# funkelab/cellulus

Measured on AMD Instinct MI355X. Metric: train crops/sec (U-Net fwd+bwd + OCE loss + Adam), higher is better.
Workload: dtype f32 (exact 3xbf16 operand split, 6 products, f32 accumulate)

## Files before the change

### cellulus_amd/_clx.py

```python

import ctypes
import os
from ctypes import POINTER, Structure, c_char_p, c_double, c_int, c_longlong, c_size_t, c_void_p

import torch

_HERE = os.path.dirname(os.path.abspath(__file__))
LIB_PATH = os.path.join(_HERE, "libclx.so")


class ClxError(RuntimeError):
    """A libclx entry point returned a negative status."""


class ClxSrc(Structure):

    _fields_ = [
        ("ptr", c_void_p),
        ("C", c_int),
        ("ld", c_int),
        ("D", c_int),
        ("H", c_int),
        ("W", c_int),
        ("oz", c_int),
        ("oy", c_int),
        ("ox", c_int),
        ("fz", c_int),
        ("fy", c_int),
        ("fx", c_int),
    ]


class ClxPackJob(Structure):

    _fields_ = [("w", c_void_p), ("wp", c_void_p), ("cout", c_int), ("cin", c_int), ("taps", c_int),
                ("cin_pad", c_int), ("cout_pad", c_int), ("mode", c_int)]


class ClxConvDesc(Structure):

    _fields_ = [
        ("nsrc", c_int),
        ("src", ClxSrc * 2),
        ("B", c_int),
        ("ID", c_int),
        ("IH", c_int),
        ("IW", c_int),
        ("KD", c_int),
        ("KH", c_int),
        ("KW", c_int),
        ("PD", c_int),
        ("PH", c_int),
        ("PW", c_int),
        ("N", c_int),
        ("wpack", c_void_p),
        ("bias", c_void_p),
        ("relu", c_int),
        ("mask", c_void_p),
        ("ld_mask", c_int),
        ("out", c_void_p),
        ("ld_out", c_int),
        ("accumulate", c_int),
        ("algo", c_int),
        ("workspace", c_void_p),
        ("workspace_bytes", c_size_t),
        ("vcache", c_void_p),
        ("vcache_valid", c_int),
        ("c_real", c_int),
        ("dy_vcache", c_void_p),
        ("gate_out", c_void_p),
        ("ld_gate", c_int),
        ("mask_bits", c_void_p),
        ("ld_mask_bits", c_int),
        ("det_turns", c_void_p),
        ("adjoint", c_int),
        ("pool_out", c_void_p),
        ("ld_pool", c_int),
        ("tile_list", c_void_p),
        ("tile_count", c_int),
        ("precision", c_int),
        ("wplanes", c_void_p),
        ("aplanes", c_void_p),
        ("aplanes_valid", c_int),
        ("dyplanes", c_void_p),
        ("dyplanes_valid", c_int),
        ("out_planes", c_void_p),
        ("out_colsum", c_void_p),
    ]


_P = c_void_p
_I = c_int
_LL = c_longlong
_D = c_double

PROTOTYPES = {
    "clx_last_error": (c_char_p, []),
    "clx_abi_version": (_I, []),
    "clx_device_count": (_I, []),
    "clx_profile_enable": (_I, [_I]),
    "clx_profile_read": (_I, [_I, POINTER(c_double), POINTER(c_double), POINTER(c_double)]),
    "clx_profile_clock": (_I, [POINTER(c_double), POINTER(c_double), _I]),
    "clx_conv_fwd": (_I, [POINTER(ClxConvDesc), _P]),
    "clx_conv_wgrad": (_I, [POINTER(ClxConvDesc), _P, _I, _P, _P, _P]),
    "clx_chain64_fwd": (_I, [_P, _I, _LL, _P, _P, _P, _I, _P, _I, _P, _P, _I, _I, _P, _I, _P, _I, _P]),
    "clx_chain64_bwd": (_I, [_P, _I, _I, _P, _I, _P, _I, _I, _LL, _P, _P, _P, _I, _P, _P, _P, _P, _P]),
    "clx_pack_weights": (_I, [_P, _P, _I, _I, _I, _I, _I, _I, _P]),
    "clx_pack_weights_batch": (_I, [_P, _I, _LL, _P]),
    "clx_unpack_wgrad": (_I, [_P, _P, _I, _I, _I, _I, _I, _P]),
    "clx_unpack_wgrad_wino": (_I, [_P, _P, _I, _I, _I, _I, _I, _I, _I, _P]),
    "clx_conv_workspace_bytes": (c_size_t, [POINTER(ClxConvDesc), _I]),
    "clx_conv_vcache_bytes": (c_size_t, [POINTER(ClxConvDesc), _I]),
    "clx_conv_sp_covers": (_I, [POINTER(ClxConvDesc), _I]),
    "clx_planes_bytes": (c_size_t, [_LL, _I]),
    "clx_split_planes": (_I, [_P, _LL, _LL, _I, _P, _P]),
    "clx_join_planes": (_I, [_P, _LL, _I, _P, _LL, _P]),
    "clx_gemm_planes": (_I, [_P, _P, _I, _I, _I, _P, _I, _P, _I, _P]),
    "clx_wgrad_planes": (_I, [_P, _P, _LL, _I, _I, _P, _I, _P]),
    "clx_conv_fused_applicable": (_I, [POINTER(ClxConvDesc)]),
    "clx_conv_fused_workspace_bytes": (c_size_t, [POINTER(ClxConvDesc)]),
    "clx_planar_to_pixel": (_I, [_P, _P, _I, _I, _LL, _I, _P]),
    "clx_pixel_to_planar": (_I, [_P, _P, _I, _I, _LL, _I, _P]),
    "clx_depth_to_space": (_I, [_P, _I, _P, _I, _I, _I, _I, _I, _I, _I, _I, _I, _P]),
    "clx_space_to_depth": (_I, [_P, _I, _P, _I, _I, _I, _I, _I, _I, _I, _I, _I, _P]),
    "clx_subpixel_split_weights": (_I, [_P, _P, _P] + [_I] * 10 + [_P]),
    "clx_subpixel_fold_grads": (_I, [_P, _P, _P] + [_I] * 10 + [_P]),
    "clx_maxpool_fwd": (_I, [_P, _P, _I, _I, _I, _I, _I, _I, _I, _I, _P]),
    "clx_changed_rows_workspace": (c_size_t, [_I, _I, _I, _I]),
    "clx_changed_rows": (_I, [_P, _P, _I, _I, _I, _I, _I, _I, _I, _I, _I, _P, _P, _LL, _P, _P]),
    "clx_changed_tiles": (_I, [_P, _I, _I, _I, _I, _I, _I, _I, _I, _I, _I, _I, _P, _P, _LL, _P]),
    "clx_grey_rows": (_I, [_P, _I, _I, _I, _I, _I, _P, _LL, _P, _P, _I, _I, _P, _I, _P]),
    "clx_conv_first_dgrad": (_I, [_P, _I, _P, _I, _I, _I, _I, _I, _I, _I, _P, _P]),
    "clx_gather_rows": (_I, [_P, _I, _P, _LL, _I, _P, _I, _P]),
    "clx_scatter_rows": (_I, [_P, _I, _P, _LL, _I, _P, _I, _P]),
    "clx_broadcast_rows": (_I, [_P, _LL, _P, _I, _P]),
    "clx_maxpool_bwd": (_I, [_P, _P, _P, _P] + [_I] * 7 + [_P] + [_I] * 8 + [_P]),
    "clx_upsample_bwd": (_I, [_P] + [_I] * 8 + [_P, _P] + [_I] * 8 + [_P]),
    "clx_gather_add_fwd": (_I, [_P, _P, _P, _I, _I, _I, _I, _I, _I, _P, _P]),
    "clx_gather_add_bwd": (_I, [_P, _P, _P, _I, _I, _I, _I, _I, _I, _P, _P]),
    "clx_oce_loss_fwd_bwd": (_I, [_P, _P, _P, _P, _LL, _I, ctypes.c_float, ctypes.c_float, ctypes.c_float, _P]),
    "clx_conv_wgrad_turns_bytes": (c_size_t, [POINTER(ClxConvDesc)]),
    "clx_colsum_scratch_bytes": (c_size_t, [_I]),
    "clx_colsum_ordered": (_I, [_P, _I, _LL, _I, _P, _P, _P]),
    "clx_oce_pairs_det_scratch_bytes": (c_size_t, [_I, _I, _LL]),
    "clx_oce_pairs_fused_det": (_I, [_P, _P, _P, _P, _P, _I, _I, _I, _I, _I, _I, ctypes.c_float, ctypes.c_float, _P, _P]),
    "clx_oce_pairs_fused": (_I, [_P, _P, _P, _P, _P, _I, _I, _I, _I, _I, _I, ctypes.c_float, ctypes.c_float, _P]),
    "clx_sample_pairs": (_I, [_P, _P, _P, _I, _I, _I, _I, _I, _I, POINTER(c_int), ctypes.c_ulonglong,
                              ctypes.c_ulonglong, _P]),
    "clx_adam_step": (_I, [_P, _P, _P, _P, _LL, _D, _D, _D, _D, _D, _I, _P]),
    "clx_adam_step_guarded": (_I, [_P, _P, _P, _P, _LL, _D, _D, _D, _D, _D, _I, _P, _P]),
    "clx_noise_stats": (_I, [_P, _P, _I, _I, _LL, _P]),
    "clx_noise_inject": (_I, [_P, _P, _P, _I, _I, _LL, ctypes.c_float, _P]),
    "clx_zero_many": (_I, [POINTER(_P), POINTER(_LL), _I, _P]),
    "clx_gather_rows_f64": (_I, [_P, _P, _LL, _I, _P, _P]),
    "clx_rows_extent_f64": (_I, [_P, _LL, _I, _P, _P]),
    "clx_noise_stats_minmax": (_I, [_P, _P, _I, _I, _LL, _P, _I, _P]),
    "clx_ms_prepare_workspace": (c_size_t, [_LL]),
    "clx_ms_prepare": (_I, [_P, _P, _D, _I, _I, _I, _I, _P, _P, _P, _P, _P]),
    "clx_ms_prepare_f32": (_I, [_P, _P, _D, _I, _I, _I, _I, _P, _P, _P, _P, _P]),
    "clx_ms_iterate": (_I, [_P, _I, _P, _I, _I, _D, _I, _P, _P, _P, _P]),
    "clx_ms_iterate_grid": (_I, [_P, _I, _P, POINTER(c_double), _D, _I, _I, _I, _P, _I, _I, _D, _I,
                                 _P, _P, _P, _P]),
    "clx_ms_assign": (_I, [_P, _P, _I, _P, _I, _I, _P, _P]),
    "clx_ms_assign_grid": (_I, [_P, _P, _I, _P, _I, _I, _P, _P, POINTER(c_double), _D, _I, _I, _I, _P, _P]),
    "clx_ms_assign_cells": (_I, [_P, _P, _I, _P, _I, _I, _P, _P, POINTER(c_double), _D, _I, _I, _I, _P, _P]),
    "clx_ms_assign_dense": (_I, [_P, _P, _I, _I, _P, _P, POINTER(c_double), _D, _I, _I, _I, _P, _I, _I, _I, _I, _P, _P]),
    "clx_ms_dedup_centers": (_I, [_P, _P, _I, _I, _D, _P, POINTER(_I)]),
    "clx_sample_offsets_mt19937": (_I, [_P, POINTER(_I), _I, _I, _LL, _P, POINTER(_I)]),
    "clx_elastic_crop_workspace": (c_size_t, [_I, POINTER(c_int), _I]),
    "clx_elastic_crop": (_I, [_P, _I, _I, _I, _I, POINTER(c_int), POINTER(c_int), POINTER(c_int), ctypes.c_float, _I, _I,
                              _P, _P, _P, _P, _P, _P]),
    "clx_ms_bucket_workspace": (c_size_t, [_I, _LL]),
    "clx_ms_bucket": (_I, [_P, _I, _I, POINTER(c_double), _D, _I, _I, _I, _P, _P, _P, _P]),
    "clx_offset_magnitude": (_I, [_P, _P, _I, _LL, _P]),
    "clx_gaussian_filter_f64": (_I, [_P, _P, _P, _I, _I, _I, _P, _I, _P]),
    "clx_negate_f64": (_I, [_P, _P, _LL, _P]),
    "clx_peak_local_max": (_I, [_P, _I, _I, _I, _P, _P, _I, _P, _P]),
    "clx_greedy_cluster": (_I, [_P, _P, _I, _I, _I, _D, _I, _D, _I, _P, _P, _P, _P]),
    "clx_cc_workspace": (c_size_t, [_LL]),
    "clx_cc_label_filter": (_I, [_P, _P, _I, _I, _I, _I, _P, _P, _P]),
    "clx_edt_workspace": (c_size_t, [_LL]),
    "clx_edt_sq": (_I, [_P, _P, _I, _I, _I, _I, _P, _P]),
    "clx_grow_shrink": (_I, [_P, _I, _I, _I, _I, _I, _P, _P]),
    "clx_minmax_f64": (_I, [_P, _LL, _P, _P]),
    "clx_histogram_f64": (_I, [_P, _LL, _P, _I, _P, _P]),
    "clx_minmax_f32": (_I, [_P, _LL, _P, _P]),
    "clx_histogram_f32": (_I, [_P, _LL, _P, _I, _P, _P]),
    "clx_inst_stats": (_I, [_P, _P, _I, _I, _I, _I, _I, _P, _P, _P]),
    "clx_inst_histogram": (_I, [_P, _P, _I, _LL, _P, _I, _P, _I, _P, _P]),
    "clx_inst_refine": (_I, [_P, _P, _I, _I, _I, _I, _I, _P, _P, _P, _P, _P, _I, _P, _P]),
    "clx_lz4_decompress": (_LL, [_P, _LL, _P, _LL]),
    "clx_blosclz_decompress": (_LL, [_P, _LL, _P, _LL]),
    "clx_blosc_compress_bound": (_LL, [_LL]),
    "clx_blosc_compress_lz4": (_LL, [_P, _LL, _I, _I, _P, _LL]),
    "clx_unshuffle_bytes": (_I, [_P, _P, _LL, _I]),
    "clx_label_presence": (_I, [_P, _LL, _I, _P, _P, _P]),
    "clx_joint_histogram": (_I, [_P, _P, _LL, _P, _P, _I, _P, _P]),
}

MINMAX_DOUBLES = 2 + 2 * 512
NOISE_MINMAX_FLOATS = 2 + 2 * 1024
ROWS_EXTENT_DOUBLES = 6 * (1 + 256)
NOISE_MINMAX_MAX_T = 64

_lib = None


def load():
    global _lib
    if _lib is not None:
        return _lib
    if not os.path.exists(LIB_PATH):
        raise ClxError(
            f"{LIB_PATH} is missing: build it with `python -m cellulus_amd._build` "
            "(hipcc --offload-arch=gfx950). cellulus_amd has no CPU fallback."
        )
    lib = ctypes.CDLL(LIB_PATH)
    for name, (restype, argtypes) in PROTOTYPES.items():
        fn = getattr(lib, name)
        fn.restype = restype
        fn.argtypes = argtypes
    _lib = lib
    return lib


def check(status, what=""):
    if status != 0:
        msg = load().clx_last_error().decode("utf-8", "replace")
        raise ClxError(f"{what or 'libclx'} failed ({status}): {msg}")


def stream_ptr(device=None):
    return c_void_p(torch.cuda.current_stream(device).cuda_stream)


def ptr(t):
    if t is None:
        return c_void_p(0)
    return c_void_p(t.data_ptr())


def zero_many(*tensors):
    ts = [t for t in tensors if t is not None and t.numel() > 0]
    if not ts:
        return
    dev = ts[0].device
    fast = []
    for t in ts:
        if not t.is_cuda:
            raise ClxError(f"zero_many: tensor on {t.device}; there is no CPU path")
        if t.device != dev:
            raise ClxError(f"zero_many: tensors on different devices ({dev} and {t.device}) in one call")
        nbytes = t.numel() * t.element_size()
        if t.is_contiguous() and t.data_ptr() % 16 == 0 and nbytes % 4 == 0:
            fast.append(t)
        else:
            t.zero_()
    if not fast:
        return
    ptrs = (_P * len(fast))(*[t.data_ptr() for t in fast])
    sizes = (_LL * len(fast))(*[t.numel() * t.element_size() for t in fast])
    call("clx_zero_many", ptrs, sizes, len(fast), stream_ptr(dev))


def zeros(shape, dtype, device):
    t = torch.empty(shape, dtype=dtype, device=device)
# ... 20 lines not shown
```

### cellulus_amd/csrc/clx_common.h

```cpp
#pragma once
#include <hip/hip_runtime.h>
#include <hip/hip_ext.h>
#include <stdint.h>
#include <stdio.h>
#include <stdarg.h>
#include "../../include/clx.h"

void clx_set_error(const char* fmt, ...);

#define CLX_REQUIRE(cond, ...)                \
  do {                                        \
    if (!(cond)) {                            \
      clx_set_error(__VA_ARGS__);             \
      return CLX_ERR_ARG;                     \
    }                                         \
  } while (0)

#define CLX_CHECK_LAUNCH(name)                                           \
  do {                                                                   \
    hipError_t e__ = hipGetLastError();                                  \
    if (e__ != hipSuccess) {                                             \
      clx_set_error("%s: launch failed: %s", name, hipGetErrorString(e__)); \
      return CLX_ERR_LAUNCH;                                             \
    }                                                                    \
  } while (0)

typedef float f32x4 __attribute__((ext_vector_type(4)));
typedef float f32x16 __attribute__((ext_vector_type(16)));

struct FastDiv {
  uint32_t m, l, d;
};
static inline FastDiv make_fastdiv(uint32_t d) {
  FastDiv f;
  f.d = d;
  uint32_t l = 0;
  while ((1ull << l) < d) ++l;
  f.l = l;
  f.m = (uint32_t)(((1ull << 32) * ((1ull << l) - d)) / d + 1);
  return f;
}
__device__ __forceinline__ uint32_t fdiv(uint32_t n, const FastDiv& f) {
  return (__umulhi(f.m, n) + n) >> f.l;
}

__device__ __forceinline__ int xcd_remap(int bid, int nblocks) {
  const int q = nblocks >> 3, r = nblocks & 7;
  const int xcd = bid & 7, idx = bid >> 3;
  const int base = (xcd < r) ? xcd * (q + 1) : r * (q + 1) + (xcd - r) * q;
  return base + idx;
}

static inline int cdiv(long long a, long long b) { return (int)((a + b - 1) / b); }

bool clx_smallc_applicable(const clx_conv_desc* d);
int clx_smallc_fwd(const clx_conv_desc* d, hipStream_t st);
int clx_smallc_wgrad(const clx_conv_desc* d, const float* dy, int ld_dy, float* dwpack,
                     float* dbias, hipStream_t st);

int clx_igemm_launch(const clx_conv_desc* d, int batch, long long bs_in, long long bs_w,
                     long long bs_out, hipStream_t st);
int clx_wgrad_launch(const clx_conv_desc* d, const float* dy, int ld_dy, float* dwpack, float* dbias,
                     int batch, long long bs_x, long long bs_dy, long long bs_out, hipStream_t st);
bool clx_sp_fwd_rule(const clx_conv_desc* d);
bool clx_sp_wgrad_rule(const clx_conv_desc* d);
bool clx_sp_applicable(const clx_conv_desc* d);
bool clx_wino_sp(const clx_conv_desc* d);
int clx_sp_launch(const void* A, const void* B, int M, int N, int K, long long rows_a, int batch, long long bs_a, long long bs_b,
                  long long bs_out, const clx_conv_desc* ep, hipStream_t st);
int clx_sp_clock_read(double* shader_ticks, double* wall_ticks, int reset);
int clx_sp_split(const float* x, long long ld, long long rows, int K, void* planes, float* colsum, int nreal, hipStream_t st);
int clx_sp_wgrad_launch(const void* dy_planes, const void* x_planes, long long rows, int N, int C, int batch, long long bs_dy,
                        long long bs_x, long long bs_out, float* dw, int ld_dw, hipStream_t st);
int clx_wino_fwd(const clx_conv_desc* d, hipStream_t st);
int clx_wino_wgrad(const clx_conv_desc* d, const float* dy, int ld_dy, float* dwpack, float* dbias,
                   hipStream_t st);
int clx_wino_pack(const float* w, float* wp, int cout, int cin, int cin_pad, int cout_pad, int dgrad, int tile,
                  int ksize, int kd, hipStream_t st);

int clx_wino_fused_fwd(const clx_conv_desc* d, hipStream_t st);

bool clx_prof_enabled();
void clx_prof_events(int kind, double flops, hipEvent_t* e0, hipEvent_t* e1);
#define CLX_LAUNCH_TIMED(kernel, grid, block, st, e0, e1, ...) \
  hipExtLaunchKernelGGL(kernel, grid, block, 0, st, e0, e1, 0, __VA_ARGS__)
#define CLX_LAUNCH_KIND(kind, kernel, grid, block, lds, st, ...)                              \
  do {                                                                                        \
    hipEvent_t e0__ = nullptr, e1__ = nullptr;                                                \
    if (clx_prof_enabled()) clx_prof_events(kind, 0.0, &e0__, &e1__);                         \
    hipExtLaunchKernelGGL(kernel, grid, block, lds, st, e0__, e1__, 0, __VA_ARGS__);          \
  } while (0)
```

### cellulus_amd/csrc/conv_igemm.hip

```cpp
#include "clx_common.h"
#include <stdlib.h>

__device__ unsigned long long g_clk_ticks[2];
extern "C" int clx_profile_clock(double* shader_ticks, double* wall_ticks_100mhz, int reset) {
  unsigned long long h[2] = {0ull, 0ull};
  if (hipMemcpyFromSymbol(h, HIP_SYMBOL(g_clk_ticks), sizeof(h)) != hipSuccess) {
    clx_set_error("clx_profile_clock: copy failed");
    return CLX_ERR_LAUNCH;
  }
  double sc = 0.0, sw = 0.0;
  if (clx_sp_clock_read(&sc, &sw, reset) != CLX_OK) {
    clx_set_error("clx_profile_clock: copy failed");
    return CLX_ERR_LAUNCH;
  }
  if (shader_ticks) *shader_ticks = (double)h[0] + sc;
  if (wall_ticks_100mhz) *wall_ticks_100mhz = (double)h[1] + sw;
  if (reset) {
    const unsigned long long z[2] = {0ull, 0ull};
    if (hipMemcpyToSymbol(HIP_SYMBOL(g_clk_ticks), z, sizeof(z)) != hipSuccess) {
      clx_set_error("clx_profile_clock: reset failed");
      return CLX_ERR_LAUNCH;
    }
  }
  return CLX_OK;
// ... 330 lines not shown
  constexpr int PH = 8;
  static_assert(ITERS % PH == 0, "phases");
  const int c4 = (tid % F4_PER_ROW) * 4;
  const int n = n0 + c4;
  const bool n_live = n < p.N;
  const bool full4 = n + 3 < p.N;
#pragma unroll 1
  for (int h0 = 0; h0 < ITERS; h0 += PH) {
    f32x4 val[PH];
    int mrow[PH];
    bool live[PH];
#pragma unroll
    for (int j = 0; j < PH; ++j) {
      const int row = (tid + 256 * (h0 + j)) / F4_PER_ROW;
      mrow[j] = m0 + row;
      live[j] = mrow[j] < p.M && n_live;
      val[j] = *reinterpret_cast<const f32x4*>(&Cs[row * LDC + c4]);
    }
    float* const out_base = p.out + blockIdx.y * p.bs_out + n;
    if (p.accumulate) {
      f32x4 prev[PH];
#pragma unroll
      for (int j = 0; j < PH; ++j)
        prev[j] = *reinterpret_cast<const f32x4*>(live[j] ? out_base + (size_t)mrow[j] * p.ld_out : p.zeros);
#pragma unroll
      for (int j = 0; j < PH; ++j) val[j] += prev[j];
    }
    if (p.relu) {
#pragma unroll
      for (int j = 0; j < PH; ++j)
#pragma unroll
        for (int e = 0; e < 4; ++e) val[j][e] = fmaxf(val[j][e], 0.f);
    }
    if (p.mask_bits) {
      unsigned int w[PH];
#pragma unroll
      for (int j = 0; j < PH; ++j)
        w[j] = live[j] ? p.mask_bits[(size_t)mrow[j] * p.ld_mask_bits + (n >> 5)] : 0u;
#pragma unroll
      for (int j = 0; j < PH; ++j)
#pragma unroll
        for (int e = 0; e < 4; ++e) val[j][e] = ((w[j] >> ((n & 31) + e)) & 1u) ? val[j][e] : 0.f;
    }
    if (p.gate_out) {
#pragma unroll
      for (int j = 0; j < PH; ++j) {
        unsigned int nib = 0u;
#pragma unroll
        for (int e = 0; e < 4; ++e) nib |= (live[j] && n + e < p.N && val[j][e] > 0.f) ? (1u << e) : 0u;
        unsigned int word = nib << (4 * (lane & 7));
        word |= __shfl_xor(word, 1, 64);
        word |= __shfl_xor(word, 2, 64);
        word |= __shfl_xor(word, 4, 64);
        if ((lane & 7) == 0 && mrow[j] < p.M && n < p.ld_out) p.gate_out[(size_t)mrow[j] * p.ld_gate + (n >> 5)] = word;
      }
    }
    if (p.mask && full4) {
      f32x4 mk[PH];
#pragma unroll
      for (int j = 0; j < PH; ++j)
        mk[j] = *reinterpret_cast<const f32x4*>(live[j] ? p.mask + (size_t)mrow[j] * p.ld_mask + n : p.zeros);
#pragma unroll
      for (int j = 0; j < PH; ++j)
#pragma unroll
        for (int e = 0; e < 4; ++e) val[j][e] = (!live[j] || mk[j][e] > 0.f) ? val[j][e] : 0.f;
    }
    if (full4) {
#pragma unroll
      for (int j = 0; j < PH; ++j)
        if (live[j]) *reinterpret_cast<f32x4*>(out_base + (size_t)mrow[j] * p.ld_out) = val[j];
    } else if (n_live) {
#pragma unroll 1
      for (int j = 0; j < PH; ++j) {
        if (!live[j]) continue;
        float* dst = out_base + (size_t)mrow[j] * p.ld_out;
        for (int e = 0; e < 4 && n + e < p.N; ++e) {
          float x = val[j][e];
          if (p.mask) x = (p.mask[(size_t)mrow[j] * p.ld_mask + n + e] > 0.f) ? x : 0.f;
          dst[e] = x;
        }
      }
    }
  }
  if (clk_block) { atomicAdd(&g_clk_ticks[0], clock64() - clk_c0); atomicAdd(&g_clk_ticks[1], wall_clock64() - clk_w0); }
}

}

static const float* zero_buffer() {
  static const float* cache[64] = {nullptr};
  int dev = 0;
  if (hipGetDevice(&dev) != hipSuccess || dev < 0 || dev >= 64) return nullptr;
  if (cache[dev] == nullptr) {
    void* ptr = nullptr;
    if (hipGetSymbolAddress(&ptr, HIP_SYMBOL(g_zero16)) != hipSuccess) return nullptr;
    cache[dev] = (const float*)ptr;
  }
  return cache[dev];
}

static int conv_validate(const clx_conv_desc* d, const char* who) {
  CLX_REQUIRE(d != nullptr, "%s: null descriptor", who);
  CLX_REQUIRE(d->nsrc == 1 || d->nsrc == 2, "%s: nsrc must be 1 or 2", who);
  CLX_REQUIRE(d->B > 0 && d->ID > 0 && d->IH > 0 && d->IW > 0, "%s: bad extent", who);
  const int K[3] = {d->KD, d->KH, d->KW};
  const int P[3] = {d->PD, d->PH, d->PW};
  const int I[3] = {d->ID, d->IH, d->IW};
  for (int i = 0; i < 3; ++i) {
    CLX_REQUIRE(K[i] >= 1 && K[i] <= 3, "%s: kernel extent must be 1, 2 or 3", who);
    CLX_REQUIRE(P[i] >= 0 && P[i] < K[i], "%s: padding must be < kernel extent", who);
    CLX_REQUIRE(I[i] + 2 * P[i] - K[i] + 1 > 0, "%s: input smaller than kernel", who);
  }
  for (int s = 0; s < d->nsrc; ++s) {
    const clx_src& S = d->src[s];
    CLX_REQUIRE(S.ptr != nullptr, "%s: null source %d", who, s);
    CLX_REQUIRE(S.C > 0 && S.C % 4 == 0 && S.ld % 4 == 0 && S.ld >= S.C,
                "%s: source channels/ld must be multiples of 4 (C=%d ld=%d)", who, S.C, S.ld);
    CLX_REQUIRE(((uintptr_t)S.ptr & 15) == 0, "%s: source pointer must be 16-byte aligned", who);
    CLX_REQUIRE(S.fz >= 1 && S.fy >= 1 && S.fx >= 1, "%s: upsample factors >= 1", who);
    CLX_REQUIRE(S.oz >= 0 && S.oy >= 0 && S.ox >= 0, "%s: negative crop", who);
    CLX_REQUIRE((d->ID - 1 + S.oz) / S.fz < S.D && (d->IH - 1 + S.oy) / S.fy < S.H &&
                    (d->IW - 1 + S.ox) / S.fx < S.W,
                "%s: source %d smaller than the logical input", who, s);
  }
  const long long M = (long long)d->B * (d->ID + 2 * d->PD - d->KD + 1) *
                      (d->IH + 2 * d->PH - d->KH + 1) * (d->IW + 2 * d->PW - d->KW + 1);
  CLX_REQUIRE(M < (1ll << 31), "%s: too many output pixels", who);
  return CLX_OK;
}

static void fill_params(const clx_conv_desc* d, ConvP& p) {
  p.nsrc = d->nsrc;
  for (int s = 0; s < 2; ++s) {
    const clx_src& S = d->src[s < d->nsrc ? s : 0];
    p.src[s] = SrcP{S.ptr, S.C, S.ld, S.D, S.H, S.W, S.oz, S.oy, S.ox, S.fz, S.fy, S.fx};
  }
  p.B = d->B; p.ID = d->ID; p.IH = d->IH; p.IW = d->IW;
  p.KD = d->KD; p.KH = d->KH; p.KW = d->KW;
  p.PD = d->PD; p.PH = d->PH; p.PW = d->PW;
  p.OD = d->ID + 2 * d->PD - d->KD + 1;
  p.OH = d->IH + 2 * d->PH - d->KH + 1;
  p.OW = d->IW + 2 * d->PW - d->KW + 1;
  p.N = d->N;
  p.M = d->B * p.OD * p.OH * p.OW;
  p.Ctot = d->src[0].C + (d->nsrc == 2 ? d->src[1].C : 0);
  p.Ktot = p.Ctot * d->KD * d->KH * d->KW;
  p.dOW = make_fastdiv(p.OW); p.dOH = make_fastdiv(p.OH); p.dOD = make_fastdiv(p.OD);
  p.wpack = d->wpack; p.bias = d->bias; p.mask = d->mask; p.out = d->out;
  p.gate_out = d->gate_out; p.ld_gate = d->ld_gate; p.mask_bits = d->mask_bits; p.ld_mask_bits = d->ld_mask_bits;
  p.relu = d->relu; p.ld_mask = d->ld_mask; p.ld_out = d->ld_out;
  p.accumulate = d->accumulate;
  p.bs_in = p.bs_w = p.bs_out = 0;
  p.flush_every = 0;
}

extern "C" int clx_conv_fwd(const clx_conv_desc* d, clx_stream stream) {
  int rc = conv_validate(d, "clx_conv_fwd");
  if (rc) return rc;
  CLX_REQUIRE(d->wpack && d->out, "clx_conv_fwd: null wpack/out");
  CLX_REQUIRE(d->N > 0 && d->ld_out >= d->N, "clx_conv_fwd: bad N/ld_out");
  CLX_REQUIRE(((uintptr_t)d->wpack & 15) == 0, "clx_conv_fwd: wpack must be 16-byte aligned");
  CLX_REQUIRE(d->mask == nullptr || (d->ld_mask >= d->N && d->ld_mask % 4 == 0 &&
                                     ((uintptr_t)d->mask & 15) == 0),
              "clx_conv_fwd: mask must be 16-byte aligned with ld_mask %% 4 == 0 and >= N");
  CLX_REQUIRE(d->ld_out % 4 == 0 && ((uintptr_t)d->out & 15) == 0,
              "clx_conv_fwd: out must be 16-byte aligned with ld_out %% 4 == 0");
  CLX_REQUIRE(d->gate_out == nullptr || (d->relu && d->ld_out % 32 == 0 && d->ld_gate * 32 >= d->ld_out),
              "clx_conv_fwd: gate_out needs relu, ld_out %% 32 == 0 and ld_gate >= ld_out / 32");
  CLX_REQUIRE(d->mask_bits == nullptr || (d->mask == nullptr && d->ld_mask_bits * 32 >= d->N),
              "clx_conv_fwd: mask_bits replaces mask and needs ld_mask_bits >= ceil(N / 32)");
  CLX_REQUIRE(d->algo == CLX_ALGO_DIRECT || d->algo == CLX_ALGO_WINOGRAD || d->algo == CLX_ALGO_WINOGRAD4 ||
                  d->algo == CLX_ALGO_WINOGRAD4_FUSED,
              "clx_conv_fwd: bad algo");
  CLX_REQUIRE((d->out_planes == nullptr && d->out_colsum == nullptr && !d->aplanes_valid) ||
                  (d->algo == CLX_ALGO_DIRECT && d->aplanes != nullptr && clx_sp_applicable(d)),
              "clx_conv_fwd: out_planes / out_colsum / aplanes_valid need the split-precision 1x1 product "
              "(clx_conv_sp_covers, wplanes and aplanes)");
  if (d->algo == CLX_ALGO_WINOGRAD4_FUSED) return clx_wino_fused_fwd(d, (hipStream_t)stream);
  if (d->algo != CLX_ALGO_DIRECT) return clx_wino_fwd(d, (hipStream_t)stream);
  CLX_REQUIRE(d->pool_out == nullptr && d->tile_list == nullptr && !d->adjoint,
              "clx_conv_fwd: pool_out / tile_list / adjoint need a Winograd algorithm (algo = %d)", d->algo);
  if (clx_smallc_applicable(d) && d->mask == nullptr && d->mask_bits == nullptr && d->gate_out == nullptr) {
    clx_smallc_fwd(d, (hipStream_t)stream);
    CLX_CHECK_LAUNCH("clx_conv_fwd(small-channel)");
    return CLX_OK;
  }
  rc = clx_igemm_launch(d, 1, 0, 0, 0, (hipStream_t)stream);
  if (rc) return rc;
  CLX_CHECK_LAUNCH("clx_conv_fwd");
  return CLX_OK;
}

int clx_igemm_launch(const clx_conv_desc* d, int batch, long long bs_in, long long bs_w,
                     long long bs_out, hipStream_t st) {
  if (batch == 1 && d->aplanes != nullptr && clx_sp_applicable(d)) {
    const clx_src& S = d->src[0];
    const long long M = (long long)d->B * d->ID * d->IH * d->IW;
    if (!d->aplanes_valid) {
      const int rc = clx_sp_split(S.ptr, S.ld, M, S.C, d->aplanes, nullptr, 0, st);
      if (rc) return rc;
    }
    return clx_sp_launch(d->aplanes, d->wplanes, (int)M, d->N, S.C, M, 1, 0, 0, 0, d, st);
  }
  ConvP p;
  fill_params(d, p);
  p.zeros = zero_buffer();
  CLX_REQUIRE(p.zeros != nullptr, "clx_conv_fwd: cannot resolve the device zero buffer");
  p.bs_in = bs_in; p.bs_w = bs_w; p.bs_out = bs_out;
  static const int flush_env = getenv("CLX_IGEMM_FLUSH") ? atoi(getenv("CLX_IGEMM_FLUSH")) : 2;
  p.flush_every = flush_env > 0 ? flush_env : 0;
  const bool wide = d->N > 64 && (double)(cdiv(d->N, 128) * 128) / d->N <= 1.2;
  hipEvent_t e0 = nullptr, e1 = nullptr;
  if (clx_prof_enabled())
    clx_prof_events(wide ? CLX_PROF_IGEMM_WIDE : CLX_PROF_IGEMM_NARROW, 2.0 * p.M * p.N * p.Ktot * batch, &e0, &e1);
  static const bool fast_env = getenv("CLX_IGEMM_FAST") == nullptr || atoi(getenv("CLX_IGEMM_FAST")) != 0;
  int fast = fast_env && (long long)p.N * p.Ktot < (1ll << 30) ? 1 : 0;
  const bool padded = d->PD != 0 || d->PH != 0 || d->PW != 0;
  for (int s = 0; s < d->nsrc && fast; ++s) {
    const clx_src& S = d->src[s];
    const long long floats = (long long)d->B * S.D * S.H * S.W * S.ld;
    if (S.C % BK != 0 || floats >= (padded ? (1ll << 29) : (1ll << 30))) fast = 0;
  }
  if (fast && padded) fast = 2;
  static const bool dbg = getenv("CLX_IGEMM_DEBUG") != nullptr;
  if (dbg) fprintf(stderr, "igemm fast=%d wide=%d M=%d N=%d K=%d batch=%d pad=%d%d%d k=%d%d%d nsrc=%d C0=%d\n", (int)fast, (int)wide, p.M, p.N, p.Ktot, batch, d->PD, d->PH, d->PW, d->KD, d->KH, d->KW, d->nsrc, d->src[0].C);
  if (wide) {
    p.nbm = cdiv(p.M, 128); p.nbn = cdiv(p.N, 128);
    if (fast == 1) CLX_LAUNCH_TIMED((conv_igemm_kernel<128, 128, 2, 2, 1>), dim3(p.nbm * p.nbn, batch), dim3(256), st, e0, e1, p);
    else if (fast == 2) CLX_LAUNCH_TIMED((conv_igemm_kernel<128, 128, 2, 2, 2>), dim3(p.nbm * p.nbn, batch), dim3(256), st, e0, e1, p);
    else CLX_LAUNCH_TIMED((conv_igemm_kernel<128, 128, 2, 2>), dim3(p.nbm * p.nbn, batch), dim3(256), st, e0, e1, p);
  } else {
    p.nbm = cdiv(p.M, 128); p.nbn = cdiv(p.N, 64);
    if (fast == 1) CLX_LAUNCH_TIMED((conv_igemm_kernel<128, 64, 4, 1, 1>), dim3(p.nbm * p.nbn, batch), dim3(256), st, e0, e1, p);
    else if (fast == 2) CLX_LAUNCH_TIMED((conv_igemm_kernel<128, 64, 4, 1, 2>), dim3(p.nbm * p.nbn, batch), dim3(256), st, e0, e1, p);
    else CLX_LAUNCH_TIMED((conv_igemm_kernel<128, 64, 4, 1>), dim3(p.nbm * p.nbn, batch), dim3(256), st, e0, e1, p);
  }
  return CLX_OK;
}
```

### cellulus_amd/csrc/conv_smallc.hip

```cpp
#include "clx_common.h"

namespace {

struct SmallP {
  const float* x;
  int ld_x, B, D, H, W;
  int oz, oy, ox;
  int ID, IH, IW, KD, KH, KW, PD, PH, PW, OD, OH, OW;
  int N, M, taps;
  FastDiv dOW, dOH, dOD;
  const float* wpack;
  const float* bias;
  float* out;
  int ld_out, relu;
  const float* dy;
  int ld_dy;
  float* dwp;
  float* dbias;
  int tiles_per_block;
  int RX, items;
  FastDiv dRX;
};

constexpr int PT = 64;
constexpr int MAX_TAPS = 27;

template <int PTILE>
__device__ __forceinline__ void stage_patch(const SmallP& p, int m0, float* Xs) {
  static_assert(256 % PTILE == 0, "a thread keeps one pixel of the tile");
  const int K4 = p.taps;
  const int pl = threadIdx.x % PTILE;
  const uint32_t m = (uint32_t)(m0 + pl);
  const bool live = m < (uint32_t)p.M;
  const uint32_t q1 = fdiv(m, p.dOW);
  const int ox = (int)(m - q1 * p.OW);
  const uint32_t q2 = fdiv(q1, p.dOH);
  const int oy = (int)(q1 - q2 * p.OH);
  const uint32_t q3 = fdiv(q2, p.dOD);
  const int oz = (int)(q2 - q3 * p.OD);
  const int b = (int)q3;
  int tx = 0, ty = 0, tz = 0;
  {
    const int tap = threadIdx.x / PTILE;
    tx = tap % p.KW; ty = (tap / p.KW) % p.KH; tz = tap / (p.KW * p.KH);
  }
  constexpr int STEP = 256 / PTILE;
  for (int tap = threadIdx.x / PTILE; tap < K4; tap += STEP) {
    f32x4 v = {0.f, 0.f, 0.f, 0.f};
    const int lz = oz + tz - p.PD, ly = oy + ty - p.PH, lx = ox + tx - p.PW;
    if (live && (unsigned)lz < (unsigned)p.ID && (unsigned)ly < (unsigned)p.IH && (unsigned)lx < (unsigned)p.IW) {
      const long long pix = (((long long)b * p.D + lz + p.oz) * p.H + ly + p.oy) * p.W + lx + p.ox;
      v = *reinterpret_cast<const f32x4*>(p.x + pix * p.ld_x);
    }
    *reinterpret_cast<f32x4*>(&Xs[(pl * K4 + tap) * 4]) = v;
    tx += STEP;
    while (tx >= p.KW) { tx -= p.KW; if (++ty == p.KH) { ty = 0; ++tz; } }
  }
}

template <int NG>
__global__ __launch_bounds__(256) void conv_smallc_fwd_kernel(const SmallP p) {
  constexpr int PL = 256 / NG;
  constexpr int PPT = PT / PL;
  extern __shared__ float smem[];
  const int K = p.taps * 4;
  float* Ws = smem;
  float* Xs = smem + K * NG * 4;
  const int n0 = blockIdx.y * NG * 4;
  const int ng = threadIdx.x % NG, pl = threadIdx.x / NG;
  __shared__ int used_channels;
  if (threadIdx.x == 0) used_channels = 0;
  __syncthreads();
  int mine_used = 0;
  for (int idx = threadIdx.x; idx < K * NG * 4; idx += 256) {
    const int n = idx / K, k = idx % K;
    const float wv = (n0 + n < p.N) ? p.wpack[(size_t)(n0 + n) * K + k] : 0.f;
    Ws[k * NG * 4 + n] = wv;
    if (wv != 0.f) mine_used |= 1 << (k & 3);
  }
  if (mine_used) atomicOr(&used_channels, mine_used);
  const int n = n0 + ng * 4;
  f32x4 bv = {0.f, 0.f, 0.f, 0.f};
  if (p.bias && n < p.N) {
#pragma unroll
    for (int e = 0; e < 4; ++e) bv[e] = (n + e < p.N) ? p.bias[n + e] : 0.f;
  }
  for (int t = 0; t < p.tiles_per_block; ++t) {
    const int m0 = (blockIdx.x * p.tiles_per_block + t) * PT;
    if (m0 >= p.M) break;
    __syncthreads();
    stage_patch<PT>(p, m0, Xs);
    __syncthreads();
    f32x4 acc[PPT];
#pragma unroll
    for (int i = 0; i < PPT; ++i) acc[i] = bv;
    const int used = used_channels;
    for (int c = 0; c < 4; ++c) {
      if (!((used >> c) & 1)) continue;
      for (int k = c; k < K; k += 4) {
        const f32x4 w = *reinterpret_cast<const f32x4*>(&Ws[k * NG * 4 + ng * 4]);
#pragma unroll
        for (int i = 0; i < PPT; ++i) {
          const float xv = Xs[(pl + i * PL) * K + k];
          acc[i] += xv * w;
        }
      }
    }
    if (n < p.N) {
#pragma unroll
      for (int i = 0; i < PPT; ++i) {
        const int m = m0 + pl + i * PL;
        if (m >= p.M) continue;
        f32x4 v = acc[i];
        if (p.relu) {
#pragma unroll
          for (int e = 0; e < 4; ++e) v[e] = fmaxf(v[e], 0.f);
        }
        float* dst = p.out + (size_t)m * p.ld_out + n;
        if (n + 3 < p.N) *reinterpret_cast<f32x4*>(dst) = v;
        else
          for (int e = 0; e < 4 && n + e < p.N; ++e) dst[e] = v[e];
      }
    }
  }
}

template <int G>
__global__ __launch_bounds__(256) void conv_smallc_wgrad_stream_kernel(const SmallP p) {
  constexpr int Q = 256 / G;
  constexpr int MT = 9;
  extern __shared__ float red[];
  const int g = threadIdx.x % G, q = threadIdx.x / G;
  const int NT = G * 4;
  const int n0 = blockIdx.y * NT, n = n0 + g * 4;
  const int tap0 = blockIdx.z * MT;
  const int ntap = p.taps - tap0 < MT ? p.taps - tap0 : MT;
  const int nred = ntap * 4 * NT + NT;
  for (int i = threadIdx.x; i < nred; i += 256) red[i] = 0.f;
  f32x4 acc[MT][4];
#pragma unroll
  for (int a = 0; a < MT; ++a)
#pragma unroll
    for (int c = 0; c < 4; ++c) acc[a][c] = f32x4{0.f, 0.f, 0.f, 0.f};
  f32x4 bsum = {0.f, 0.f, 0.f, 0.f};
  const long long per = (long long)p.tiles_per_block;
  const long long m_begin = (long long)blockIdx.x * per;
  const long long m_end = m_begin + per < p.M ? m_begin + per : p.M;
  const bool live = n < p.N;
  const int gtap = tap0 + (g < ntap ? g : 0);
  const int my_tx = gtap % p.KW - p.PW, my_ty = (gtap / p.KW) % p.KH - p.PH, my_tz = gtap / (p.KW * p.KH) - p.PD;
  for (long long mm = m_begin + q; mm < m_end; mm += Q) {
    const uint32_t m = (uint32_t)mm;
    const uint32_t q1 = fdiv(m, p.dOW);
    const int ox = (int)(m - q1 * p.OW);
    const uint32_t q2 = fdiv(q1, p.dOH);
    const int oy = (int)(q1 - q2 * p.OH);
    const uint32_t q3 = fdiv(q2, p.dOD);
    const int oz = (int)(q2 - q3 * p.OD);
    const int b = (int)q3;
    f32x4 dyv = {0.f, 0.f, 0.f, 0.f};
    if (live) dyv = *reinterpret_cast<const f32x4*>(p.dy + (size_t)m * p.ld_dy + n);
    if (tap0 == 0) bsum += dyv;
    if constexpr (G >= 16) {
      f32x4 mine = {0.f, 0.f, 0.f, 0.f};
      if (g < ntap) {
        const int lz = oz + my_tz, ly = oy + my_ty, lx = ox + my_tx;
        if ((unsigned)lz < (unsigned)p.ID && (unsigned)ly < (unsigned)p.IH && (unsigned)lx < (unsigned)p.IW) {
          const long long pix = (((long long)b * p.D + lz + p.oz) * p.H + ly + p.oy) * p.W + lx + p.ox;
          mine = *reinterpret_cast<const f32x4*>(p.x + pix * p.ld_x);
        }
      }
#pragma unroll
      for (int a = 0; a < MT; ++a) {
        if (a < ntap) {
          f32x4 xv;
#pragma unroll
          for (int c = 0; c < 4; ++c) {
            xv[c] = __shfl(mine[c], (int)(threadIdx.x & 63 & ~(G - 1)) + a, 64);
          }
#pragma unroll
          for (int c = 0; c < 4; ++c) acc[a][c] += xv[c] * dyv;
        }
      }
    } else {
#pragma unroll
      for (int a = 0; a < MT; ++a) {
        if (a < ntap) {
          const int tap = tap0 + a;
          const int lz = oz + tap / (p.KW * p.KH) - p.PD, ly = oy + (tap / p.KW) % p.KH - p.PH, lx = ox + tap % p.KW - p.PW;
          f32x4 xv = {0.f, 0.f, 0.f, 0.f};
          if ((unsigned)lz < (unsigned)p.ID && (unsigned)ly < (unsigned)p.IH && (unsigned)lx < (unsigned)p.IW) {
            const long long pix = (((long long)b * p.D + lz + p.oz) * p.H + ly + p.oy) * p.W + lx + p.ox;
            xv = *reinterpret_cast<const f32x4*>(p.x + pix * p.ld_x);
          }
#pragma unroll
          for (int c = 0; c < 4; ++c) acc[a][c] += xv[c] * dyv;
        }
      }
    }
  }
  __syncthreads();
#pragma unroll
  for (int a = 0; a < MT; ++a) {
    if (a < ntap) {
#pragma unroll
      for (int c = 0; c < 4; ++c)
#pragma unroll
        for (int e = 0; e < 4; ++e) atomicAdd(&red[(a * 4 + c) * NT + g * 4 + e], acc[a][c][e]);
    }
  }
#pragma unroll
  for (int e = 0; e < 4; ++e) atomicAdd(&red[ntap * 4 * NT + g * 4 + e], bsum[e]);
  __syncthreads();
  for (int i = threadIdx.x; i < ntap * 4 * NT; i += 256) {
    const int nl = i % NT, c = (i / NT) & 3, tap = tap0 + i / (4 * NT);
    if (n0 + nl < p.N) atomicAdd(p.dwp + ((size_t)tap * p.N + n0 + nl) * 4 + c, red[i]);
  }
  if (p.dbias && tap0 == 0)
    for (int i = threadIdx.x; i < NT; i += 256)
      if (n0 + i < p.N) atomicAdd(p.dbias + n0 + i, red[ntap * 4 * NT + i]);
}

struct Run {
  int ox0, m0;
  long long base;
};

__device__ __forceinline__ Run decode_run(const SmallP& p, uint32_t item) {
  const uint32_t q1 = fdiv(item, p.dRX);
  const int rx = (int)(item - q1 * p.RX);
  const uint32_t q2 = fdiv(q1, p.dOH);
  const int oy = (int)(q1 - q2 * p.OH);
  const uint32_t q3 = fdiv(q2, p.dOD);
  const int oz = (int)(q2 - q3 * p.OD);
  const int b = (int)q3;
  Run r;
  r.ox0 = rx * 4;
  r.m0 = ((b * p.OD + oz) * p.OH + oy) * p.OW + r.ox0;
  r.base = (((long long)b * p.D + oz + p.oz) * p.H + oy + p.oy) * p.W + r.ox0 + p.ox;
  return r;
}

template <int KD>
struct GreyLane {
  static constexpr int R = KD * 3, NP = R * 6, TAPS = R * 3;
  int px, cq, col;
  long long poff;
  __device__ __forceinline__ GreyLane(const SmallP& p) {
    const int lane = threadIdx.x & 63;
    px = lane >> 4; cq = lane & 15;
    const int l = lane < NP ? lane : 0;
    const int r = l / 6;
    col = l - r * 6;
    const int tz = r / 3, ty = r - tz * 3;
    poff = ((long long)tz * p.H + ty) * p.W;
  }
  __device__ __forceinline__ float load_patch(const SmallP& p, const Run& r) const {
    const int c = r.ox0 + col < p.IW ? col : p.IW - 1 - r.ox0;
    return p.x[(r.base + poff + c) * p.ld_x];
  }
  __device__ __forceinline__ float tap(float pv, int row, int tx) const {
    return __shfl(pv, row * 6 + tx + px, 64);
  }
};

template <int KD>
__global__ __launch_bounds__(256) void conv_grey_fwd_kernel(const SmallP p) {
  using L = GreyLane<KD>;
  const L ln(p);
  const int wave = __builtin_amdgcn_readfirstlane(threadIdx.x >> 6);
  const int n = blockIdx.y * 64 + ln.cq * 4;
  const bool live_n = n < p.N;
  f32x4 w[L::TAPS];
#pragma unroll
  for (int t = 0; t < L::TAPS; ++t)
#pragma unroll
    for (int e = 0; e < 4; ++e) w[t][e] = live_n ? p.wpack[((size_t)(n + e) * L::TAPS + t) * 4] : 0.f;
  f32x4 bv = {0.f, 0.f, 0.f, 0.f};
  if (p.bias && live_n) bv = *reinterpret_cast<const f32x4*>(p.bias + n);
  const uint32_t last = (uint32_t)p.items - 1, stride = gridDim.x * 4;
  uint32_t item = blockIdx.x * 4 + wave;
  Run r[3];
  float pv[3];
#pragma unroll
  for (int s = 0; s < 2; ++s) {
    r[s] = decode_run(p, item + s * stride < last ? item + s * stride : last);
    pv[s] = ln.load_patch(p, r[s]);
  }
  while (true) {
#pragma unroll
    for (int s = 0; s < 3; ++s) {
      if (item > last) return;
      const int s2 = (s + 2) % 3;
      const uint32_t nxt = item + 2 * stride;
      r[s2] = decode_run(p, nxt < last ? nxt : last);
      pv[s2] = ln.load_patch(p, r[s2]);
      f32x4 acc = bv;
#pragma unroll
      for (int row = 0; row < L::R; ++row)
#pragma unroll
        for (int tx = 0; tx < 3; ++tx) acc += ln.tap(pv[s], row, tx) * w[row * 3 + tx];
      if (p.relu) {
#pragma unroll
        for (int e = 0; e < 4; ++e) acc[e] = fmaxf(acc[e], 0.f);
      }
      if (live_n && r[s].ox0 + ln.px < p.OW)
        *reinterpret_cast<f32x4*>(p.out + (size_t)(r[s].m0 + ln.px) * p.ld_out + n) = acc;
      item += stride;
    }
  }
}

template <int KD>
__global__ __launch_bounds__(256) void conv_grey_wgrad_kernel(const SmallP p) {
  using L = GreyLane<KD>;
  __shared__ float red[(L::TAPS + 1) * 64];
  const L ln(p);
  const int wave = __builtin_amdgcn_readfirstlane(threadIdx.x >> 6);
  const int n0 = blockIdx.y * 64, n = n0 + ln.cq * 4;
  const bool live_n = n < p.N;
  const int nld = live_n ? n : 0;
  for (int i = threadIdx.x; i < (L::TAPS + 1) * 64; i += 256) red[i] = 0.f;
  f32x4 acc[L::TAPS];
#pragma unroll
  for (int t = 0; t < L::TAPS; ++t) acc[t] = f32x4{0.f, 0.f, 0.f, 0.f};
  f32x4 bsum = {0.f, 0.f, 0.f, 0.f};
  const uint32_t last = (uint32_t)p.items - 1, stride = gridDim.x * 4;
  uint32_t item = blockIdx.x * 4 + wave;
  auto load_dy = [&](const Run& r) {
    const int m = r.ox0 + ln.px < p.OW ? r.m0 + ln.px : r.m0;
    return *reinterpret_cast<const f32x4*>(p.dy + (size_t)m * p.ld_dy + nld);
  };
  Run r[3];
  float pv[3];
  f32x4 dy[3];
#pragma unroll
  for (int s = 0; s < 2; ++s) {
    r[s] = decode_run(p, item + s * stride < last ? item + s * stride : last);
    pv[s] = ln.load_patch(p, r[s]);
    dy[s] = load_dy(r[s]);
  }
  bool more = item <= last;
  while (more) {
#pragma unroll
    for (int s = 0; s < 3; ++s) {
      if (more) {
        const int s2 = (s + 2) % 3;
        const uint32_t nxt = item + 2 * stride;
        r[s2] = decode_run(p, nxt < last ? nxt : last);
        pv[s2] = ln.load_patch(p, r[s2]);
        dy[s2] = load_dy(r[s2]);
        const bool ok = live_n && r[s].ox0 + ln.px < p.OW;
        f32x4 dyv;
#pragma unroll
        for (int e = 0; e < 4; ++e) dyv[e] = ok ? dy[s][e] : 0.f;
        bsum += dyv;
#pragma unroll
        for (int row = 0; row < L::R; ++row)
#pragma unroll
          for (int tx = 0; tx < 3; ++tx) acc[row * 3 + tx] += ln.tap(pv[s], row, tx) * dyv;
        item += stride;
        more = item <= last;
      }
    }
  }
  __syncthreads();
#pragma unroll
  for (int t = 0; t < L::TAPS; ++t)
#pragma unroll
    for (int e = 0; e < 4; ++e) atomicAdd(&red[t * 64 + ln.cq * 4 + e], acc[t][e]);
#pragma unroll
  for (int e = 0; e < 4; ++e) atomicAdd(&red[L::TAPS * 64 + ln.cq * 4 + e], bsum[e]);
  __syncthreads();
  for (int i = threadIdx.x; i < L::TAPS * 64; i += 256) {
    const int nl = i & 63, t = i >> 6;
    if (n0 + nl < p.N) atomicAdd(p.dwp + ((size_t)t * p.N + n0 + nl) * 4, red[i]);
  }
  if (p.dbias && threadIdx.x < 64 && n0 + threadIdx.x < p.N)
    atomicAdd(p.dbias + n0 + threadIdx.x, red[L::TAPS * 64 + threadIdx.x]);
}

template <int KD>
__global__ __launch_bounds__(256) void conv_grey_rows_kernel(const float* __restrict__ x, int D, int H, int W, int OD,
                                                             int OH, int OW, const int* __restrict__ rows, long long n,
                                                             const float* __restrict__ wpack,
                                                             const float* __restrict__ bias, int relu, int N,
                                                             float* __restrict__ out, int ld_out) {
  constexpr int R = KD * 3, TAPS = R * 3;
  const int lane = threadIdx.x & 63, px = lane >> 4, cq = lane & 15;
  const int nn = blockIdx.y * 64 + cq * 4;
  const bool live_n = nn < N;
  f32x4 w[TAPS];
#pragma unroll
  for (int t = 0; t < TAPS; ++t)
#pragma unroll
    for (int e = 0; e < 4; ++e) w[t][e] = live_n ? wpack[((size_t)(nn + e) * TAPS + t) * 4] : 0.f;
  f32x4 bv = {0.f, 0.f, 0.f, 0.f};
  if (bias && live_n) bv = *reinterpret_cast<const f32x4*>(bias + nn);
  const long long npo = (long long)OD * OH * OW;
  const long long groups = (n + 3) / 4;
  for (long long g = (long long)blockIdx.x * 4 + (threadIdx.x >> 6); g < groups; g += (long long)gridDim.x * 4) {
    const long long r = g * 4 + px;
    const bool live = r < n;
    const long long row = rows[live ? r : n - 1];
    const long long b = row / npo, pix = row - b * npo;
    const int ox = (int)(pix % OW), oy = (int)((pix / OW) % OH), oz = (int)(pix / ((long long)OW * OH));
    const float* src = x + ((b * D + oz) * H + oy) * (long long)W + ox;
    float xv[TAPS];
#pragma unroll
    for (int rr = 0; rr < R; ++rr)
#pragma unroll
      for (int tx = 0; tx < 3; ++tx) xv[rr * 3 + tx] = src[((long long)(rr / 3) * H + (rr % 3)) * W + tx];
    f32x4 acc = bv;
#pragma unroll
    for (int rr = 0; rr < R; ++rr)
#pragma unroll
      for (int tx = 0; tx < 3; ++tx) acc += xv[rr * 3 + tx] * w[rr * 3 + tx];
    if (relu) {
#pragma unroll
      for (int e = 0; e < 4; ++e) acc[e] = fmaxf(acc[e], 0.f);
    }
    if (live && live_n) *reinterpret_cast<f32x4*>(out + (size_t)r * ld_out + nn) = acc;
  }
}

bool grey_applicable(const clx_conv_desc* d, int ld_act) {
  return d->c_real == 1 && d->KH == 3 && d->KW == 3 && (d->KD == 1 || d->KD == 3) && d->PD == 0 &&
         d->PH == 0 && d->PW == 0 && d->N % 4 == 0 && ld_act % 4 == 0;
}

dim3 grey_grid(SmallP& p) {
  p.RX = cdiv(p.OW, 4);
  p.items = p.B * p.OD * p.OH * p.RX;
  p.dRX = make_fastdiv(p.RX);
  const int ny = cdiv(p.N, 64);
  int nx = 768 / ny;
  if (nx < 1) nx = 1;
  if (nx > cdiv(p.items, 4)) nx = cdiv(p.items, 4);
  return dim3(nx, ny);
}

bool fill(const clx_conv_desc* d, SmallP& p) {
  const clx_src& S = d->src[0];
  p.x = S.ptr; p.ld_x = S.ld; p.B = d->B; p.D = S.D; p.H = S.H; p.W = S.W;
  p.oz = S.oz; p.oy = S.oy; p.ox = S.ox;
  p.ID = d->ID; p.IH = d->IH; p.IW = d->IW;
  p.KD = d->KD; p.KH = d->KH; p.KW = d->KW;
  p.PD = d->PD; p.PH = d->PH; p.PW = d->PW;
  p.OD = d->ID + 2 * d->PD - d->KD + 1;
  p.OH = d->IH + 2 * d->PH - d->KH + 1;
  p.OW = d->IW + 2 * d->PW - d->KW + 1;
  p.N = d->N;
  p.M = d->B * p.OD * p.OH * p.OW;
  p.taps = d->KD * d->KH * d->KW;
  p.dOW = make_fastdiv(p.OW); p.dOH = make_fastdiv(p.OH); p.dOD = make_fastdiv(p.OD);
  return true;
}

int pick_ng(int N) {
  int ng = 4;
  while (ng < 64 && ng * 4 < N) ng *= 2;
  return ng;
}

}

bool clx_smallc_applicable(const clx_conv_desc* d) {
  if (d->nsrc != 1 || d->accumulate) return false;
  const clx_src& S = d->src[0];
  if (S.C != 4 || S.fz != 1 || S.fy != 1 || S.fx != 1) return false;
  const int taps = d->KD * d->KH * d->KW;
  return taps > 1 && taps <= MAX_TAPS && d->N >= 4;
}

int clx_smallc_fwd(const clx_conv_desc* d, hipStream_t st) {
  SmallP p{};
  fill(d, p);
  p.wpack = d->wpack; p.bias = d->bias; p.out = d->out; p.ld_out = d->ld_out; p.relu = d->relu;
  if (grey_applicable(d, d->ld_out) && ((uintptr_t)d->out & 15) == 0 && (!d->bias || ((uintptr_t)d->bias & 15) == 0)) {
    const dim3 grid = grey_grid(p);
    if (d->KD == 1) conv_grey_fwd_kernel<1><<<grid, 256, 0, st>>>(p);
    else conv_grey_fwd_kernel<3><<<grid, 256, 0, st>>>(p);
    return CLX_OK;
  }
  const int ng = pick_ng(p.N);
  const int K = p.taps * 4;
  const int tiles = cdiv(p.M, PT);
  p.tiles_per_block = tiles > 4096 ? 4 : 1;
  const dim3 grid(cdiv(tiles, p.tiles_per_block), cdiv(p.N, ng * 4));
  const size_t lds = (size_t)(K * ng * 4 + PT * K) * sizeof(float);
  switch (ng) {
    case 4: conv_smallc_fwd_kernel<4><<<grid, 256, lds, st>>>(p); break;
    case 8: conv_smallc_fwd_kernel<8><<<grid, 256, lds, st>>>(p); break;
    case 16: conv_smallc_fwd_kernel<16><<<grid, 256, lds, st>>>(p); break;
    case 32: conv_smallc_fwd_kernel<32><<<grid, 256, lds, st>>>(p); break;
    default: conv_smallc_fwd_kernel<64><<<grid, 256, lds, st>>>(p); break;
  }
  return CLX_OK;
}

int clx_smallc_wgrad(const clx_conv_desc* d, const float* dy, int ld_dy, float* dwpack,
                     float* dbias, hipStream_t st) {
  SmallP p{};
  fill(d, p);
  p.dy = dy; p.ld_dy = ld_dy; p.dwp = dwpack; p.dbias = dbias;
  if (grey_applicable(d, ld_dy) && ((uintptr_t)dy & 15) == 0) {
    const dim3 grid = grey_grid(p);
    if (d->KD == 1) conv_grey_wgrad_kernel<1><<<grid, 256, 0, st>>>(p);
    else conv_grey_wgrad_kernel<3><<<grid, 256, 0, st>>>(p);
    return CLX_OK;
  }
  const int ng = pick_ng(p.N);
  const int blocks = p.M < 512 * 64 ? cdiv(p.M, 64) : 512;
  p.tiles_per_block = cdiv(p.M, blocks);
  const dim3 grid(cdiv(p.M, p.tiles_per_block), cdiv(p.N, ng * 4), cdiv(p.taps, 9));
  const size_t lds = (size_t)((p.taps < 9 ? p.taps : 9) * 4 * ng * 4 + ng * 4) * sizeof(float);
  switch (ng) {
    case 4: conv_smallc_wgrad_stream_kernel<4><<<grid, 256, lds, st>>>(p); break;
    case 8: conv_smallc_wgrad_stream_kernel<8><<<grid, 256, lds, st>>>(p); break;
    case 16: conv_smallc_wgrad_stream_kernel<16><<<grid, 256, lds, st>>>(p); break;
    case 32: conv_smallc_wgrad_stream_kernel<32><<<grid, 256, lds, st>>>(p); break;
    default: conv_smallc_wgrad_stream_kernel<64><<<grid, 256, lds, st>>>(p); break;
  }
  return CLX_OK;
}

extern "C" int clx_grey_rows(const float* x, int B, int ID, int IH, int IW, int KD, const int* rows, long long n,
                             const float* wpack, const float* bias, int relu, int N, float* out, int ld_out,
                             clx_stream stream) {
  CLX_REQUIRE(n >= 0, "clx_grey_rows: bad count");
  if (n == 0) return CLX_OK;
  CLX_REQUIRE(x && rows && wpack && out, "clx_grey_rows: null pointer");
  CLX_REQUIRE(B > 0 && (KD == 1 || KD == 3) && ID >= KD && IH >= 3 && IW >= 3, "clx_grey_rows: a 3x3 or 3x3x3 window");
  CLX_REQUIRE(N > 0 && N % 4 == 0 && ld_out % 4 == 0 && ld_out >= N && ((uintptr_t)out & 15) == 0 &&
                  (!bias || ((uintptr_t)bias & 15) == 0),
              "clx_grey_rows: N, ld_out multiples of 4, aligned out / bias");
  const int OD = ID - KD + 1, OH = IH - 2, OW = IW - 2;
  long long gx = (n + 15) / 16;
  if (gx > 4096) gx = 4096;
  const dim3 grid((unsigned)gx, (unsigned)((N + 63) / 64));
  hipStream_t st = (hipStream_t)stream;
  if (KD == 1) conv_grey_rows_kernel<1><<<grid, 256, 0, st>>>(x, ID, IH, IW, OD, OH, OW, rows, n, wpack, bias, relu, N, out, ld_out);
  else conv_grey_rows_kernel<3><<<grid, 256, 0, st>>>(x, ID, IH, IW, OD, OH, OW, rows, n, wpack, bias, relu, N, out, ld_out);
  CLX_CHECK_LAUNCH("clx_grey_rows");
  return CLX_OK;
}
```

### cellulus_amd/csrc/gemm_sp.hip

```cpp
#include "clx_common.h"
#include "sp_planes.h"
#include <stdlib.h>
#include <type_traits>

__device__ unsigned long long g_sp_clk_ticks[2];
int clx_sp_clock_read(double* shader_ticks, double* wall_ticks, int reset) {
  unsigned long long h[2] = {0ull, 0ull};
  if (hipMemcpyFromSymbol(h, HIP_SYMBOL(g_sp_clk_ticks), sizeof(h)) != hipSuccess) return CLX_ERR_LAUNCH;
  *shader_ticks = (double)h[0];
  *wall_ticks = (double)h[1];
  if (reset) {
    const unsigned long long z[2] = {0ull, 0ull};
    if (hipMemcpyToSymbol(HIP_SYMBOL(g_sp_clk_ticks), z, sizeof(z)) != hipSuccess) return CLX_ERR_LAUNCH;
  }
  return CLX_OK;
}

namespace {

typedef __bf16 bf16x8 __attribute__((ext_vector_type(8)));
using sp::u32x2;
using sp::u32x4;
using sp::FRAG;
using sp::KSTEP;
constexpr int SP_BM = 256, SP_BN = 128;
constexpr int A_FRAGS = SP_BM / 32 * 3;
constexpr int B_FRAGS = SP_BN / 32 * 3;
constexpr int STAGE = (A_FRAGS + B_FRAGS) * FRAG;
constexpr int RING = 4;
constexpr int LDC = SP_BN + 4;

__device__ __forceinline__ void glds16(const char* g, char* l) {
  __builtin_amdgcn_global_load_lds((const __attribute__((address_space(1))) void*)g,
                                   (__attribute__((address_space(3))) void*)l, 16, 0, 0);
}

using sp::split4;

template <bool COLSUM>
__global__ __launch_bounds__(256) void sp_split_kernel(const float* __restrict__ x, long long ld, long long rows, int ksteps,
                                                       char* __restrict__ out, long long nfrag, float* __restrict__ colsum, int nreal) {
  const int lane = threadIdx.x & 63;
  const long long w0 = ((long long)blockIdx.x * blockDim.x + threadIdx.x) >> 6, nw = ((long long)gridDim.x * blockDim.x) >> 6;
  const int r = lane & 31, h = lane >> 5;
  f32x4 s0 = {0.f, 0.f, 0.f, 0.f}, s1 = s0;
  for (long long f = w0; f < nfrag; f += nw) {
    const int ks = (int)(f % ksteps);
    const long long rb = f / ksteps;
    const long long row = rb * 32 + r;
    f32x4 v0 = {0.f, 0.f, 0.f, 0.f}, v1 = v0;
    if (row < rows) {
      const float* src = x + row * ld + ks * 16 + h * 8;
      v0 = *reinterpret_cast<const f32x4*>(src);
      v1 = *reinterpret_cast<const f32x4*>(src + 4);
    }
    if constexpr (COLSUM) { s0 += v0; s1 += v1; }
    u32x2 a0, a1, a2, b0, b1, b2;
    split4(v0, a0, a1, a2);
    split4(v1, b0, b1, b2);
    char* dst = out + f * KSTEP + lane * 16;
    *reinterpret_cast<u32x4*>(dst) = u32x4{a0[0], a0[1], b0[0], b0[1]};
    *reinterpret_cast<u32x4*>(dst + FRAG) = u32x4{a1[0], a1[1], b1[0], b1[1]};
    *reinterpret_cast<u32x4*>(dst + 2 * FRAG) = u32x4{a2[0], a2[1], b2[0], b2[1]};
  }
  if constexpr (COLSUM) {
    if (w0 < nfrag) {
      const int ks = (int)(w0 % ksteps);
#pragma unroll
      for (int e = 0; e < 4; ++e) {
#pragma unroll
        for (int m = 1; m < 32; m <<= 1) { s0[e] += __shfl_xor(s0[e], m, 64); s1[e] += __shfl_xor(s1[e], m, 64); }
      }
      if (r == 0) {
#pragma unroll
        for (int e = 0; e < 4; ++e) {
          const int k0 = ks * 16 + h * 8 + e;
          if (k0 < nreal) atomicAdd(colsum + k0, s0[e]);
          if (k0 + 4 < nreal) atomicAdd(colsum + k0 + 4, s1[e]);
        }
      }
    }
  }
}

__global__ __launch_bounds__(256) void sp_join_kernel(const char* __restrict__ in, long long ld, long long rows, int ksteps,
                                                      float* __restrict__ x, long long nfrag) {
  const int lane = threadIdx.x & 63;
  const long long w0 = ((long long)blockIdx.x * blockDim.x + threadIdx.x) >> 6, nw = ((long long)gridDim.x * blockDim.x) >> 6;
  const int r = lane & 31, h = lane >> 5;
  for (long long f = w0; f < nfrag; f += nw) {
    const int ks = (int)(f % ksteps);
    const long long rb = f / ksteps;
    const long long row = rb * 32 + r;
    if (row >= rows) continue;
    const char* src = in + f * KSTEP + lane * 16;
    const u32x4 q0 = *reinterpret_cast<const u32x4*>(src), q1 = *reinterpret_cast<const u32x4*>(src + FRAG),
                q2 = *reinterpret_cast<const u32x4*>(src + 2 * FRAG);
    float* dst = x + row * ld + ks * 16 + h * 8;
#pragma unroll
    for (int e = 0; e < 8; ++e) {
      const int sh = (e & 1) * 16;
      const float f0 = __uint_as_float(((q0[e >> 1] >> sh) & 0xffffu) << 16);
      const float f1 = __uint_as_float(((q1[e >> 1] >> sh) & 0xffffu) << 16);
      const float f2 = __uint_as_float(((q2[e >> 1] >> sh) & 0xffffu) << 16);
      dst[e] = (f0 + f1) + f2;
    }
  }
}

__global__ __launch_bounds__(256) void sp_zero_tail_kernel(char* __restrict__ planes, long long bs, long long rows, int ksteps) {
  const long long rb0 = rows >> 5, rb1 = sp::padded_rows(rows) / 32;
  const int per_rb = ksteps * 6 * 32;
  const long long total = (rb1 - rb0) * per_rb;
  for (long long i = (long long)blockIdx.x * blockDim.x + threadIdx.x; i < total; i += (long long)gridDim.x * blockDim.x) {
    const long long rb = rb0 + i / per_rb;
    const int k = (int)(i % per_rb), r = k & 31, q = k >> 5;
    if (rb * 32 + r >= rows)
      *reinterpret_cast<u32x4*>(planes + blockIdx.y * bs + rb * ksteps * (long long)KSTEP + (long long)q * 512 + r * 16) = u32x4{0u, 0u, 0u, 0u};
  }
}

struct SpP {
  const char* A;
  const char* B;
  long long bs_a, bs_b, bs_out;
  float* out;
  int M, N, ksteps;
  int rb_a;
  int rb_b;
  const float* bias;
  const float* mask;
  const unsigned int* mask_bits;
  unsigned int* gate_out;
  const float* zeros;
  int relu, accumulate, ld_out, ld_mask, ld_mask_bits, ld_gate;
  int nbm, nbn;
  char* out_planes;
  float* colsum; int colsum_n;
  unsigned int stride_a, stride_b;
  int total_steps, steps_per_slice, nslices;
};

template <int BM = SP_BM, int NWAVES = 8, int BN = SP_BN>
__device__ __forceinline__ void sp_epilogue_from_lds(const SpP& p, const float* Cs, int m0, int n0, int batch, int tid, int lane) {
  constexpr int WPR = BN / 32;
  constexpr int LDC = BN + 4;
  constexpr int PASS_ROWS = NWAVES / WPR * 8;
  constexpr int ITERS = BM / PASS_ROWS;
  constexpr int PH = 8;
  static_assert(ITERS % PH == 0, "whole groups of passes");
  const int wv = tid >> 6;
  const int c4 = (wv % WPR) * 32 + (lane & 7) * 4;
  const int row0 = (wv / WPR) * 8 + (lane >> 3);
  const int n = n0 + c4;
  const bool n_live = n < p.N;
  f32x4 csum = {0.f, 0.f, 0.f, 0.f};
  const long long prow = p.out_planes ? sp::padded_rows(p.M) : 0;
#pragma unroll 1
  for (int h0 = 0; h0 < ITERS; h0 += PH) {
    f32x4 val[PH];
    int mrow[PH];
    bool live[PH];
#pragma unroll
    for (int j = 0; j < PH; ++j) {
      const int row = row0 + PASS_ROWS * (h0 + j);
      mrow[j] = m0 + row;
      live[j] = mrow[j] < p.M && n_live;
      val[j] = *reinterpret_cast<const f32x4*>(&Cs[row * LDC + c4]);
    }
    float* const out_base = p.out + batch * p.bs_out + n;
    if (p.accumulate) {
      f32x4 prev[PH];
#pragma unroll
      for (int j = 0; j < PH; ++j)
        prev[j] = *reinterpret_cast<const f32x4*>(live[j] ? out_base + (size_t)mrow[j] * p.ld_out : p.zeros);
#pragma unroll
      for (int j = 0; j < PH; ++j) val[j] += prev[j];
    }
    if (p.relu) {
#pragma unroll
      for (int j = 0; j < PH; ++j)
#pragma unroll
        for (int e = 0; e < 4; ++e) val[j][e] = fmaxf(val[j][e], 0.f);
    }
    if (p.mask_bits) {
      unsigned int wd[PH];
#pragma unroll
      for (int j = 0; j < PH; ++j) wd[j] = live[j] ? p.mask_bits[(size_t)mrow[j] * p.ld_mask_bits + (n >> 5)] : 0u;
#pragma unroll
      for (int j = 0; j < PH; ++j)
#pragma unroll
        for (int e = 0; e < 4; ++e) val[j][e] = ((wd[j] >> ((n & 31) + e)) & 1u) ? val[j][e] : 0.f;
    }
    if (p.gate_out) {
#pragma unroll
      for (int j = 0; j < PH; ++j) {
        unsigned int nib = 0u;
#pragma unroll
        for (int e = 0; e < 4; ++e) nib |= (live[j] && val[j][e] > 0.f) ? (1u << e) : 0u;
        unsigned int word = nib << (4 * (lane & 7));
        word |= __shfl_xor(word, 1, 64);
        word |= __shfl_xor(word, 2, 64);
        word |= __shfl_xor(word, 4, 64);
        if ((lane & 7) == 0 && mrow[j] < p.M && n_live) p.gate_out[(size_t)mrow[j] * p.ld_gate + (n >> 5)] = word;
      }
    }
    if (p.mask) {
      f32x4 mk[PH];
#pragma unroll
      for (int j = 0; j < PH; ++j)
        mk[j] = *reinterpret_cast<const f32x4*>(live[j] ? p.mask + (size_t)mrow[j] * p.ld_mask + n : p.zeros);
#pragma unroll
      for (int j = 0; j < PH; ++j)
#pragma unroll
        for (int e = 0; e < 4; ++e) val[j][e] = (!live[j] || mk[j][e] > 0.f) ? val[j][e] : 0.f;
    }
#pragma unroll
    for (int j = 0; j < PH; ++j)
      if (live[j]) *reinterpret_cast<f32x4*>(out_base + (size_t)mrow[j] * p.ld_out) = val[j];
    if (p.out_planes) {
#pragma unroll
      for (int j = 0; j < PH; ++j)
        if (n_live && mrow[j] < prow)
          sp::store4(p.out_planes, mrow[j], n, p.N >> 4, live[j] ? val[j] : f32x4{0.f, 0.f, 0.f, 0.f});
    }
    if (p.colsum) {
#pragma unroll
      for (int j = 0; j < PH; ++j)
        if (live[j]) csum += val[j];
    }
  }
  if (p.colsum) {
#pragma unroll
    for (int e = 0; e < 4; ++e) {
      csum[e] += __shfl_xor(csum[e], 8, 64);
      csum[e] += __shfl_xor(csum[e], 16, 64);
      csum[e] += __shfl_xor(csum[e], 32, 64);
    }
    if ((lane >> 3) == 0 && n_live) {
#pragma unroll
      for (int e = 0; e < 4; ++e)
        if (n + e < p.colsum_n) atomicAdd(p.colsum + n + e, csum[e]);
    }
  }
}

template <int MODE>
__global__ __launch_bounds__(512, 1) void gemm_sp_kernel(const SpP p) {
  __shared__ __attribute__((aligned(16))) char smem[RING * STAGE];
  const int tid = threadIdx.x, lane = tid & 63;
  const int w = __builtin_amdgcn_readfirstlane(tid >> 6);
  const int wm = w >> 1, wn = w & 1;
  int tile_m, tile_n, batch, step0 = 0, ksteps;
  if constexpr (MODE == 0) {
    const int v = xcd_remap(blockIdx.x, p.nbm * p.nbn);
    tile_n = v % p.nbn; tile_m = v / p.nbn;
    batch = blockIdx.y;
    ksteps = p.ksteps;
  } else {
    const int T = p.nbm * p.nbn;
    const int u = xcd_remap(blockIdx.x, gridDim.x);
    const int per_batch = T * p.nslices;
    batch = u / per_batch;
    const int v = u % per_batch;
    const int slice = v / T, t = v % T;
    tile_n = t % p.nbn; tile_m = t / p.nbn;
    step0 = slice * p.steps_per_slice;
    ksteps = p.total_steps - step0 < p.steps_per_slice ? p.total_steps - step0 : p.steps_per_slice;
  }
  const int m0 = tile_m * SP_BM, n0 = tile_n * SP_BN;
  const bool clk_block = blockIdx.x == gridDim.x / 2 && blockIdx.y == gridDim.y / 2 && threadIdx.x == 0;
  unsigned long long clk_c0 = 0, clk_w0 = 0;
  if (clk_block) { clk_c0 = clock64(); clk_w0 = wall_clock64(); }

  const char* const Ab = p.A + batch * p.bs_a;
  const char* const Bb = p.B + batch * p.bs_b;
  auto frag_base = [&](int f) __attribute__((always_inline)) -> const char* {
    if constexpr (MODE == 0) {
      if (f < A_FRAGS) {
        int rb = tile_m * (SP_BM / 32) + f / 3;
        if (rb > p.rb_a - 1) rb = p.rb_a - 1;
        return Ab + ((long long)rb * ksteps * 3 + f % 3) * FRAG;
      }
      const int g = f - A_FRAGS;
      int nb = tile_n * (SP_BN / 32) + g / 3;
      if (nb > p.rb_b - 1) nb = p.rb_b - 1;
      return Bb + ((long long)nb * ksteps * 3 + g % 3) * FRAG;
    } else {
      if (f < A_FRAGS) {
        int cb = tile_m * (SP_BM / 32) + f / 3;
        if (cb > p.M / 32 - 1) cb = p.M / 32 - 1;
        return Ab + ((long long)(2 * cb) * 3 + f % 3) * FRAG;
      }
      const int g = f - A_FRAGS;
      int cb = tile_n * (SP_BN / 32) + g / 3;
      if (cb > p.N / 32 - 1) cb = p.N / 32 - 1;
      return Bb + ((long long)(2 * cb) * 3 + g % 3) * FRAG;
    }
  };
  const char* gsrc[5];
#pragma unroll
  for (int q = 0; q < 4; ++q) gsrc[q] = frag_base(w + 8 * q);
  gsrc[4] = frag_base(32 + (w & 3));
  const int l_oct = lane >> 4, l_pix = (lane & 15) ^ (4 * (lane >> 4));
  const unsigned int lane16 = MODE == 0 ? (unsigned int)lane * 16u
                                        : (unsigned int)((l_oct >> 1) * KSTEP + (l_oct & 1) * 512 + l_pix * 16);
  const bool low_half = w < 4;
  auto issue = [&](int t, int slot, bool odd) __attribute__((always_inline)) {
    char* const dst = smem + slot * STAGE;
    if constexpr (MODE == 0) {
      const unsigned int voff = lane16 + (unsigned int)t * KSTEP;
#pragma unroll
      for (int q = 0; q < 4; ++q) glds16(gsrc[q] + (size_t)voff, dst + (w + 8 * q) * FRAG);
      if (low_half != odd) glds16(gsrc[4] + (size_t)voff, dst + (32 + (w & 3)) * FRAG);
    } else {
      const unsigned int ts = (unsigned int)(step0 + t);
      const unsigned int va = lane16 + (ts >> 1) * p.stride_a + (ts & 1u) * 256u;
      const unsigned int vb = lane16 + (ts >> 1) * p.stride_b + (ts & 1u) * 256u;
#pragma unroll
      for (int q = 0; q < 3; ++q) glds16(gsrc[q] + (size_t)va, dst + (w + 8 * q) * FRAG);
      glds16(gsrc[3] + (size_t)vb, dst + (w + 24) * FRAG);
      if (low_half != odd) glds16(gsrc[4] + (size_t)vb, dst + (32 + (w & 3)) * FRAG);
    }
  };
  auto wait_two = [&]() __attribute__((always_inline)) { asm volatile("s_waitcnt vmcnt(9)" ::: "memory"); };
  auto wait_one = [&]() __attribute__((always_inline)) { asm volatile("s_waitcnt vmcnt(4)" ::: "memory"); };

  f32x16 acc[2][2], tot[2][2];
#pragma unroll
  for (int i = 0; i < 2; ++i)
#pragma unroll
    for (int j = 0; j < 2; ++j)
#pragma unroll
      for (int r = 0; r < 16; ++r) { acc[i][j][r] = 0.f; tot[i][j][r] = 0.f; }

  const int li = lane & 31, lh = lane >> 5;
  float bias_v[2];
#pragma unroll
  for (int j = 0; j < 2; ++j) {
    const int n = n0 + (wn * 2 + j) * 32 + li;
    bias_v[j] = (p.bias && n < p.N) ? p.bias[n] : 0.f;
  }

  unsigned int la[RING], lb[RING];
#pragma unroll
  for (int k = 0; k < RING; ++k) {
    const int r_oct = 2 * ((lane >> 4) & 1) + ((lane & 3) >> 1), r_pix = 8 * (lane >> 5) + ((lane >> 2) & 3);
    const int lterm = MODE == 0 ? lane * 16 : r_oct * 256 + (r_pix ^ (4 * r_oct)) * 16 + (lane & 1) * 8;
    la[k] = k * STAGE + (wm * 2 * 3) * FRAG + lterm;
    lb[k] = k * STAGE + (A_FRAGS + wn * 2 * 3) * FRAG + lterm;
    asm volatile("" : "+v"(la[k]), "+v"(lb[k]));
  }

  u32x4 fa[2][3], fb[2][3];
  auto read_frags = [&](int slot) __attribute__((always_inline)) {
    const char* const as = smem + la[slot];
    const char* const bs = smem + lb[slot];
    auto rd = [&](const char* ptr) __attribute__((always_inline)) -> u32x4 {
      if constexpr (MODE == 0) {
        return *reinterpret_cast<const u32x4*>(ptr);
      } else {
        typedef short s16x4 __attribute__((ext_vector_type(4)));
        typedef __attribute__((address_space(3))) s16x4* lds_s16x4;
        const s16x4 lo = __builtin_amdgcn_ds_read_tr16_b64_v4i16((lds_s16x4)(ptr));
        const s16x4 hi = __builtin_amdgcn_ds_read_tr16_b64_v4i16((lds_s16x4)((uintptr_t)ptr ^ 64));
        const u32x2 l2 = __builtin_bit_cast(u32x2, lo), h2 = __builtin_bit_cast(u32x2, hi);
        return u32x4{l2[0], l2[1], h2[0], h2[1]};
      }
    };
    fa[0][2] = rd(as + 2 * FRAG);
    fb[0][0] = rd(bs);
    fa[0][0] = rd(as);
// ... 564 lines not shown
      period(per, late_tag, T{}, F{}, P0{});
      period(per + 1, late_tag, F{}, F{}, P0{});
    }
    if (per + 2 == nper) {
      period(per, late_tag, T{}, F{}, P0{});
      period(per + 1, late_tag, F{}, F{}, P2{});
    } else {
      period(per, late_tag, T{}, F{}, P2{});
    }
  };
  issue_a(0, 0);
  issue_b(0, 0);
  issue_a(1, 1);
  if (w >= 4) __builtin_amdgcn_s_setprio(1);
  if (w < 4) k_loop(std::false_type{});
  else k_loop(std::true_type{});
  __builtin_amdgcn_s_setprio(0);

  if (clk_block) { atomicAdd(&g_sp_clk_ticks[0], clock64() - clk_c0); atomicAdd(&g_sp_clk_ticks[1], wall_clock64() - clk_w0); }
  __syncthreads();
  float* Cs = reinterpret_cast<float*>(smem);
#pragma unroll
  for (int j = 0; j < 4; ++j) {
    const int col = wn * 64 + 16 * j + (lane & 15);
    const int n = n0 + col;
    const float bv = (p.bias && n < p.N) ? p.bias[n] : 0.f;
#pragma unroll
    for (int i = 0; i < 4; ++i)
#pragma unroll
      for (int r = 0; r < 4; ++r) Cs[(wm * 64 + 16 * i + 4 * (lane >> 4) + r) * LDC + col] = tot[i][j][r] + bv;
  }
  __syncthreads();
  sp_epilogue_from_lds(p, Cs, m0, n0, batch, tid, lane);
}

__device__ __attribute__((aligned(16))) float g_sp_zero16[4] = {0.f, 0.f, 0.f, 0.f};

}

static const float* sp_zero_buffer() {
  static const float* cache[64] = {nullptr};
  int dev = 0;
  if (hipGetDevice(&dev) != hipSuccess || dev < 0 || dev >= 64) return nullptr;
  if (cache[dev] == nullptr) {
    void* ptr = nullptr;
    if (hipGetSymbolAddress(&ptr, HIP_SYMBOL(g_sp_zero16)) != hipSuccess) return nullptr;
    cache[dev] = (const float*)ptr;
  }
  return cache[dev];
}

int clx_sp_zero_tail(void* planes, long long rows, int K, int batch, long long bs, hipStream_t st) {
  if (sp::padded_rows(rows) == rows || batch <= 0) return CLX_OK;
  const int ksteps = K / 16;
  const long long total = (sp::padded_rows(rows) / 32 - rows / 32) * ksteps * 6 * 32;
  sp_zero_tail_kernel<<<dim3((unsigned)cdiv(total, 256), (unsigned)batch), 256, 0, st>>>((char*)planes, bs, rows, ksteps);
  return CLX_OK;
}

extern "C" size_t clx_planes_bytes(long long rows, int K) {
  if (rows <= 0 || K <= 0 || K % 16 != 0) return 0;
  return (size_t)sp::planes_bytes(rows, K);
}

int clx_sp_split(const float* x, long long ld, long long rows, int K, void* planes, float* colsum, int nreal, hipStream_t st) {
  CLX_REQUIRE(x != nullptr && planes != nullptr, "clx_split_planes: null pointer");
  CLX_REQUIRE(rows > 0 && K > 0 && K % 16 == 0 && ld >= K && ld % 4 == 0, "clx_split_planes: K must be a multiple of 16, ld >= K a multiple of 4");
  CLX_REQUIRE(((uintptr_t)x & 15) == 0 && ((uintptr_t)planes & 15) == 0, "clx_split_planes: pointers must be 16-byte aligned");
  const int ksteps = K / 16;
  const long long nfrag = sp::padded_rows(rows) / 32 * ksteps;
  long long blocks = (nfrag + 3) / 4;
  if (blocks > 8192) blocks = 8192;
  if (colsum != nullptr) {
    if (blocks > 2048) blocks = 2048;
    int g = ksteps % 4 == 0 ? 4 : ksteps % 2 == 0 ? 2 : 1;
    const long long unit = ksteps / g;
    blocks = (blocks + unit - 1) / unit * unit;
    CLX_LAUNCH_KIND(CLX_PROF_SPLIT_PLANES, sp_split_kernel<true>, dim3((unsigned)blocks), dim3(256), 0, st, x, ld, rows, ksteps, (char*)planes,
                    nfrag, colsum, nreal);
  } else {
    CLX_LAUNCH_KIND(CLX_PROF_SPLIT_PLANES, sp_split_kernel<false>, dim3((unsigned)blocks), dim3(256), 0, st, x, ld, rows, ksteps, (char*)planes,
                    nfrag, (float*)nullptr, 0);
  }
  return CLX_OK;
}

extern "C" int clx_split_planes(const float* x, long long ld, long long rows, int K, void* planes, clx_stream stream) {
  const int rc = clx_sp_split(x, ld, rows, K, planes, nullptr, 0, (hipStream_t)stream);
  if (rc) return rc;
  CLX_CHECK_LAUNCH("clx_split_planes");
  return CLX_OK;
}

extern "C" int clx_join_planes(const void* planes, long long rows, int K, float* x, long long ld, clx_stream stream) {
  CLX_REQUIRE(x != nullptr && planes != nullptr, "clx_join_planes: null pointer");
  CLX_REQUIRE(rows > 0 && K > 0 && K % 16 == 0 && ld >= K, "clx_join_planes: K must be a multiple of 16, ld >= K");
  const long long nfrag = sp::padded_rows(rows) / 32 * (K / 16);
  long long blocks = (nfrag + 3) / 4;
  if (blocks > 8192) blocks = 8192;
  sp_join_kernel<<<dim3((unsigned)blocks), dim3(256), 0, (hipStream_t)stream>>>((const char*)planes, ld, rows, K / 16, x, nfrag);
  CLX_CHECK_LAUNCH("clx_join_planes");
  return CLX_OK;
}

static bool sp_pointwise(const clx_conv_desc* d) {
  if ((d->precision != CLX_PREC_F32X3BF16 && d->precision != CLX_PREC_F32X3BF16_G64) || d->nsrc != 1) return false;
  if (d->KD != 1 || d->KH != 1 || d->KW != 1 || d->PD || d->PH || d->PW) return false;
  const clx_src& S = d->src[0];
  if (S.fz != 1 || S.fy != 1 || S.fx != 1 || S.oz || S.oy || S.ox) return false;
  return S.D == d->ID && S.H == d->IH && S.W == d->IW;
}

bool clx_sp_fwd_rule(const clx_conv_desc* d) {
  if (!sp_pointwise(d)) return false;
  const bool g64 = d->precision == CLX_PREC_F32X3BF16_G64;
  return d->N % (g64 ? 64 : SP_BN) == 0 && d->N >= 128 && d->src[0].C % 64 == 0 && d->src[0].C >= 128 && d->ld_out % 4 == 0;
}

bool clx_sp_wgrad_rule(const clx_conv_desc* d) {
  if (!sp_pointwise(d)) return false;
  const int granule = d->precision == CLX_PREC_F32X3BF16_G64 ? 64 : 128;
  if (d->N % granule != 0 || d->src[0].C % granule != 0 || d->N < 128 || d->src[0].C < 128) return false;
  const long long ch = d->N > d->src[0].C ? d->N : d->src[0].C;
  return (long long)d->B * d->ID * d->IH * d->IW * ch * 6 < (1ll << 32) - (1 << 24);
}

bool clx_sp_applicable(const clx_conv_desc* d) { return d->wplanes != nullptr && clx_sp_fwd_rule(d); }

extern "C" int clx_conv_sp_covers(const clx_conv_desc* d, int pass) {
  if (d == nullptr || (pass != CLX_PASS_FWD && pass != CLX_PASS_WGRAD)) return 0;
  if (d->algo == CLX_ALGO_WINOGRAD || d->algo == CLX_ALGO_WINOGRAD4) return clx_wino_sp(d) ? 1 : 0;
  if (d->algo != CLX_ALGO_DIRECT) return 0;
  return (pass == CLX_PASS_FWD ? clx_sp_fwd_rule(d) : clx_sp_wgrad_rule(d)) ? 1 : 0;
}

int clx_sp_launch(const void* A, const void* B, int M, int N, int K, long long rows_a, int batch, long long bs_a, long long bs_b,
                  long long bs_out, const clx_conv_desc* ep, hipStream_t st) {
  CLX_REQUIRE(M > 0 && N > 0 && N % 64 == 0 && K >= 128 && K % 64 == 0,
              "clx_gemm_planes: needs N %% 64 == 0 (whole 128-wide tiles: N %% 128 == 0), K %% 64 == 0 and K >= 128");
  CLX_REQUIRE(rows_a >= M, "clx_gemm_planes: the A planes hold fewer rows than M");
  SpP p = {};
  p.A = (const char*)A; p.B = (const char*)B;
  p.bs_a = bs_a; p.bs_b = bs_b; p.bs_out = bs_out;
  p.out = ep->out; p.ld_out = ep->ld_out;
  p.M = M; p.N = N; p.ksteps = K / 16;
  p.rb_a = (int)(sp::padded_rows(rows_a) / 32);
  p.rb_b = (int)(sp::padded_rows(N) / 32);
  p.bias = ep->bias; p.mask = ep->mask; p.mask_bits = ep->mask_bits; p.gate_out = ep->gate_out;
  p.relu = ep->relu; p.accumulate = ep->accumulate; p.ld_mask = ep->ld_mask; p.ld_mask_bits = ep->ld_mask_bits; p.ld_gate = ep->ld_gate;
  p.zeros = sp_zero_buffer();
  CLX_REQUIRE(p.zeros != nullptr, "clx_gemm_planes: cannot resolve the device zero buffer");
  p.out_planes = batch == 1 ? (char*)ep->out_planes : nullptr;
  p.colsum = batch == 1 ? ep->out_colsum : nullptr; p.colsum_n = N;
  CLX_REQUIRE(p.out_planes == nullptr || ep->ld_out == N, "clx_gemm_planes: out_planes needs a dense output (ld_out == N)");
  p.nbm = cdiv(M, SP_BM); p.nbn = cdiv(N, SP_BN);
  const char* const tile_env = getenv("CLX_SP_TILE");
  const int tile_choice = tile_env != nullptr ? atoi(tile_env) : 0;
  const char* const maxk_env = getenv("CLX_SP_TILE_MAXK");
  const int maxk = maxk_env != nullptr ? atoi(maxk_env) : 1024;
  const bool small_tiles = tile_choice == 128 || (tile_choice != 256 && K <= maxk);
  const char* const shape_env = getenv("CLX_SP_MFMA");
  const bool mfma16 = shape_env != nullptr && atoi(shape_env) == 16 && N % SP_BN == 0;
  hipEvent_t e0 = nullptr, e1 = nullptr;
  if (clx_prof_enabled())
    clx_prof_events(small_tiles && !mfma16 ? CLX_PROF_GEMM_SP2 : CLX_PROF_GEMM_SP, 2.0 * M * N * K * batch, &e0, &e1);
  if (mfma16) CLX_LAUNCH_TIMED(gemm_sp16_kernel, dim3(p.nbm * p.nbn, batch), dim3(512), st, e0, e1, p);
  else if (small_tiles && N % 128 == 0) CLX_LAUNCH_TIMED(gemm_sp2_kernel<128>, dim3(cdiv(M, S2_BM) * (N / 128), batch), dim3(256), st, e0, e1, p);
  else if (small_tiles) CLX_LAUNCH_TIMED(gemm_sp2_kernel<64>, dim3(cdiv(M, S2_BM) * (N / 64), batch), dim3(256), st, e0, e1, p);
  else CLX_LAUNCH_TIMED(gemm_sp_kernel<0>, dim3(p.nbm * p.nbn, batch), dim3(512), st, e0, e1, p);
  return CLX_OK;
}

int clx_sp_wgrad_launch(const void* dy_planes, const void* x_planes, long long rows, int N, int C, int batch, long long bs_dy,
                        long long bs_x, long long bs_out, float* dw, int ld_dw, hipStream_t st) {
  CLX_REQUIRE(rows > 0 && N > 0 && C >= 128 && N % 64 == 0 && C % 64 == 0,
              "clx_wgrad_planes: needs N %% 64 == 0, C %% 64 == 0 and C >= 128");
  SpP p = {};
  p.A = (const char*)dy_planes; p.B = (const char*)x_planes;
  p.bs_a = bs_dy; p.bs_b = bs_x; p.bs_out = bs_out;
  p.out = dw; p.ld_out = ld_dw;
  p.M = N; p.N = C;
  p.stride_a = (unsigned int)(N / 16) * KSTEP; p.stride_b = (unsigned int)(C / 16) * KSTEP;
  CLX_REQUIRE(sp::planes_bytes(rows, N) < (1ll << 32) && sp::planes_bytes(rows, C) < (1ll << 32), "clx_wgrad_planes: operand planes beyond 4 GB");
  p.total_steps = (int)(sp::padded_rows(rows) / 16);
  p.nbm = cdiv(N, SP_BM); p.nbn = cdiv(C, SP_BN);
  const int tiles = p.nbm * p.nbn * batch;
  int cus = 256, dev = 0;
  if (hipGetDevice(&dev) == hipSuccess) (void)hipDeviceGetAttribute(&cus, hipDeviceAttributeMultiprocessorCount, dev);
  int best_ns = 1;
  double best = 1e30;
  const int max_ns = p.total_steps / 8 > 0 ? p.total_steps / 8 : 1;
  for (int ns = 1; ns <= max_ns && ns <= 4096; ++ns) {
    const int sps = (cdiv(p.total_steps, ns) + 7) / 8 * 8;
    const int real_ns = cdiv(p.total_steps, sps);
    if (p.total_steps - (real_ns - 1) * sps < 8) continue;
    const double cost = (double)cdiv((long long)tiles * real_ns, cus) * (sps + 12);
    if (cost < best) { best = cost; best_ns = ns; }
    if ((long long)tiles * ns > 16ll * cus) break;
  }
  p.steps_per_slice = (cdiv(p.total_steps, best_ns) + 7) / 8 * 8;
  p.nslices = cdiv(p.total_steps, p.steps_per_slice);
  CLX_REQUIRE(p.total_steps >= 8 && p.total_steps - (p.nslices - 1) * p.steps_per_slice >= 8, "clx_wgrad_planes: internal: a slice of fewer than 8 steps");
  hipEvent_t e0 = nullptr, e1 = nullptr;
  if (clx_prof_enabled()) clx_prof_events(CLX_PROF_WGRAD_SP, 2.0 * rows * N * C * batch, &e0, &e1);
  CLX_LAUNCH_TIMED(gemm_sp_kernel<1>, dim3(p.nbm * p.nbn * p.nslices * batch), dim3(512), st, e0, e1, p);
  return CLX_OK;
}

extern "C" int clx_wgrad_planes(const void* dy_planes, const void* x_planes, long long rows, int N, int C, float* dw, int ld_dw,
                                clx_stream stream) {
  CLX_REQUIRE(dy_planes && x_planes && dw && ld_dw >= C, "clx_wgrad_planes: null pointer / ld_dw < C");
  const int rc = clx_sp_wgrad_launch(dy_planes, x_planes, rows, N, C, 1, 0, 0, 0, dw, ld_dw, (hipStream_t)stream);
  if (rc) return rc;
  CLX_CHECK_LAUNCH("clx_wgrad_planes");
  return CLX_OK;
}

extern "C" int clx_gemm_planes(const void* a_planes, const void* b_planes, int M, int N, int K, const float* bias, int relu,
                               float* out, int ld_out, clx_stream stream) {
  CLX_REQUIRE(a_planes && b_planes && out, "clx_gemm_planes: null pointer");
  CLX_REQUIRE(ld_out >= N && ld_out % 4 == 0 && ((uintptr_t)out & 15) == 0, "clx_gemm_planes: out must be 16-byte aligned, ld_out %% 4 == 0");
  clx_conv_desc ep = {};
  ep.out = out; ep.ld_out = ld_out; ep.bias = bias; ep.relu = relu;
  const int rc = clx_sp_launch(a_planes, b_planes, M, N, K, M, 1, 0, 0, 0, &ep, (hipStream_t)stream);
  if (rc) return rc;
  CLX_CHECK_LAUNCH("clx_gemm_planes");
  return CLX_OK;
}
```

### cellulus_amd/csrc/sp_planes.h

```cpp
#pragma once
#include "clx_common.h"

namespace sp {

typedef unsigned int u32x2 __attribute__((ext_vector_type(2)));
typedef unsigned int u32x4 __attribute__((ext_vector_type(4)));

constexpr int FRAG = 1024;
constexpr int KSTEP = 3 * FRAG;

__host__ __device__ inline long long padded_rows(long long rows) { return rows <= 128 ? 128 : (rows + 63) / 64 * 64; }
__host__ __device__ inline long long planes_bytes(long long rows, int K) { return padded_rows(rows) / 32 * (long long)(K / 16) * KSTEP; }

__host__ __device__ inline long long piece_offset(long long row, int octet, int ksteps) {
  return ((row >> 5) * ksteps + (octet >> 1)) * (long long)KSTEP + (octet & 1) * 512 + (row & 31) * 16;
}

__device__ __forceinline__ void split4(const f32x4 v, u32x2& p0, u32x2& p1, u32x2& p2) {
  typedef float f32x2_ __attribute__((ext_vector_type(2)));
  typedef __bf16 bf16x2_ __attribute__((ext_vector_type(2)));
  auto pack = [](float a, float b) -> unsigned int {
    const bf16x2_ h = __builtin_convertvector(f32x2_{a, b}, bf16x2_);
    return __builtin_bit_cast(unsigned int, h);
  };
#pragma unroll
  for (int e = 0; e < 2; ++e) {
    const float x0 = v[2 * e], x1 = v[2 * e + 1];
    const unsigned int w0 = pack(x0, x1);
    const float r0 = x0 - __uint_as_float(w0 << 16), r1 = x1 - __uint_as_float(w0 & 0xffff0000u);
    const unsigned int w1 = pack(r0, r1);
    const float s0 = r0 - __uint_as_float(w1 << 16), s1 = r1 - __uint_as_float(w1 & 0xffff0000u);
    p0[e] = w0;
    p1[e] = w1;
    p2[e] = pack(s0, s1);
  }
}

__device__ __forceinline__ void store4(char* base, long long row, int c, int ksteps, const f32x4 v) {
  u32x2 p0, p1, p2;
  split4(v, p0, p1, p2);
  char* dst = base + piece_offset(row, c >> 3, ksteps) + ((c >> 2) & 1) * 8;
  *reinterpret_cast<u32x2*>(dst) = p0;
  *reinterpret_cast<u32x2*>(dst + FRAG) = p1;
  *reinterpret_cast<u32x2*>(dst + 2 * FRAG) = p2;
}

__device__ __forceinline__ void item_to_row_channel(long long i, int C, long long& row, int& c) {
  const int lane = (int)(i & 63);
  const long long wv = i >> 6;
  const int nblk = C >> 5;
  const int cblk = (int)(wv % nblk);
  row = (wv / nblk) * 8 + (lane >> 3);
  c = cblk * 32 + (lane & 7) * 4;
}

}

int clx_sp_zero_tail(void* planes, long long rows, int K, int batch, long long bs, hipStream_t st);
```

### cellulus_amd/csrc/wino.hip

```cpp
#include "clx_common.h"
#include "sp_planes.h"
#include "wino_tables.h"

namespace {

inline int grid_for(long long total, int block) {
  long long g = (total + block - 1) / block;
  if (g > 16384) g = 16384;
  if (g < 1) g = 1;
  return (int)g;
}

__device__ __forceinline__ f32x4 ld4(const float* p) { return *reinterpret_cast<const f32x4*>(p); }
__device__ __forceinline__ void st4(float* p, f32x4 v) { *reinterpret_cast<f32x4*>(p) = v; }

struct Geom {
  int B, SH, SW, oy, ox;
  int ID, SD, oz;
  int IH, IW, P;
  int OH, OW, th, tw;
  long long T;
};

template <int MT, int R, bool PL = false>
__global__ __launch_bounds__(256) void wino_input_kernel(const float* __restrict__ x, int ld_x, int C4, Geom g,
                                                         float* __restrict__ V, long long total,
                                                         const int* __restrict__ tile_list = nullptr, long long Tc = 0,
                                                         long long plane_bytes = 0) {
  using W = WT<MT, R>;
  constexpr int A = W::A;
  const int C = C4 * 4;
  const long long Trows = tile_list ? Tc : g.T;
  const long long plane = Trows * C;
  for (long long i = (long long)blockIdx.x * blockDim.x + threadIdx.x; i < total;
       i += (long long)gridDim.x * blockDim.x) {
    int c;
    long long t;
    if constexpr (PL) {
      sp::item_to_row_channel(i, C, t, c);
      if (t >= Trows) continue;
    } else {
      c = (int)(i % C4) * 4;
      t = i / C4;
    }
    const long long tg = tile_list ? (long long)tile_list[t] : t;
    const int tx = (int)(tg % g.tw);
    const long long q = tg / g.tw;
    const int ty = (int)(q % g.th);
    const int b = (int)(q / g.th);
    const int bb = b / g.ID, bz = b - bb * g.ID;
    f32x4 d[A][A];
#pragma unroll
    for (int r = 0; r < A; ++r) {
      const int ly = MT * ty - g.P + r;
#pragma unroll
      for (int s = 0; s < A; ++s) {
        const int lx = MT * tx - g.P + s;
        f32x4 v = {0.f, 0.f, 0.f, 0.f};
        if ((unsigned)ly < (unsigned)g.IH && (unsigned)lx < (unsigned)g.IW) {
          const long long pix = (((long long)bb * g.SD + bz + g.oz) * g.SH + ly + g.oy) * g.SW + lx + g.ox;
          v = ld4(x + pix * ld_x + c);
        }
        d[r][s] = v;
      }
    }
    f32x4 w[A][A];
#pragma unroll
    for (int s = 0; s < A; ++s)
#pragma unroll
      for (int r = 0; r < A; ++r) {
        f32x4 acc = {0.f, 0.f, 0.f, 0.f};
        bool first = true;
#pragma unroll
        for (int k = 0; k < A; ++k) axpy(acc, first, W::BT[r][k], d[k][s]);
        w[r][s] = acc;
      }
    float* dst = V + t * C + c;
#pragma unroll
    for (int r = 0; r < A; ++r)
#pragma unroll
      for (int qq = 0; qq < A; ++qq) {
        f32x4 acc = {0.f, 0.f, 0.f, 0.f};
        bool first = true;
#pragma unroll
        for (int k = 0; k < A; ++k) axpy(acc, first, W::BT[qq][k], w[r][k]);
        if constexpr (PL) sp::store4(reinterpret_cast<char*>(V) + (r * A + qq) * plane_bytes, t, c, C >> 4, acc);
        else st4(dst + (r * A + qq) * plane, acc);
      }
  }
}

template <int MT, int R>
__global__ __launch_bounds__(256) void wino_output_kernel(const float* __restrict__ M, int N4, Geom g,
                                                          const float* __restrict__ bias, int relu,
                                                          const float* __restrict__ mask, int ld_mask,
                                                          float* __restrict__ out, int ld_out, int Nreal,
                                                          int accumulate, unsigned int* __restrict__ gate_out,
                                                          int ld_gate, const unsigned int* __restrict__ mask_bits,
                                                          int ld_mask_bits, float* __restrict__ pool_out, int ld_pool,
                                                          long long total, const int* __restrict__ tile_list = nullptr,
                                                          long long Tc = 0) {
  using W = WT<MT, R>;
  constexpr int A = W::A;
  constexpr int MP = MT / 2;
  const int N = N4 * 4;
  const long long plane = (tile_list ? Tc : g.T) * N;
  const int sub = threadIdx.x & 7;
  for (long long i = (long long)blockIdx.x * blockDim.x + threadIdx.x; i < total;
       i += (long long)gridDim.x * blockDim.x) {
    const int n = (int)(i % N4) * 4;
    const long long t = i / N4;
    const long long tg = tile_list ? (long long)tile_list[t] : t;
    const int tx = (int)(tg % g.tw);
    const long long q = tg / g.tw;
    const int ty = (int)(q % g.th);
    const int b = (int)(q / g.th);
    const float* src = M + t * N + n;
    f32x4 rr[MT][A];
#pragma unroll
    for (int s = 0; s < A; ++s) {
      f32x4 m[A];
#pragma unroll
      for (int k = 0; k < A; ++k) m[k] = ld4(src + (k * A + s) * plane);
#pragma unroll
      for (int a = 0; a < MT; ++a) {
        f32x4 acc = {0.f, 0.f, 0.f, 0.f};
        bool first = true;
#pragma unroll
        for (int k = 0; k < A; ++k) axpy(acc, first, W::AT[a][k], m[k]);
        rr[a][s] = acc;
      }
    }
    f32x4 bv = {0.f, 0.f, 0.f, 0.f};
    if (bias) {
#pragma unroll
      for (int e = 0; e < 4; ++e) bv[e] = (n + e < Nreal) ? bias[n + e] : 0.f;
    }
    f32x4 pm[MP][MP];
#pragma unroll
    for (int a = 0; a < MT; ++a) {
      const int oy = MT * ty + a;
      if (oy >= g.OH) continue;
#pragma unroll
      for (int cc = 0; cc < MT; ++cc) {
        const int ox = MT * tx + cc;
        if (ox >= g.OW) continue;
        f32x4 v = {0.f, 0.f, 0.f, 0.f};
        bool first = true;
#pragma unroll
        for (int k = 0; k < A; ++k) axpy(v, first, W::AT[cc][k], rr[a][k]);
        v += bv;
        const long long m = ((long long)b * g.OH + oy) * g.OW + ox;
        if (accumulate) {
          v += ld4(out + m * ld_out + n);
        }
        if (relu) {
#pragma unroll
          for (int e = 0; e < 4; ++e) v[e] = fmaxf(v[e], 0.f);
        }
        if (mask_bits) {
          const unsigned int wbits = mask_bits[m * ld_mask_bits + (n >> 5)] >> (n & 31);
#pragma unroll
          for (int e = 0; e < 4; ++e) v[e] = ((wbits >> e) & 1u) ? v[e] : 0.f;
        }
        if (gate_out) {
          unsigned int nib = 0u;
#pragma unroll
          for (int e = 0; e < 4; ++e) nib |= (n + e < Nreal && v[e] > 0.f) ? (1u << e) : 0u;
          unsigned int word = nib << (4 * sub);
          word |= __shfl_xor(word, 1, 64);
          word |= __shfl_xor(word, 2, 64);
          word |= __shfl_xor(word, 4, 64);
          if (sub == 0) gate_out[m * ld_gate + (n >> 5)] = word;
        }
        if (n + 3 < Nreal) {
          if (mask) {
            const f32x4 mk = ld4(mask + m * ld_mask + n);
#pragma unroll
            for (int e = 0; e < 4; ++e) v[e] = (mk[e] > 0.f) ? v[e] : 0.f;
          }
          st4(out + m * ld_out + n, v);
        } else {
          for (int e = 0; e < 4 && n + e < Nreal; ++e) {
            float xv = v[e];
            if (mask) xv = (mask[m * ld_mask + n + e] > 0.f) ? xv : 0.f;
            out[m * ld_out + n + e] = xv;
          }
        }
        if (pool_out) {
          if ((a & 1) == 0 && (cc & 1) == 0) pm[a >> 1][cc >> 1] = v;
          else {
#pragma unroll
            for (int e = 0; e < 4; ++e) pm[a >> 1][cc >> 1][e] = fmaxf(pm[a >> 1][cc >> 1][e], v[e]);
          }
          if ((a & 1) && (cc & 1)) {
            const long long pm_ = ((long long)b * (g.OH >> 1) + (oy >> 1)) * (g.OW >> 1) + (ox >> 1);
            st4(pool_out + pm_ * ld_pool + n, pm[a >> 1][cc >> 1]);
          }
        }
      }
    }
  }
}

constexpr int ADJ_SEG = 8;

__global__ __launch_bounds__(256) void wino_adjoint_output_kernel(const float* __restrict__ Pm, int C4, int Bn, int th,
                                                                  int tw, int IH, int IW, const float* __restrict__ mask,
                                                                  int ld_mask, const unsigned int* __restrict__ mask_bits,
                                                                  int ld_mask_bits, float* __restrict__ out, int ld_out,
                                                                  int Creal, long long total) {
  using W = WT<4, 3>;
  constexpr int A = 6;
  const int C = C4 * 4;
  const int bh = (IH + 3) / 4, bw = (IW + 3) / 4;
  const int nseg = (bh + ADJ_SEG - 1) / ADJ_SEG;
  const long long plane = (long long)Bn * th * tw * C;
  for (long long i = (long long)blockIdx.x * blockDim.x + threadIdx.x; i < total;
       i += (long long)gridDim.x * blockDim.x) {
    const int c = (int)(i % C4) * 4;
    long long t = i / C4;
    const int bx = (int)(t % bw);
    long long q = t / bw;
    const int sg = (int)(q % nseg);
    const int b = (int)(q / nseg);
    const int by0 = sg * ADJ_SEG, by1 = min(by0 + ADJ_SEG, bh);
    f32x4 carry[2][4];
#pragma unroll
    for (int a = 0; a < 2; ++a)
#pragma unroll
      for (int e = 0; e < 4; ++e) carry[a][e] = f32x4{0.f, 0.f, 0.f, 0.f};
    for (int ty = by0 - 1; ty < by1; ++ty) {
      f32x4 d[A][4];
#pragma unroll
      for (int a = 0; a < A; ++a)
#pragma unroll
        for (int e = 0; e < 4; ++e) d[a][e] = f32x4{0.f, 0.f, 0.f, 0.f};
      if (ty >= 0 && ty < th) {
#pragma unroll
        for (int ux = 0; ux < 2; ++ux) {
          const int tx = bx - ux;
          if (tx < 0 || tx >= tw) continue;
          const float* src = Pm + (((long long)b * th + ty) * tw + tx) * C + c;
#pragma unroll
          for (int s2 = 0; s2 < A; ++s2) {
            f32x4 pcol[A], wcol[A];
#pragma unroll
            for (int r = 0; r < A; ++r) pcol[r] = ld4(src + (r * A + s2) * plane);
#pragma unroll
            for (int a = 0; a < A; ++a) {
              f32x4 v = {0.f, 0.f, 0.f, 0.f};
              bool first = true;
#pragma unroll
              for (int r = 0; r < A; ++r) axpy(v, first, W::BT[r][a], pcol[r]);
              wcol[a] = v;
            }
#pragma unroll
            for (int e = 0; e < 4; ++e) {
              if (ux && e >= 2) continue;
              const float coef = ux ? W::BT[s2][4 + (e & 1)] : W::BT[s2][e];
#pragma unroll
              for (int a = 0; a < A; ++a) {
                bool first = false;
                axpy(d[a][e], first, coef, wcol[a]);
              }
            }
          }
        }
      }
      if (ty >= by0) {
#pragma unroll
        for (int a = 0; a < 4; ++a) {
          const int y = 4 * ty + a;
          if (y >= IH) continue;
#pragma unroll
          for (int e = 0; e < 4; ++e) {
            const int x = 4 * bx + e;
            if (x >= IW) continue;
            f32x4 v = d[a][e];
            if (a < 2) v += carry[a][e];
            const long long m = ((long long)b * IH + y) * IW + x;
            if (mask_bits) {
              const unsigned int wbits = mask_bits[m * ld_mask_bits + (c >> 5)] >> (c & 31);
#pragma unroll
              for (int k = 0; k < 4; ++k) v[k] = ((wbits >> k) & 1u) ? v[k] : 0.f;
            }
            if (c + 3 < Creal) {
              if (mask) {
                const f32x4 mk = ld4(mask + m * ld_mask + c);
#pragma unroll
                for (int k = 0; k < 4; ++k) v[k] = (mk[k] > 0.f) ? v[k] : 0.f;
              }
              st4(out + m * ld_out + c, v);
            } else {
              for (int k = 0; k < 4 && c + k < Creal; ++k) {
                float xv = v[k];
                if (mask) xv = (mask[m * ld_mask + c + k] > 0.f) ? xv : 0.f;
                out[m * ld_out + c + k] = xv;
              }
            }
          }
        }
      }
#pragma unroll
      for (int e = 0; e < 4; ++e) { carry[0][e] = d[4][e]; carry[1][e] = d[5][e]; }
    }
  }
}

template <int MT, int R, bool PL = false>
__global__ __launch_bounds__(256) void wino_dy_kernel(const float* __restrict__ dy, int ld_dy, int N4,
                                                      Geom g, float* __restrict__ Md,
                                                      float* __restrict__ dbias, int Nreal,
                                                      long long total, long long plane_bytes = 0) {
  using W = WT<MT, R>;
  constexpr int A = W::A;
  extern __shared__ float bacc[];
  const int N = N4 * 4;
  const long long plane = g.T * N;
  if (dbias) {
    for (int k = threadIdx.x; k < N; k += blockDim.x) bacc[k] = 0.f;
    __syncthreads();
  }
  for (long long i = (long long)blockIdx.x * blockDim.x + threadIdx.x; i < total;
       i += (long long)gridDim.x * blockDim.x) {
    int n;
    long long t;
    if constexpr (PL) {
      sp::item_to_row_channel(i, N, t, n);
      if (t >= g.T) continue;
    } else {
      n = (int)(i % N4) * 4;
      t = i / N4;
    }
    const int tx = (int)(t % g.tw);
    const long long q = t / g.tw;
    const int ty = (int)(q % g.th);
    const int b = (int)(q / g.th);
    f32x4 d[MT][MT];
    f32x4 sum = {0.f, 0.f, 0.f, 0.f};
#pragma unroll
    for (int a = 0; a < MT; ++a)
#pragma unroll
      for (int c = 0; c < MT; ++c) {
        const int oy = MT * ty + a, ox = MT * tx + c;
        f32x4 v = {0.f, 0.f, 0.f, 0.f};
        if (oy < g.OH && ox < g.OW) v = ld4(dy + (((long long)b * g.OH + oy) * g.OW + ox) * ld_dy + n);
        d[a][c] = v;
        sum += v;
      }
    if (dbias) {
#pragma unroll
      for (int e = 0; e < 4; ++e) atomicAdd(&bacc[n + e], sum[e]);
    }
    f32x4 w[A][MT];
#pragma unroll
    for (int c = 0; c < MT; ++c)
#pragma unroll
      for (int r = 0; r < A; ++r) {
        f32x4 acc = {0.f, 0.f, 0.f, 0.f};
        bool first = true;
#pragma unroll
        for (int a = 0; a < MT; ++a) axpy(acc, first, W::AT[a][r], d[a][c]);
        w[r][c] = acc;
      }
    float* dst = Md + t * N + n;
#pragma unroll
    for (int r = 0; r < A; ++r)
#pragma unroll
      for (int qq = 0; qq < A; ++qq) {
        f32x4 acc = {0.f, 0.f, 0.f, 0.f};
        bool first = true;
#pragma unroll
        for (int c = 0; c < MT; ++c) axpy(acc, first, W::AT[c][qq], w[r][c]);
        if constexpr (PL) sp::store4(reinterpret_cast<char*>(Md) + (r * A + qq) * plane_bytes, t, n, N >> 4, acc);
        else st4(dst + (r * A + qq) * plane, acc);
      }
  }
  if (dbias) {
    __syncthreads();
    for (int k = threadIdx.x; k < Nreal; k += blockDim.x)
      if (bacc[k] != 0.f) atomicAdd(dbias + k, bacc[k]);
  }
}

template <int MT, int R, bool PL = false>
__global__ __launch_bounds__(256) void wino_dy_dual_kernel(const float* __restrict__ dy, int ld_dy, int N4,
                                                           Geom gd, Geom gw, float* __restrict__ Vd,
                                                           float* __restrict__ Md, float* __restrict__ dbias,
                                                           int Nreal, long long total, long long pb_d = 0, long long pb_w = 0) {
  using W = WT<MT, R>;
  constexpr int A = W::A;
  constexpr int P = R - 1;
  extern __shared__ float bacc[];
  const int N = N4 * 4;
  const long long plane_d = gd.T * N, plane_w = gw.T * N;
  if (dbias) {
    for (int k = threadIdx.x; k < N; k += blockDim.x) bacc[k] = 0.f;
    __syncthreads();
  }
  for (long long i = (long long)blockIdx.x * blockDim.x + threadIdx.x; i < total;
       i += (long long)gridDim.x * blockDim.x) {
    int n;
    long long t;
    if constexpr (PL) {
      sp::item_to_row_channel(i, N, t, n);
      if (t >= gd.T) continue;
    } else {
      n = (int)(i % N4) * 4;
      t = i / N4;
    }
    const int tx = (int)(t % gd.tw);
    const long long q = t / gd.tw;
    const int ty = (int)(q % gd.th);
    const int b = (int)(q / gd.th);
    if (ty < gw.th && tx < gw.tw) {
      f32x4 dd[MT][MT];
      f32x4 sum = {0.f, 0.f, 0.f, 0.f};
#pragma unroll
      for (int a = 0; a < MT; ++a)
#pragma unroll
        for (int c = 0; c < MT; ++c) {
          const int oy = MT * ty + a, ox = MT * tx + c;
          f32x4 v = {0.f, 0.f, 0.f, 0.f};
          if (oy < gd.IH && ox < gd.IW) v = ld4(dy + (((long long)b * gd.IH + oy) * gd.IW + ox) * ld_dy + n);
          dd[a][c] = v;
          sum += v;
        }
      if (dbias) {
#pragma unroll
        for (int e = 0; e < 4; ++e) atomicAdd(&bacc[n + e], sum[e]);
      }
      f32x4 w[A][MT];
#pragma unroll
      for (int c = 0; c < MT; ++c)
#pragma unroll
        for (int r = 0; r < A; ++r) {
          f32x4 acc = {0.f, 0.f, 0.f, 0.f};
          bool first = true;
#pragma unroll
          for (int a = 0; a < MT; ++a) axpy(acc, first, W::AT[a][r], dd[a][c]);
          w[r][c] = acc;
        }
      const long long tw_lin = ((long long)b * gw.th + ty) * gw.tw + tx;
      float* dst = Md + tw_lin * N + n;
#pragma unroll
      for (int r = 0; r < A; ++r)
#pragma unroll
        for (int qq = 0; qq < A; ++qq) {
          f32x4 acc = {0.f, 0.f, 0.f, 0.f};
          bool first = true;
#pragma unroll
          for (int c = 0; c < MT; ++c) axpy(acc, first, W::AT[c][qq], w[r][c]);
          if constexpr (PL) sp::store4(reinterpret_cast<char*>(Md) + (r * A + qq) * pb_w, tw_lin, n, N >> 4, acc);
          else st4(dst + (r * A + qq) * plane_w, acc);
        }
    }
    f32x4 d[A][A];
// ... 139 lines not shown
  const long long plane = (long long)kdt * rows * cin_pad;
  for (long long i = (long long)blockIdx.x * blockDim.x + threadIdx.x; i < total;
       i += (long long)gridDim.x * blockDim.x) {
    const int dz = (int)(i % kdt);
    const long long q = i / kdt;
    const int c = (int)(q % cin), n = (int)(q / cin);
    const float* src = dU + ((long long)dz * rows + n) * cin_pad + c;
    double t[R][A];
#pragma unroll
    for (int s2 = 0; s2 < A; ++s2) {
      double u[A];
#pragma unroll
      for (int r = 0; r < A; ++r) u[r] = (double)src[(r * A + s2) * plane];
#pragma unroll
      for (int k = 0; k < R; ++k) {
        double acc = 0.0;
#pragma unroll
        for (int r = 0; r < A; ++r) acc += W::G[r][k] * u[r];
        t[k][s2] = acc;
      }
    }
    float* dst = dw + i * (R * R);
#pragma unroll
    for (int k = 0; k < R; ++k)
#pragma unroll
      for (int l = 0; l < R; ++l) {
        double acc = 0.0;
#pragma unroll
        for (int s2 = 0; s2 < A; ++s2) acc += t[k][s2] * W::G[s2][l];
        dst[k * R + l] = (float)acc;
      }
  }
}

bool applicable(const clx_conv_desc* d) {
  if (d->nsrc != 1 || d->KH != d->KW) return false;
  if (d->KD == 1) {
    if (d->ID != 1 || d->PD != 0) return false;
  } else {
    if (d->KD != d->KH || d->algo != CLX_ALGO_WINOGRAD4 || d->PD != d->PH) return false;
  }
  if (d->KH != 3 && !(d->KH == 2 && d->algo == CLX_ALGO_WINOGRAD4)) return false;
  if (d->PH != d->PW || (d->PH != 0 && d->PH != d->KH - 1)) return false;
  const clx_src& S = d->src[0];
  if (S.fz != 1 || S.fy != 1 || S.fx != 1) return false;
  if (d->KD == 1 && (S.D != 1 || S.oz != 0)) return false;
  if (S.C % 4 != 0 || d->N <= 0) return false;
  return true;
}

inline int tile_of(const clx_conv_desc* d) { return d->algo == CLX_ALGO_WINOGRAD4 ? 4 : 2; }

Geom geom(const clx_conv_desc* d, int mt, int planes) {
  Geom g;
  const clx_src& S = d->src[0];
  g.B = d->B * planes; g.SH = S.H; g.SW = S.W; g.oy = S.oy; g.ox = S.ox;
  g.ID = planes; g.SD = S.D; g.oz = S.oz;
  g.IH = d->IH; g.IW = d->IW; g.P = d->PH;
  g.OH = d->IH + 2 * d->PH - (d->KH - 1); g.OW = d->IW + 2 * d->PW - (d->KW - 1);
  g.th = (g.OH + mt - 1) / mt; g.tw = (g.OW + mt - 1) / mt;
  g.T = (long long)g.B * g.th * g.tw;
  return g;
}
inline int out_planes(const clx_conv_desc* d) { return d->ID + 2 * d->PD - (d->KD - 1); }

inline int pad4(int n) { return (n + 3) / 4 * 4; }

inline bool wino_sp(const clx_conv_desc* d) {
  if (d->KD != 1 || d->ID != 1) return false;
  if (d->precision == CLX_PREC_F32X3BF16_G64) {
    if (d->N % 64 != 0 || d->src[0].C % 64 != 0 || d->N < 128 || d->src[0].C < 128) return false;
  } else if (d->precision != CLX_PREC_F32X3BF16 || d->N % 128 != 0 || d->src[0].C % 128 != 0) {
    return false;
  }
  const int mt = d->algo == CLX_ALGO_WINOGRAD ? 2 : 4;
  const long long eh = d->IH + (d->PH ? d->KH - 1 : 0), ew = d->IW + (d->PW ? d->KW - 1 : 0);
  const long long tiles = (long long)d->B * ((eh + mt - 1) / mt) * ((ew + mt - 1) / mt);
  const int ch = d->N > d->src[0].C ? d->N : d->src[0].C;
  return sp::planes_bytes(tiles, ch) < (1ll << 32);
}
inline long long sp_items(long long rows, int C) { return (rows + 7) / 8 * 8 * (C / 4); }

clx_conv_desc gemm_desc(float* V, int C, const clx_conv_desc* d, const Geom& gin) {
  clx_conv_desc gd = {};
  gd.nsrc = 1;
  gd.src[0].ptr = V; gd.src[0].C = C; gd.src[0].ld = C;
  gd.src[0].D = d->ID; gd.src[0].H = 1; gd.src[0].W = gin.th * gin.tw;
  gd.src[0].fz = gd.src[0].fy = gd.src[0].fx = 1;
  gd.B = d->B; gd.ID = d->ID; gd.IH = 1; gd.IW = gin.th * gin.tw;
  gd.KD = d->KD; gd.KH = gd.KW = 1;
  gd.PD = d->PD;
  return gd;
}

template <int MT, int R>
int wino_fwd_t(const clx_conv_desc* d, hipStream_t st) {
  constexpr int AA = WT<MT, R>::A * WT<MT, R>::A;
  const Geom gin = geom(d, MT, d->ID), gout = geom(d, MT, out_planes(d));
  const clx_src& S = d->src[0];
  const int C = S.C, Np = pad4(d->N);
  const bool spx = wino_sp(d);
  CLX_REQUIRE(!spx || d->wplanes != nullptr, "clx_conv_fwd(winograd): precision f32x3bf16 needs wplanes (the planes of wpack)");
  float* V = d->vcache ? (float*)d->vcache : (float*)d->workspace;
  const int* list = d->tile_list;
  if (list != nullptr) {
    CLX_REQUIRE(d->KD == 1 && d->ID == 1 && d->PH == 0 && d->vcache == nullptr && !d->accumulate && d->tile_count >= 0 &&
                    d->tile_count <= gin.T && gin.T == gout.T,
                "clx_conv_fwd(winograd): tile_list needs a 2-D valid convolution without vcache / accumulate and at most "
                "th * tw * B tiles");
    if (d->tile_count == 0) return CLX_OK;
  }
  const long long Tin = list ? d->tile_count : gin.T, Tout = list ? d->tile_count : gout.T;
  const long long pbV = spx ? sp::planes_bytes(Tin, C) : 0;
  float* M = spx ? (float*)((char*)d->workspace + AA * sp::planes_bytes(gin.T, C)) : (float*)d->workspace + AA * Tin * C;
  if (!(d->vcache && d->vcache_valid)) {
    if (spx) {
      const long long tot_in = sp_items(Tin, C);
      int rc = clx_sp_zero_tail(V, Tin, C, AA, pbV, st);
      if (rc) return rc;
      CLX_LAUNCH_KIND(CLX_PROF_WINO_TRANSFORM, (wino_input_kernel<MT, R, true>), dim3(grid_for(tot_in, 256)), dim3(256), 0, st, S.ptr, S.ld, C / 4,
                      gin, V, tot_in, list, Tin, pbV);
    } else {
      const long long tot_in = Tin * (C / 4);
      CLX_LAUNCH_KIND(CLX_PROF_WINO_TRANSFORM, (wino_input_kernel<MT, R>), dim3(grid_for(tot_in, 256)), dim3(256), 0, st, S.ptr, S.ld, C / 4, gin, V,
                      tot_in, list, Tin, 0ll);
    }
  }
  if (spx) {
    clx_conv_desc ep = {};
    ep.out = M; ep.ld_out = Np;
    const int rc = clx_sp_launch(V, d->wplanes, (int)Tin, d->N, C, Tin, AA, pbV, sp::planes_bytes(Np, C), Tout * Np, &ep, st);
    if (rc) return rc;
  } else {
    clx_conv_desc gd = gemm_desc(V, C, d, gin);
    if (list) {
      gd.B = 1;
      gd.src[0].W = gd.IW = (int)Tin;
    }
    gd.N = d->N; gd.wpack = d->wpack; gd.out = M; gd.ld_out = Np;
    const int rc = clx_igemm_launch(&gd, AA, Tin * C, (long long)Np * d->KD * C, Tout * Np, st);
    if (rc) return rc;
  }
  const long long tot_out = Tout * (Np / 4);
  CLX_REQUIRE((d->gate_out == nullptr && d->mask_bits == nullptr) || Np % 32 == 0,
              "clx_conv_fwd(winograd): gate_out / mask_bits need a channel count that is a multiple of 32");
  CLX_REQUIRE(d->gate_out == nullptr || d->relu, "clx_conv_fwd(winograd): gate_out needs relu");
  if (d->pool_out != nullptr) {
    CLX_REQUIRE(d->KD == 1 && d->ID == 1 && gout.OH % 2 == 0 && gout.OW % 2 == 0,
                "clx_conv_fwd(winograd): pool_out needs a 2-D layer with even output height and width");
    CLX_REQUIRE(d->N % 4 == 0 && d->ld_pool % 4 == 0 && d->ld_pool >= d->N && ((uintptr_t)d->pool_out & 15) == 0 &&
                    d->mask == nullptr && d->mask_bits == nullptr && !d->accumulate,
                "clx_conv_fwd(winograd): pool_out needs N %% 4 == 0, an aligned ld_pool >= N, and no mask / accumulate");
  }
  CLX_LAUNCH_KIND(CLX_PROF_WINO_TRANSFORM, (wino_output_kernel<MT, R>), dim3(grid_for(tot_out, 256)), dim3(256), 0, st, M, Np / 4, gout, d->bias,
                  d->relu, d->mask, d->ld_mask, d->out, d->ld_out, d->N, d->accumulate, d->gate_out, d->ld_gate, d->mask_bits,
                  d->ld_mask_bits, d->pool_out, d->ld_pool, tot_out, list, Tout);
  CLX_CHECK_LAUNCH("clx_conv_fwd(winograd)");
  return CLX_OK;
}

template <int MT, int R>
int wino_wgrad_t(const clx_conv_desc* d, const float* dy, int ld_dy, float* dwpack, float* dbias, hipStream_t st) {
  constexpr int AA = WT<MT, R>::A * WT<MT, R>::A;
  const Geom gin = geom(d, MT, d->ID), gout = geom(d, MT, out_planes(d));
  const clx_src& S = d->src[0];
  const int C = S.C, N = d->N;
  const bool spx = wino_sp(d);
  float* V = d->vcache ? (float*)d->vcache : (float*)d->workspace;
  const long long pbV = spx ? sp::planes_bytes(gin.T, C) : 0, pbM = spx ? sp::planes_bytes(gout.T, N) : 0;
  float* Md = spx ? (float*)((char*)d->workspace + AA * pbV) : (float*)d->workspace + AA * gin.T * C;
  if (!(d->vcache && d->vcache_valid)) {
    if (spx) {
      const long long tot_in = sp_items(gin.T, C);
      int rc = clx_sp_zero_tail(V, gin.T, C, AA, pbV, st);
      if (rc) return rc;
      CLX_LAUNCH_KIND(CLX_PROF_WINO_TRANSFORM, (wino_input_kernel<MT, R, true>), dim3(grid_for(tot_in, 256)), dim3(256), 0, st, S.ptr, S.ld, C / 4,
                      gin, V, tot_in, (const int*)nullptr, 0ll, pbV);
    } else {
      const long long tot_in = gin.T * (C / 4);
      CLX_LAUNCH_KIND(CLX_PROF_WINO_TRANSFORM, (wino_input_kernel<MT, R>), dim3(grid_for(tot_in, 256)), dim3(256), 0, st, S.ptr, S.ld, C / 4, gin, V,
                      tot_in, (const int*)nullptr, 0ll, 0ll);
    }
  }
  if (spx) {
    const int rc = clx_sp_zero_tail(Md, gout.T, N, AA, pbM, st);
    if (rc) return rc;
  }
  if (d->dy_vcache) {
    Geom gd = gout;
    gd.SH = gout.OH; gd.SW = gout.OW; gd.oy = gd.ox = 0;
    gd.ID = gd.SD = out_planes(d); gd.oz = 0;
    gd.IH = gout.OH; gd.IW = gout.OW; gd.P = R - 1;
    gd.OH = gout.OH + R - 1; gd.OW = gout.OW + R - 1;
    gd.th = (gd.OH + MT - 1) / MT; gd.tw = (gd.OW + MT - 1) / MT;
    gd.T = (long long)gd.B * gd.th * gd.tw;
    const long long tot = spx ? sp_items(gd.T, N) : gd.T * (N / 4);
    int blocks = grid_for(tot, 256);
    if (dbias && blocks > 2048) blocks = 2048;
    if (spx) {
      const long long pbD = sp::planes_bytes(gd.T, N);
      const int rc = clx_sp_zero_tail(d->dy_vcache, gd.T, N, AA, pbD, st);
      if (rc) return rc;
      CLX_LAUNCH_KIND(CLX_PROF_WINO_TRANSFORM, (wino_dy_dual_kernel<MT, R, true>), dim3(blocks), dim3(256), (size_t)N * sizeof(float), st, dy, ld_dy,
                      N / 4, gd, gout, (float*)d->dy_vcache, Md, dbias, N, tot, pbD, pbM);
    } else {
      CLX_LAUNCH_KIND(CLX_PROF_WINO_TRANSFORM, (wino_dy_dual_kernel<MT, R>), dim3(blocks), dim3(256), (size_t)N * sizeof(float), st, dy, ld_dy, N / 4,
                      gd, gout, (float*)d->dy_vcache, Md, dbias, N, tot, 0ll, 0ll);
    }
  } else {
    const long long tot_dy = spx ? sp_items(gout.T, N) : gout.T * (N / 4);
    int blocks = grid_for(tot_dy, 256);
    if (blocks > 2048) blocks = 2048;
    if (spx)
      CLX_LAUNCH_KIND(CLX_PROF_WINO_TRANSFORM, (wino_dy_kernel<MT, R, true>), dim3(blocks), dim3(256), (size_t)N * sizeof(float), st, dy, ld_dy, N / 4,
                      gout, Md, dbias, N, tot_dy, pbM);
    else
      CLX_LAUNCH_KIND(CLX_PROF_WINO_TRANSFORM, (wino_dy_kernel<MT, R>), dim3(blocks), dim3(256), (size_t)N * sizeof(float), st, dy, ld_dy, N / 4, gout,
                      Md, dbias, N, tot_dy, 0ll);
  }
  if (spx) {
    CLX_REQUIRE(gin.T == gout.T, "clx_conv_wgrad(winograd): tile counts of input and output differ");
    CLX_REQUIRE(d->det_turns == nullptr, "clx_conv_wgrad: the reproducible mode exists for the float32 precision only");
    const int rc = clx_sp_wgrad_launch(Md, V, gin.T, N, C, AA, pbM, pbV, (long long)N * C, dwpack, C, st);
    if (rc) return rc;
    CLX_CHECK_LAUNCH("clx_conv_wgrad(winograd, split precision)");
    return CLX_OK;
  }
  clx_conv_desc gd = gemm_desc(V, C, d, gin);
  gd.N = N;
  gd.det_turns = d->det_turns;
  const int rc = clx_wgrad_launch(&gd, Md, N, dwpack, nullptr, AA, gin.T * C, gout.T * N,
                                  (long long)d->KD * N * C, st);
  if (rc) return rc;
  CLX_CHECK_LAUNCH("clx_conv_wgrad(winograd)");
  return CLX_OK;
}

}

bool clx_wino_sp(const clx_conv_desc* d) { return wino_sp(d); }

extern "C" size_t clx_conv_workspace_bytes(const clx_conv_desc* d, int pass) {
  if (d == nullptr || !applicable(d)) return 0;
  if (pass == CLX_PASS_WGRAD && d->PH != 0) return 0;
  const int mt = tile_of(d), a = mt + d->KH - 1;
  const Geom gin = geom(d, mt, d->ID), gout = geom(d, mt, out_planes(d));
  if (gout.OH <= 0 || gout.OW <= 0 || out_planes(d) <= 0 || gin.T >= (1ll << 31) || gout.T >= (1ll << 31)) return 0;
  const long long C = d->src[0].C, N = pad4(d->N);
  if (wino_sp(d)) {
    const long long v = sp::planes_bytes(gin.T, (int)C);
    const long long m = pass == CLX_PASS_WGRAD ? sp::planes_bytes(gout.T, (int)N) : gout.T * N * (long long)sizeof(float);
    return (size_t)(a * a * (v + m));
  }
  return (size_t)(a * a * (gin.T * C + gout.T * N)) * sizeof(float);
}

extern "C" size_t clx_conv_vcache_bytes(const clx_conv_desc* d, int which) {
  if (d == nullptr || !applicable(d)) return 0;
  const int mt = tile_of(d), a = mt + d->KH - 1, R = d->KH;
  const Geom gin = geom(d, mt, d->ID), gout = geom(d, mt, out_planes(d));
  const long long C = d->src[0].C, N = pad4(d->N);
  if (which == 0) return wino_sp(d) ? (size_t)(a * a * sp::planes_bytes(gin.T, (int)C)) : (size_t)(a * a * gin.T * C) * sizeof(float);
  const long long th = (gout.OH + R - 1 + mt - 1) / mt, tw = (gout.OW + R - 1 + mt - 1) / mt;
  const long long Td = (long long)gout.B * th * tw;
  return wino_sp(d) ? (size_t)(a * a * sp::planes_bytes(Td, (int)N)) : (size_t)(a * a * Td * N) * sizeof(float);
}

static int wino_adjoint(const clx_conv_desc* d, hipStream_t st) {
  CLX_REQUIRE(d->algo == CLX_ALGO_WINOGRAD4 && d->KH == 3 && d->KW == 3 && d->PH == 2 && d->PW == 2 && d->nsrc == 1 &&
                  ((d->KD == 1 && d->ID == 1 && d->PD == 0) || (d->KD == 3 && d->PD == 2)),
              "clx_conv_fwd(adjoint): a 3x3 (2-D) or 3x3x3 layer in its data-gradient form (padding 2) with "
              "CLX_ALGO_WINOGRAD4 only");
  CLX_REQUIRE(d->bias == nullptr && !d->relu && !d->accumulate && d->gate_out == nullptr,
              "clx_conv_fwd(adjoint): only the ReLU-gate epilogues (mask / mask_bits) exist");
  CLX_REQUIRE(d->N % 4 == 0 && d->src[0].C % 4 == 0, "clx_conv_fwd(adjoint): channel counts must be multiples of 4");
  const int OHf = d->IH, OWf = d->IW;
  const int th = (OHf + 3) / 4, tw = (OWf + 3) / 4;
  const int planes_dy = d->ID, planes_dx = d->ID + 2 * d->PD - (d->KD - 1);
  const long long Tdy = (long long)d->B * planes_dy * th * tw, Tdx = (long long)d->B * planes_dx * th * tw;
  const int Nf = d->src[0].C, Cp = d->N;
  const bool spx = wino_sp(d);
  const size_t need = spx ? (size_t)36 * (sp::planes_bytes(Tdx, Cp) + sp::planes_bytes(Tdy, Nf))
                          : (size_t)36 * (Tdx * Cp + Tdy * Nf) * sizeof(float);
  CLX_REQUIRE(d->workspace != nullptr && d->workspace_bytes >= need && ((uintptr_t)d->workspace & 15) == 0,
              "clx_conv_fwd(adjoint): needs the %zu workspace bytes of the layer's weight gradient (%zu given)", need,
              d->workspace_bytes);
  CLX_REQUIRE(d->mask_bits == nullptr || Cp % 32 == 0, "clx_conv_fwd(adjoint): mask_bits needs whole words per pixel");
  float* P = (float*)d->workspace;
  float* Mdy = P + (size_t)36 * Tdx * Cp;
  if (spx) {
    CLX_REQUIRE(d->wplanes != nullptr, "clx_conv_fwd(adjoint): precision f32x3bf16 needs wplanes");
    const char* Mp = (const char*)d->workspace + 36 * sp::planes_bytes(Tdx, Cp);
    clx_conv_desc ep = {};
    ep.out = P; ep.ld_out = Cp;
    const int rc = clx_sp_launch(Mp, d->wplanes, (int)Tdy, Cp, Nf, Tdy, 36, sp::planes_bytes(Tdy, Nf), sp::planes_bytes(Cp, Nf),
                                 Tdx * Cp, &ep, st);
    if (rc) return rc;
  } else {
  clx_conv_desc gd = {};
  gd.nsrc = 1;
  gd.src[0].ptr = Mdy; gd.src[0].C = Nf; gd.src[0].ld = Nf;
  gd.src[0].D = planes_dy; gd.src[0].H = 1; gd.src[0].W = th * tw;
  gd.src[0].fz = gd.src[0].fy = gd.src[0].fx = 1;
  gd.B = d->B; gd.ID = planes_dy; gd.IH = 1; gd.IW = th * tw;
  gd.KD = d->KD; gd.KH = gd.KW = 1; gd.PD = d->PD;
  gd.N = Cp; gd.wpack = d->wpack; gd.out = P; gd.ld_out = Cp;
  const int rc = clx_igemm_launch(&gd, 36, Tdy * Nf, (long long)Cp * d->KD * Nf, Tdx * Cp, st);
  if (rc) return rc;
  }
  const int IH = OHf + 2, IW = OWf + 2;
  const int nseg = ((IH + 3) / 4 + ADJ_SEG - 1) / ADJ_SEG;
  const long long total = (long long)d->B * planes_dx * nseg * ((IW + 3) / 4) * (Cp / 4);
  CLX_LAUNCH_KIND(CLX_PROF_WINO_TRANSFORM, wino_adjoint_output_kernel, dim3(grid_for(total, 256)), dim3(256), 0, st, P, Cp / 4,
                  d->B * planes_dx, th, tw, IH, IW, d->mask, d->ld_mask, d->mask_bits, d->ld_mask_bits, d->out, d->ld_out, Cp, total);
  CLX_CHECK_LAUNCH("clx_conv_fwd(winograd adjoint)");
  return CLX_OK;
}

int clx_wino_fwd(const clx_conv_desc* d, hipStream_t st) {
  if (d->adjoint) return wino_adjoint(d, st);
  CLX_REQUIRE(applicable(d), "clx_conv_fwd: Winograd does not apply to this geometry");
  const size_t need = clx_conv_workspace_bytes(d, CLX_PASS_FWD);
  CLX_REQUIRE(d->workspace != nullptr && d->workspace_bytes >= need && need > 0,
              "clx_conv_fwd: Winograd needs %zu workspace bytes (%zu given)", need, d->workspace_bytes);
  CLX_REQUIRE(((uintptr_t)d->workspace & 15) == 0 && ((uintptr_t)d->vcache & 15) == 0,
              "clx_conv_fwd: workspace / vcache must be 16-byte aligned");
  if (d->KH == 2) return wino_fwd_t<4, 2>(d, st);
  return tile_of(d) == 4 ? wino_fwd_t<4, 3>(d, st) : wino_fwd_t<2, 3>(d, st);
}

int clx_wino_wgrad(const clx_conv_desc* d, const float* dy, int ld_dy, float* dwpack, float* dbias,
                   hipStream_t st) {
  CLX_REQUIRE(applicable(d) && d->PH == 0, "clx_conv_wgrad: Winograd does not apply to this geometry");
  const size_t need = clx_conv_workspace_bytes(d, CLX_PASS_WGRAD);
  CLX_REQUIRE(d->workspace != nullptr && d->workspace_bytes >= need && need > 0,
              "clx_conv_wgrad: Winograd needs %zu workspace bytes (%zu given)", need, d->workspace_bytes);
  CLX_REQUIRE(((uintptr_t)d->workspace & 15) == 0 && ((uintptr_t)d->vcache & 15) == 0,
              "clx_conv_wgrad: workspace / vcache must be 16-byte aligned");
  CLX_REQUIRE(d->N <= 8192, "clx_conv_wgrad: too many output channels for the Winograd bias accumulator");
  if (d->KH == 2) return wino_wgrad_t<4, 2>(d, dy, ld_dy, dwpack, dbias, st);
  return tile_of(d) == 4 ? wino_wgrad_t<4, 3>(d, dy, ld_dy, dwpack, dbias, st)
                         : wino_wgrad_t<2, 3>(d, dy, ld_dy, dwpack, dbias, st);
}

int clx_wino_pack(const float* w, float* wp, int cout, int cin, int cin_pad, int cout_pad, int dgrad,
                  int tile, int ksize, int kd, hipStream_t st) {
  const bool fused = dgrad == 3;
  if (fused) dgrad = 0;
  const int rows = dgrad ? cin_pad : cout_pad, cols = dgrad ? cout_pad : cin_pad;
  const long long total = (long long)rows * kd * cols;
  const int grid = grid_for(total, 256);
  if (ksize == 2) wino_filter_kernel<4, 2><<<grid, 256, 0, st>>>(w, wp, cout, cin, rows, cols, kd, dgrad, total, fused);
  else if (tile == 4) wino_filter_kernel<4, 3><<<grid, 256, 0, st>>>(w, wp, cout, cin, rows, cols, kd, dgrad, total, fused);
  else wino_filter_kernel<2, 3><<<grid, 256, 0, st>>>(w, wp, cout, cin, rows, cols, kd, dgrad, total, fused);
  return CLX_OK;
}

extern "C" int clx_pack_weights_batch(const clx_pack_job* jobs, int njobs, long long max_total, clx_stream stream) {
  CLX_REQUIRE(jobs != nullptr && njobs > 0 && njobs < 65536 && max_total > 0, "clx_pack_weights_batch: bad arguments");
  CLX_REQUIRE(((uintptr_t)jobs & 7) == 0, "clx_pack_weights_batch: the job table must be 8-byte aligned");
  long long gx = (max_total + 255) / 256;
  if (gx > 512) gx = 512;
  pack_batch_kernel<<<dim3((unsigned)gx, (unsigned)njobs), 256, 0, (hipStream_t)stream>>>(jobs);
  CLX_CHECK_LAUNCH("clx_pack_weights_batch");
  return CLX_OK;
}

extern "C" int clx_unpack_wgrad_wino(const float* du, float* dw, int cout, int cin, int rows,
                                     int cin_pad, int tile, int ksize, int kd, clx_stream stream) {
  CLX_REQUIRE(du && dw, "clx_unpack_wgrad_wino: null pointer");
  CLX_REQUIRE(cout > 0 && cin > 0 && rows >= cout && cin_pad >= cin, "clx_unpack_wgrad_wino: bad extents");
  CLX_REQUIRE((ksize == 3 && (tile == 2 || tile == 4)) || (ksize == 2 && tile == 4),
              "clx_unpack_wgrad_wino: (tile, ksize) must be (2, 3), (4, 3) or (4, 2)");
  CLX_REQUIRE(kd == 1 || (kd == ksize && tile == 4), "clx_unpack_wgrad_wino: kd must be 1 or ksize (F(4x4) only)");
  const long long total = (long long)cout * cin * kd;
  const int grid = grid_for(total, 256);
  hipStream_t st = (hipStream_t)stream;
  if (ksize == 2) wino_unpack_kernel<4, 2><<<grid, 256, 0, st>>>(du, dw, cout, cin, rows, cin_pad, kd, total);
  else if (tile == 4) wino_unpack_kernel<4, 3><<<grid, 256, 0, st>>>(du, dw, cout, cin, rows, cin_pad, kd, total);
  else wino_unpack_kernel<2, 3><<<grid, 256, 0, st>>>(du, dw, cout, cin, rows, cin_pad, kd, total);
  CLX_CHECK_LAUNCH("clx_unpack_wgrad_wino");
  return CLX_OK;
}
```

### cellulus_amd/models/plan.py

```python

import ctypes
import math
import os
from dataclasses import dataclass, field
from typing import List, Tuple

import torch

from .. import _clx
from .._clx import ClxConvDesc, ClxSrc


def pad4(c: int) -> int:
    return (c + 3) // 4 * 4


WINO_MIN_CHANNELS = int(os.environ.get("CLX_WINOGRAD_MIN_CHANNELS", "64"))
WINO_TAPS = {1: 16, 2: 36, 3: 36}
WINO_PACK_FWD = {1: 2, 2: 4, 3: 7}
WINO_PACK_DGRAD = {1: 3, 2: 5}
WINO_TILE = {1: 2, 2: 4, 3: 4}


WINO_MIN_CHANNELS_3D = int(os.environ.get("CLX_WINOGRAD_MIN_CHANNELS_3D", "64"))
# ... 1085 lines not shown
                                          5 if sp["wino"] else 1))
                    continue
                gapped = len(layer.sources) > 1 and not all(s.channels % 4 == 0 for s in layer.sources[:-1])
                if gapped or not w.is_contiguous():
                    singles.append(layer)
                    continue
                algo = self.algo[layer.name]
                biggest = max(biggest, job(w, self.wpack_fwd[layer.name], layer.cout, layer.cin, layer.taps,
                                           layer.cin_pad, pad4(layer.cout), WINO_PACK_FWD.get(algo["fwd"], 0)))
                if need_dgrad and layer.name in self.wpack_dgrad:
                    biggest = max(biggest, job(w, self.wpack_dgrad[layer.name], layer.cout, layer.cin, layer.taps,
                                               layer.cin_pad, pad4(layer.cout),
                                               6 if layer.name in self.adjoint else WINO_PACK_DGRAD.get(algo["dgrad"], 1)))
            table = None
            if jobs:
                arr = (ClxPackJob * len(jobs))(*jobs)
                host = torch.frombuffer(bytearray(bytes(arr)), dtype=torch.uint8)
                table = host.to(self.device)
            cache = self._pack_table = dict(sig=sig, table=table, njobs=len(jobs), biggest=int(biggest), singles=singles)
        for layer in self.topo.convs:
            if layer.name in self.subpixel:
                sp = self.subpixel[layer.name]
                wv = params[2 * layer.param_index].detach()
                if not wv.is_contiguous():
                    wv = wv.contiguous()
                _clx.call("clx_subpixel_split_weights", _clx.ptr(wv), _clx.ptr(sp["w_skip"]), _clx.ptr(sp["weff"]),
                          layer.cout, layer.cin, sp["C0"], sp["N"], *layer.kernel, *sp["fac"], st)
        if cache["table"] is not None:
            _clx.call("clx_pack_weights_batch", _clx.ptr(cache["table"]), cache["njobs"], cache["biggest"], st)
        for layer in cache["singles"]:
            self._pack_layer(layer, params[2 * layer.param_index], need_dgrad, st)
        self._split_wplanes(need_dgrad, st)

    def pack_weights(self, params, version, need_dgrad):
        if need_dgrad and not self._bwd_ready:
            self._alloc_backward()
        key = (version, need_dgrad)
        if self._packed_version is not None and self._packed_version[0] == version and \
                (self._packed_version[1] or not need_dgrad):
            return
        st = _clx.stream_ptr(self.device)
        if os.environ.get("CLX_PACK_BATCH", "1") != "0":
            self._pack_batched(params, need_dgrad, st)
            self._packed_version = key
            return
        for layer in self.topo.convs:
            w = params[2 * layer.param_index]
            if layer.name in self.subpixel:
                self._sp_pack(layer, self.subpixel[layer.name], w, need_dgrad, st)
                continue
            self._pack_layer(layer, w, need_dgrad, st)
        self._split_wplanes(need_dgrad, st)
        self._packed_version = key

    def pointwise_prefix(self):
        ops = self.topo.fwd_order
        if not ops or not isinstance(ops[0], ConvLayer):
            return None
        special = lambda op: op.name in self.chains or op.name in self.chain_second or op.name in self.subpixel
        first = ops[0]
        if special(first) or len(first.sources) != 1 or first.sources[0].tensor != "raw":
            return None
        readers = tensor_consumers(self.topo)
        tail, src = [], first.out
        for op in ops[1:]:
            if not isinstance(op, ConvLayer) or op.taps != 1 or special(op) or self.algo[op.name]["fwd"]:
                break
            s = op.sources[0]
            if len(op.sources) != 1 or s.tensor != src or tuple(s.crop) != (0, 0, 0) or tuple(s.factor) != (1, 1, 1):
                break
            if readers.get(src, 0) != 1:
                break
            tail.append(op)
            src = op.out
        return (first, tail) if tail else None

    def first_layer_on_rows(self):
        prefix = self.pointwise_prefix()
        if prefix is None or os.environ.get("CLX_SPARSE_FIRST", "1") == "0":
            return False
        first = prefix[0]
        return (self.topo.in_channels == 1 and tuple(first.kernel) in ((1, 3, 3), (3, 3, 3)) and first.cout % 4 == 0
                and first.in_shape[0] >= first.kernel[0])

    def tiled_layer_behind_prefix(self):
        prefix = self.pointwise_prefix()
        if prefix is None:
            return None
        first, tail = prefix
        ops = self.topo.fwd_order
        k = 1 + len(tail)
        if k >= len(ops) or not isinstance(ops[k], ConvLayer):
            return None
        op = ops[k]
        code = self.algo[op.name]["fwd"]
        if (not code or op.kernel[0] != 1 or op.in_shape[0] != 1 or op.name in self.subpixel or op.name in self.chains
                or op.name in self.chain_second or len(op.sources) != 1):
            return None
        s = op.sources[0]
        if s.tensor != tail[-1].out or tuple(s.crop) != (0, 0, 0) or tuple(s.factor) != (1, 1, 1):
            return None
        return op, WINO_TILE[code]

    def _compact(self, slot, rows, width):
        bufs = self.__dict__.setdefault("_compact_bufs", {})
        b = bufs.get(slot)
        if b is None or b.shape[0] < rows or b.shape[1] != width:
            b = bufs[slot] = _clx.zeros((max(rows, 1), width), torch.float32, self.device)
        return b

    def forward_prefix(self, raw, params, nlayers):
        t = self.topo
        st = _clx.stream_ptr(self.device)
        npix_in = t.in_shape[0] * t.in_shape[1] * t.in_shape[2]
        raw = raw.contiguous()
        _clx.call("clx_planar_to_pixel", _clx.ptr(raw), _clx.ptr(self.buf["raw"]), self.B,
                  t.in_channels, npix_in, pad4(t.in_channels), st)
        for op in t.fwd_order[:1 + nlayers]:
            self._conv_forward(op, params, st)
        return self.buf[t.fwd_order[nlayers].out]

    def _conv_forward(self, op, params, st, tiles=None):
        d = self._desc(op)
        d.N = op.cout
        self._set_wpack(d, self.wpack_fwd[op.name])
        b = params[2 * op.param_index + 1]
        d.bias = b.data_ptr() if b is not None else None
        d.relu = 1 if op.relu else 0
        d.mask = None
        d.ld_mask = 0
        d.out = self.buf[op.out].data_ptr()
        d.ld_out = pad4(op.cout)
        if op.relu and self.keep:
            self._set_gate_out(d, op.out)
        if self.sp_pass[op.name][0] and not self.algo[op.name]["fwd"]:
            xp = self.xplanes.get(op.name) if self.keep and self._bwd_ready and tiles is None else None
            d.aplanes = (xp if xp is not None else self.aplanes).data_ptr()
            if xp is not None:
                d.aplanes_valid = 1 if op.name in self._xplanes_fresh else 0
                self._xplanes_fresh.add(op.name)
                nxt = self._pointwise_reader.get(op.out)
                if nxt is not None and os.environ.get("CLX_SP_EPILOGUE_PLANES", "1") != "0":
                    d.out_planes = self.xplanes[nxt.name].data_ptr()
                    self._xplanes_fresh.add(nxt.name)
        if self.algo[op.name]["fwd"]:
            self._use_workspace(d, self.algo[op.name]["fwd"])
            if self.keep and self._bwd_ready and op.name in self.vcache:
                d.vcache = self.vcache[op.name].data_ptr()
                self._vcache_fresh.add(op.name)
            pool = self.fused_pool.get(op.name)
            if pool is not None:
                d.pool_out = self.buf[pool.out].data_ptr()
                d.ld_pool = pad4(pool.channels)
        if tiles is not None:
            d.tile_list = tiles[0].data_ptr()
            d.tile_count = int(tiles[1])
        _clx.call("clx_conv_fwd", ctypes.byref(d), st)

    def _tiles_forward(self, op, params, sparse, st):
        dense = self.buf[op.out]
        clean = sparse["clean_tile_rows"]
        assert clean.shape[1] == dense.shape[1] and clean.shape[0] * self.B == dense.shape[0]
        _clx.call("clx_broadcast_rows", _clx.ptr(clean), clean.numel(), _clx.ptr(dense), self.B, st)
        pool = self.fused_pool.get(op.name)
        if pool is not None:
            pooled, clean_pooled = self.buf[pool.out], sparse["clean_pool_rows"]
            assert clean_pooled.shape[0] * self.B == pooled.shape[0]
            _clx.call("clx_broadcast_rows", _clx.ptr(clean_pooled), clean_pooled.numel(), _clx.ptr(pooled), self.B, st)
        if int(sparse["ntiles"]) > 0:
            self._conv_forward(op, params, st, tiles=(sparse["tiles"], sparse["ntiles"]))

    def _pointwise_on_rows(self, tail, params, sparse, st):
        n, rows = int(sparse["n"]), sparse["rows"]
        src = self.buf[tail[0].sources[0].tensor]
        width = src.shape[1]
        cur = None
        if n > 0:
            cur = self._compact(0, n, width)
            if sparse.get("noisy") is not None:
                first = self.topo.fwd_order[0]
                b = params[2 * first.param_index + 1]
                _clx.call("clx_grey_rows", _clx.ptr(sparse["noisy"]), self.B, *first.in_shape, first.kernel[0],
                          _clx.ptr(rows), n, _clx.ptr(self.wpack_fwd[first.name]), _clx.ptr(b) if b is not None else None,
                          1 if first.relu else 0, first.cout, _clx.ptr(cur), width, st)
            else:
                _clx.call("clx_gather_rows", _clx.ptr(src), width, _clx.ptr(rows), n, width, _clx.ptr(cur), width, st)
            for k, op in enumerate(tail):
                y = self._compact(1 + k % 2, n, pad4(op.cout))
                d = ClxConvDesc()
                d.nsrc = 1
                src_d = ClxSrc()
                src_d.ptr = cur.data_ptr()
                src_d.C = src_d.ld = cur.shape[1]
                src_d.D, src_d.H, src_d.W = 1, 1, n
                src_d.oz = src_d.oy = src_d.ox = 0
                src_d.fz = src_d.fy = src_d.fx = 1
                d.src[0] = src_d
                d.B = 1
                d.ID, d.IH, d.IW = 1, 1, n
                d.KD = d.KH = d.KW = 1
                d.PD = d.PH = d.PW = 0
                d.N = op.cout
                self._set_wpack(d, self.wpack_fwd[op.name])
                d.precision = self.precision
                if self.precision and self.aplanes is not None:
                    d.aplanes = self.aplanes.data_ptr()
                b = params[2 * op.param_index + 1]
                d.bias = b.data_ptr() if b is not None else None
                d.relu = 1 if op.relu else 0
                d.out = y.data_ptr()
                d.ld_out = y.shape[1]
                _clx.call("clx_conv_fwd", ctypes.byref(d), st)
                cur = y
        dense = self.buf[tail[-1].out]
        clean = sparse["clean_rows"]
        assert clean.shape[1] == dense.shape[1] and clean.shape[0] * self.B == dense.shape[0]
        _clx.call("clx_broadcast_rows", _clx.ptr(clean), clean.numel(), _clx.ptr(dense), self.B, st)
        if n > 0:
            _clx.call("clx_scatter_rows", _clx.ptr(cur), cur.shape[1], _clx.ptr(rows), n, dense.shape[1],
                      _clx.ptr(dense), dense.shape[1], st)

    def forward(self, raw, params, out=None, on_op=None, sparse=None):
        t = self.topo
        st = _clx.stream_ptr(self.device)
        sparse_tail = self.pointwise_prefix()[1] if sparse is not None else None
        self._vcache_fresh = set()
        self._xplanes_fresh = set()
        npix_in = t.in_shape[0] * t.in_shape[1] * t.in_shape[2]
        raw = raw.contiguous()
        rows_only_first = sparse is not None and self.first_layer_on_rows()
        if rows_only_first:
            sparse = dict(sparse, noisy=raw)
        else:
            _clx.call("clx_planar_to_pixel", _clx.ptr(raw), _clx.ptr(self.buf["raw"]), self.B,
                      t.in_channels, npix_in, pad4(t.in_channels), st)
        for op_index, op in enumerate(t.fwd_order):
            if on_op is not None and op_index > 0:
                on_op(op_index - 1)
            if op_index == 0 and rows_only_first:
                continue
            if isinstance(op, ConvLayer) and op.name in self.chain_second:
                continue
            if isinstance(op, ConvLayer) and op.name in self.chains:
                self._chain_forward(*self.chains[op.name], params, st)
            elif isinstance(op, ConvLayer) and op.name in self.subpixel:
                self._sp_forward(op, self.subpixel[op.name], params[2 * op.param_index + 1], st)
            elif isinstance(op, ConvLayer) and sparse_tail and op is sparse_tail[0]:
                self._pointwise_on_rows(sparse_tail, params, sparse, st)
            elif isinstance(op, ConvLayer) and sparse_tail and any(op is q for q in sparse_tail):
                continue
            elif isinstance(op, ConvLayer) and sparse is not None and sparse.get("tiles") is not None \
                    and op is sparse["tile_op"]:
                self._tiles_forward(op, params, sparse, st)
            elif isinstance(op, ConvLayer):
                self._conv_forward(op, params, st)
            elif any(p is op for p in self.fused_pool.values()):
                continue
            else:
                D, H, W = op.in_shape
                _clx.call("clx_maxpool_fwd", _clx.ptr(self.buf[op.src]), _clx.ptr(self.buf[op.out]),
                          self.B, D, H, W, pad4(op.channels), *op.factor, st)
        npix_out = t.out_shape[0] * t.out_shape[1] * t.out_shape[2]
        spatial = t.out_shape[3 - t.nd:]
        if out is None:
            out = torch.empty((self.B, t.out_channels) + tuple(spatial), dtype=torch.float32, device=self.device)
        assert out.is_contiguous() and tuple(out.shape) == (self.B, t.out_channels) + tuple(spatial)
        _clx.call("clx_pixel_to_planar", _clx.ptr(self.buf["h1"]), _clx.ptr(out), self.B,
                  t.out_channels, npix_out, pad4(t.out_channels), st)
        return out

    def backward(self, dout, params, grads, on_layer_done=None, flat_grad=None, dx=None):
        st = _clx.stream_ptr(self.device)
        self.zero_gradients(grads, flat_grad)
        for done, unpack in self.backward_steps(dout, params, grads, dx=dx):
            unpack(st)
            if on_layer_done is not None:
                for i in done:
                    on_layer_done(i)

    def train_pass(self, raw, params, grads, flat_grad, loss_fn, after_loss=None, on_layer_done=None):
        out = self.forward(raw, params)
        dout = loss_fn(out, 0, self.B)
        if after_loss is not None:
            after_loss()
        self.backward(dout, params, grads, on_layer_done=on_layer_done, flat_grad=flat_grad)
        return out

    def zero_gradients(self, grads, flat_grad=None):
        if flat_grad is not None:
            _clx.zero_many(self.dwpack, flat_grad)
        else:
            _clx.zero_many(self.dwpack)
            for g in grads[1::2]:
                if g is not None:
                    g.zero_()

    def first_dgrad(self, layer, dy, w, dx, st):
        assert dx.is_contiguous() and dx.dtype == torch.float32 and dx.shape[0] == self.B
        wv = w.detach()
        if not wv.is_contiguous():
            wv = wv.contiguous()
        OD, OH, OW = layer.out_shape
        if _first_dgrad_kernel_wanted(layer):
            _clx.call("clx_conv_first_dgrad", _clx.ptr(dy), dy.shape[1], _clx.ptr(wv), layer.cout, layer.cin, self.B,
                      OD, OH, OW, layer.kernel[0], _clx.ptr(dx), st)
            return
        if not self.dx_bufs:
            n = self.B * layer.in_shape[0] * layer.in_shape[1] * layer.in_shape[2]
            self.dx_bufs["wpack"] = torch.empty(layer.cin_pad * layer.taps * pad4(layer.cout), dtype=torch.float32,
                                                device=self.device)
            self.dx_bufs["pixels"] = torch.empty((n, layer.cin_pad), dtype=torch.float32, device=self.device)
        wp, px = self.dx_bufs["wpack"], self.dx_bufs["pixels"]
        _clx.call("clx_pack_weights", _clx.ptr(wv), _clx.ptr(wp), layer.cout, layer.cin, layer.taps, layer.cin_pad,
                  pad4(layer.cout), 1, st)
        dd = self._dgrad_desc(layer, dy)
        dd.wpack = wp.data_ptr()
        dd.mask = None
        dd.ld_mask = 0
        dd.out = px.data_ptr()
        dd.ld_out = layer.cin_pad
        _clx.call("clx_conv_fwd", ctypes.byref(dd), st)
        _clx.call("clx_pixel_to_planar", _clx.ptr(px), _clx.ptr(dx), self.B, layer.cin,
                  layer.in_shape[0] * layer.in_shape[1] * layer.in_shape[2], layer.cin_pad, st)

    def backward_steps(self, dout, params, grads, dx=None):
        t = self.topo
        st = _clx.stream_ptr(self.device)
        assert self._bwd_ready, "pack_weights(need_dgrad=True) must run before backward"
        npix_out = t.out_shape[0] * t.out_shape[1] * t.out_shape[2]
        dout = dout.contiguous()
        _clx.call("clx_planar_to_pixel", _clx.ptr(dout), _clx.ptr(self.gbuf["h1"]), self.B,
                  t.out_channels, npix_out, pad4(t.out_channels), st)

        by_out = {layer.out: layer for layer in t.convs}
        pool_by_out = {p.out: p for p in t.pools}
        r_by_conv0 = {info["conv0"].name: info for info in t.r_info}
        pending_skip = {}
        dy_planes_of = {}

        for op in reversed(t.fwd_order):
            if isinstance(op, PoolOp):
                continue
            layer = op
            dy = self.gbuf[layer.out]
            if layer.name in self.chains:
                continue
            if layer.name in self.chain_second:
                a, b = self.chain_second[layer.name]
                yield (b.param_index, a.param_index), self._chain_backward(a, b, by_out[a.sources[0].tensor], grads, st)
                continue
            if layer.name in self.subpixel:
                sp = self.subpixel[layer.name]
                yield (layer.param_index,), self._sp_wgrad(layer, sp, dy, grads[2 * layer.param_index],
                                                           grads[2 * layer.param_index + 1], st)
                dskip = self._sp_dgrad(layer, sp, dy, st)
                pending_skip[layer.sources[0].tensor] = (dskip, sp["C0p"], layer)
                continue
            d = self._desc(layer)
            d.N = pad4(layer.cout)
            gb = grads[2 * layer.param_index + 1]
            off = self.dw_off[layer.name]
            wino_w = self.algo[layer.name]["wgrad"]
            wtaps = wino_taps(wino_w, layer.kernel) if wino_w else layer.taps
            dwp = self.dwpack[off:off + wtaps * pad4(layer.cout) * layer.cin_pad]
            adjoint = layer.name in self.adjoint
            dual = (self.dycache is not None and wino_w and layer.param_index > 0
                    and self.algo[layer.name]["dgrad"] == wino_w and not adjoint)
            if wino_w:
                self._use_workspace(d, wino_w)
                if layer.name in self.vcache and layer.name in self._vcache_fresh:
                    d.vcache = self.vcache[layer.name].data_ptr()
                    d.vcache_valid = 1
                if dual:
                    d.dy_vcache = self.dycache.data_ptr()
            dy_planes = dy_planes_of.pop(layer.out, None)
            dy_ready = dy_planes is not None
            if dy_planes is None and self.dyplanes is not None:
                dy_planes = self.dyplanes
            if self.sp_pass[layer.name][2] and not wino_w:
                d.aplanes = self.xplanes[layer.name].data_ptr()
                d.aplanes_valid = 1 if layer.name in self._xplanes_fresh else 0
                d.dyplanes = dy_planes.data_ptr()
                d.dyplanes_valid = 1 if dy_ready else 0
                if dy_ready:
                    gb = None
                dy_ready = True
            elif dy_ready:
                raise AssertionError("planes of dY were written for a layer whose weight gradient does not read them")
            self._wgrad(d, dy, pad4(layer.cout), dwp, gb, layer.cout, st)
            yield (layer.param_index,), self._unpack_step(layer, dwp, grads[2 * layer.param_index], wino_w)
            if layer.param_index == 0:
                if dx is not None:
                    self.first_dgrad(layer, dy, params[0], dx, st)
                continue
            dd = self._dgrad_desc(layer, dy)
            self._set_wpack(dd, self.wpack_dgrad[layer.name])
            dgrad_sp = self.sp_pass[layer.name][1] and not self.algo[layer.name]["dgrad"]
            if dgrad_sp:
                dd.aplanes = dy_planes.data_ptr()
                dd.aplanes_valid = 1 if dy_ready else 0
            if self.algo[layer.name]["dgrad"]:
                self._use_workspace(dd, self.algo[layer.name]["dgrad"])
                if adjoint:
                    dd.adjoint = 1
                elif dual:
                    dd.vcache = self.dycache.data_ptr()
                    dd.vcache_valid = 1
            if len(layer.sources) == 2:
                info = r_by_conv0[layer.name]
                cat = self.gbuf["cat%d" % info["level"]]
                dd.mask = None
                dd.ld_mask = 0
                dd.out = cat.data_ptr()
                dd.ld_out = layer.cin_pad
                _clx.call("clx_conv_fwd", ctypes.byref(dd), st)
                skip_s, up_s = layer.sources
                ushape, uc = t.shapes[up_s.tensor]
                LD, LH, LW = layer.in_shape
                _clx.call("clx_upsample_bwd", _clx.ptr(cat), layer.cin_pad, pad4(skip_s.channels),
                          LD, LH, LW, *up_s.crop, _clx.ptr(self.buf[up_s.tensor]),
                          _clx.ptr(self.gbuf[up_s.tensor]), self.B, ushape[0], ushape[1], ushape[2],
                          pad4(uc), *up_s.factor, st)
                pending_skip[skip_s.tensor] = (cat, layer.cin_pad, layer)
            else:
                s = layer.sources[0]
                if s.tensor in pool_by_out:
                    pool = pool_by_out[s.tensor]
                    dd.mask = None
                    dd.ld_mask = 0
                    dd.out = self.gbuf[pool.out].data_ptr()
                    dd.ld_out = pad4(pool.channels)
                    _clx.call("clx_conv_fwd", ctypes.byref(dd), st)
                    cat, ld_cat, rl = pending_skip.pop(pool.src)
                    skip_s = rl.sources[0]
                    D, H, W = pool.in_shape
                    SD, SH, SW = rl.in_shape
                    _clx.call("clx_maxpool_bwd", _clx.ptr(self.buf[pool.src]), _clx.ptr(self.buf[pool.out]),
                              _clx.ptr(self.gbuf[pool.out]), _clx.ptr(cat), ld_cat, SD, SH, SW,
                              *skip_s.crop, _clx.ptr(self.gbuf[pool.src]), self.B, D, H, W,
                              pad4(pool.channels), *pool.factor, st)
                else:
                    prev = by_out[s.tensor]
                    self._set_mask(dd, prev.out, relu=prev.relu)
                    dd.out = self.gbuf[prev.out].data_ptr()
                    dd.ld_out = pad4(prev.cout)
                    if (dgrad_sp and prev.name in self.xplanes and self.sp_pass[prev.name][2]
                            and os.environ.get("CLX_SP_EPILOGUE_PLANES", "1") != "0"):
                        other = self.dyplanes2 if dy_planes is self.dyplanes else self.dyplanes
                        dd.out_planes = other.data_ptr()
                        gbp = grads[2 * prev.param_index + 1]
                        dd.out_colsum = gbp.data_ptr() if gbp is not None else None
                        dy_planes_of[prev.out] = other
                    _clx.call("clx_conv_fwd", ctypes.byref(dd), st)
        assert not pending_skip


def _first_dgrad_kernel_wanted(layer):
    return layer.cin <= 4 and os.environ.get("CLX_FIRST_DGRAD", "1") != "0"


def forward_flops(topo, batch):
    total = 0
    for layer in topo.convs:
        m = batch * layer.out_shape[0] * layer.out_shape[1] * layer.out_shape[2]
        total += 2 * m * layer.cout * layer.cin * layer.taps
    return total


class _Rows:

    def __init__(self, parts, attr):
        self._parts, self._attr = parts, attr

    def __getitem__(self, name):
        return torch.cat([getattr(p, self._attr)[name] for p in self._parts], dim=0)

    def __contains__(self, name):
        return name in getattr(self._parts[0], self._attr)

    def __bool__(self):
        return bool(getattr(self._parts[0], self._attr))

    def get(self, name, default=None):
        return self[name] if name in self else default

    def keys(self):
        return getattr(self._parts[0], self._attr).keys()


def dual_stream_wanted(topo, batch, keep_activations):
    if not keep_activations or batch < 2 or batch % 2 or os.environ.get("CLX_STREAMS", "2") == "1":
        return False
    if os.environ.get("CLX_DETERMINISTIC", "0") == "1":
        return False
    return forward_flops(topo, batch // 2) >= float(os.environ.get("CLX_STREAMS_MIN_GFLOP", "100")) * 1e9


class DualPlan:

    def __init__(self, topo, batch, device, keep_activations):
        assert batch % 2 == 0 and keep_activations
        self.topo, self.B, self.device, self.keep = topo, int(batch), device, True
        self.parts = [UNetPlan(topo, batch // 2, device, True) for _ in range(2)]
        self.streams = [torch.cuda.Stream(device=device) for _ in range(2)]
        self._events = [[], [], []]
        self._shared = False
        self.buf = _Rows(self.parts, "buf")

    def __getattr__(self, name):
        if name in ("parts", "streams"):
            raise AttributeError(name)
        if name == "gbuf":
            return _Rows(self.parts, "gbuf")
        return getattr(self.parts[0], name)

    def pack_weights(self, params, version, need_dgrad):
        a, b = self.parts
        a.pack_weights(params, version, need_dgrad)
        if need_dgrad and not self._shared:
            b._alloc_backward()
            b.share_from(a)
            self._shared = True
        b._packed_version = a._packed_version

    def _fork(self):
        main = torch.cuda.current_stream(self.device)
        for s in self.streams:
            s.wait_stream(main)
        return main

    def _join(self, main):
        for s in self.streams:
            main.wait_stream(s)

    def forward(self, raw, params, out=None):
        t = self.topo
        assert self._shared, "pack_weights(need_dgrad=True) must run before forward"
        raw = raw.contiguous()
        if out is None:
            out = torch.empty((self.B, t.out_channels) + tuple(t.out_shape[3 - t.nd:]), dtype=torch.float32,
                              device=self.device)
        h = self.B // 2
        main = self._fork()
        for i, (p, s) in enumerate(zip(self.parts, self.streams)):
            with torch.cuda.stream(s):
                p.forward(raw[i * h:(i + 1) * h], params, out=out[i * h:(i + 1) * h])
        self._join(main)
        return out

    def _event(self, i, k):
        ev = self._events[i]
        while len(ev) <= k:
            ev.append(torch.cuda.Event())
        return ev[k]

    def backward(self, dout, params, grads, on_layer_done=None, flat_grad=None, dx=None):
        dout = dout.contiguous()
        h = self.B // 2
        self.parts[0].zero_gradients(grads, flat_grad)
        main = self._fork()
        dxs = [dx[:h], dx[h:]] if dx is not None else [None, None]
        self._backward_halves([dout[:h], dout[h:]], params, grads, on_layer_done, main, dxs=dxs)
        self._join(main)

    def train_pass(self, raw, params, grads, flat_grad, loss_fn, after_loss=None, on_layer_done=None):
        t = self.topo
        assert self._shared, "pack_weights(need_dgrad=True) must run before train_pass"
        raw = raw.contiguous()
        out = torch.empty((self.B, t.out_channels) + tuple(t.out_shape[3 - t.nd:]), dtype=torch.float32,
                          device=self.device)
        h = self.B // 2
        main = self._fork()
        douts = []
        for i, (p, s) in enumerate(zip(self.parts, self.streams)):
            with torch.cuda.stream(s):
                o = p.forward(raw[i * h:(i + 1) * h], params, out=out[i * h:(i + 1) * h])
                douts.append(loss_fn(o, i * h, (i + 1) * h))
                self._event(i, 0).record(s)
        self.parts[0].zero_gradients(grads, flat_grad)
        zeroed = self._event(2, 0)
        zeroed.record(main)
        for i, s in enumerate(self.streams):
            main.wait_event(self._event(i, 0))
            s.wait_event(zeroed)
        if after_loss is not None:
            after_loss()
        self._backward_halves(douts, params, grads, on_layer_done, main)
        self._join(main)
        return out

    def _backward_halves(self, douts, params, grads, on_layer_done, main, dxs=(None, None)):
        st_main = _clx.stream_ptr(self.device)
        gens = []
        for p, s, d, dx in zip(self.parts, self.streams, douts, dxs):
            with torch.cuda.stream(s):
                gens.append(p.backward_steps(d, params, grads, dx=dx))
        k = 1
        while True:
            items = []
            for i, (g, s) in enumerate(zip(gens, self.streams)):
                with torch.cuda.stream(s):
                    item = next(g, None)
                    if item is not None:
                        self._event(i, k).record(s)
                items.append(item)
# ... 13 lines not shown
```

### include/clx.h

```cpp
#ifndef CLX_H
#define CLX_H

#include <stddef.h>
#include <stdint.h>

#ifdef __cplusplus
extern "C" {
#endif

typedef void* clx_stream;

enum clx_status {
  CLX_OK = 0,
  CLX_ERR_ARG = -1,
  CLX_ERR_LAUNCH = -2,
  CLX_ERR_WORKSPACE = -3
};

const char* clx_last_error(void);
int clx_abi_version(void);
int clx_device_count(void);

enum clx_profile_kind {
  CLX_PROF_IGEMM_WIDE = 0,
  CLX_PROF_IGEMM_NARROW = 1,
  CLX_PROF_WGRAD = 2,
  CLX_PROF_GEMM_SP = 3,
  CLX_PROF_WGRAD_SP = 4,
  CLX_PROF_SPLIT_PLANES = 5,
  CLX_PROF_CHAIN64 = 6,
  CLX_PROF_MS_PREPARE = 7,
  CLX_PROF_MS_ASSIGN = 8,
  CLX_PROF_CC = 9,
  CLX_PROF_GROW_SHRINK = 10,
  CLX_PROF_MINMAX = 11,
  CLX_PROF_HISTOGRAM = 12,
  CLX_PROF_NOISE_STATS = 13,
  CLX_PROF_WINO_FUSED = 14,
  CLX_PROF_WINO_TRANSFORM = 15,
  CLX_PROF_GEMM_SP2 = 16
};
int clx_profile_enable(int on);
int clx_profile_read(int kind, double* launches, double* total_ms, double* total_flops);
int clx_profile_clock(double* shader_ticks, double* wall_ticks_100mhz, int reset);


typedef struct clx_src {
  const float* ptr;
  int C;
  int ld;
  int D, H, W;
  int oz, oy, ox;
  int fz, fy, fx;
} clx_src;

typedef struct clx_conv_desc {
  int nsrc;
  clx_src src[2];
  int B;
  int ID, IH, IW;
  int KD, KH, KW;
  int PD, PH, PW;
  int N;
  const float* wpack;
  const float* bias;
  int relu;
  const float* mask;
  int ld_mask;
  float* out;
  int ld_out;
  int accumulate;
  int algo;
  void* workspace;
  size_t workspace_bytes;
  void* vcache;
  int vcache_valid;
  int c_real;
  void* dy_vcache;
  unsigned int* gate_out;
  int ld_gate;
  const unsigned int* mask_bits;
  int ld_mask_bits;
  int* det_turns;
  int adjoint;
  float* pool_out;
  int ld_pool;
  const int* tile_list;
  int tile_count;
  int precision;
  const void* wplanes;
  void* aplanes;
  int aplanes_valid;
  void* dyplanes;
  int dyplanes_valid;
  void* out_planes;
  float* out_colsum;
} clx_conv_desc;

enum clx_conv_precision { CLX_PREC_F32 = 0, CLX_PREC_F32X3BF16 = 1, CLX_PREC_F32X3BF16_G64 = 2 };

enum clx_conv_algo {
  CLX_ALGO_DIRECT = 0,
  CLX_ALGO_WINOGRAD = 1,
  CLX_ALGO_WINOGRAD4 = 2,
  CLX_ALGO_WINOGRAD4_FUSED = 3
};
int clx_conv_fused_applicable(const clx_conv_desc* d);
size_t clx_conv_fused_workspace_bytes(const clx_conv_desc* d);
enum clx_conv_pass { CLX_PASS_FWD = 0, CLX_PASS_WGRAD = 1 };
size_t clx_conv_workspace_bytes(const clx_conv_desc* d, int pass);
size_t clx_conv_vcache_bytes(const clx_conv_desc* d, int which);

size_t clx_planes_bytes(long long rows, int K);
int clx_split_planes(const float* x, long long ld, long long rows, int K, void* planes, clx_stream stream);
int clx_join_planes(const void* planes, long long rows, int K, float* x, long long ld, clx_stream stream);
int clx_gemm_planes(const void* a_planes, const void* b_planes, int M, int N, int K, const float* bias, int relu,
                    float* out, int ld_out, clx_stream stream);
int clx_wgrad_planes(const void* dy_planes, const void* x_planes, long long rows, int N, int C, float* dw, int ld_dw,
                     clx_stream stream);

int clx_conv_sp_covers(const clx_conv_desc* d, int pass);

int clx_conv_fwd(const clx_conv_desc* d, clx_stream stream);

size_t clx_conv_wgrad_turns_bytes(const clx_conv_desc* d);
size_t clx_colsum_scratch_bytes(int N);
int clx_colsum_ordered(const float* x, int ld, long long M, int N, float* out, void* scratch, clx_stream stream);

int clx_chain64_fwd(const float* x, int ld_x, long long M, const float* w1, const float* b1, float* y1,
                    int ld_y1, unsigned int* gate1, int ld_gate1, const float* w2, const float* b2, int N2,
                    int relu2, float* y2, int ld_y2, unsigned int* gate2, int ld_gate2, clx_stream stream);
int clx_chain64_bwd(const float* dp2, int ld_dp2, int N2, const float* y1, int ld_y1, const float* x,
                    int ld_x, int gate_x, long long M, const float* w2t, const float* w1t, float* dp0,
                    int ld_dp0, float* dw2, float* db2, float* dw1, float* db1, clx_stream stream);

int clx_conv_wgrad(const clx_conv_desc* d, const float* dy, int ld_dy,
                   float* dwpack, float* dbias, clx_stream stream);

enum clx_pack_mode {
  CLX_PACK_FWD = 0,
  CLX_PACK_DGRAD = 1,
  CLX_PACK_WINO_FWD = 2,
  CLX_PACK_WINO_DGRAD = 3,
  CLX_PACK_WINO4_FWD = 4,
  CLX_PACK_WINO4_DGRAD = 5,
  CLX_PACK_WINO4_ADJOINT = 6,
  CLX_PACK_WINO4_FUSED = 7
};
int clx_pack_weights(const float* w, float* wp, int cout, int cin, int taps,
                     int cin_pad, int cout_pad, int mode, clx_stream stream);
typedef struct clx_pack_job {
  const float* w;
  float* wp;
  int cout, cin, taps, cin_pad, cout_pad, mode;
} clx_pack_job;
int clx_pack_weights_batch(const clx_pack_job* jobs, int njobs, long long max_total, clx_stream stream);
int clx_unpack_wgrad(const float* dwpack, float* dw, int cout, int cin, int taps,
                     int rows, int cin_pad, clx_stream stream);
int clx_unpack_wgrad_wino(const float* du, float* dw, int cout, int cin, int rows,
                          int cin_pad, int tile, int ksize, int kd, clx_stream stream);

int clx_planar_to_pixel(const float* planar, float* pixel, int B, int C,
                        long long n, int ld, clx_stream stream);
int clx_pixel_to_planar(const float* pixel, float* planar, int B, int C,
                        long long n, int ld, clx_stream stream);

int clx_depth_to_space(const float* lo, int ld_lo, float* hi, int ld_hi, int B, int D, int H,
                       int W, int N, int fz, int fy, int fx, clx_stream stream);
int clx_space_to_depth(const float* hi, int ld_hi, float* lo, int ld_lo, int B, int D, int H,
                       int W, int N, int fz, int fy, int fx, clx_stream stream);

int clx_subpixel_split_weights(const float* w, float* w_skip, float* weff, int cout, int cin,
                               int C0, int N, int kd, int kh, int kw, int fz, int fy, int fx,
                               clx_stream stream);
int clx_subpixel_fold_grads(const float* g_skip, const float* g_eff, float* gw, int cout, int cin,
                            int C0, int N, int kd, int kh, int kw, int fz, int fy, int fx,
                            clx_stream stream);

int clx_maxpool_fwd(const float* x, float* y, int B, int D, int H, int W, int C,
                    int fz, int fy, int fx, clx_stream stream);
int clx_maxpool_bwd(const float* x, const float* y, const float* dy_pool,
                    const float* dskip, int ld_skip, int SD, int SH, int SW,
                    int cz, int cy, int cx, float* dx, int B, int D, int H,
                    int W, int C, int fz, int fy, int fx, clx_stream stream);
int clx_upsample_bwd(const float* dcat, int ld_cat, int coff, int LD, int LH,
                     int LW, int oz, int oy, int ox, const float* y, float* dy,
                     int B, int D, int H, int W, int C, int fz, int fy, int fx,
                     clx_stream stream);

int clx_gather_add_fwd(const float* offsets, const long long* coords, float* sel,
                       int B, int P, int ND, int Z, int Y, int X, int* oob_count,
                       clx_stream stream);
int clx_gather_add_bwd(const float* dsel, const long long* coords, float* doffsets,
                       int B, int P, int ND, int Z, int Y, int X, int* oob_count,
                       clx_stream stream);
int clx_oce_loss_fwd_bwd(const float* a, const float* r, float* da, double* sums,
                         long long npairs, int ND, float temperature,
                         float reg_weight, float grad_scale, clx_stream stream);
int clx_oce_pairs_fused(const float* offsets, const long long* anchor,
                        const long long* reference, float* doffsets, double* sums,
                        int B, int P, int ND, int Z, int Y, int X,
                        float temperature, float reg_weight, clx_stream stream);
size_t clx_oce_pairs_det_scratch_bytes(int B, int ND, long long npix);
int clx_oce_pairs_fused_det(const float* offsets, const long long* anchor, const long long* reference,
                            float* doffsets, double* sums, int B, int P, int ND, int Z, int Y, int X,
                            float temperature, float reg_weight, void* scratch, clx_stream stream);

int clx_sample_pairs(long long* anchor, long long* reference, const int* offsets, int noffsets,
                     int B, int num_anchors, int num_refs, int ND, int lo, const int* hi,
                     unsigned long long seed, unsigned long long stream_id, clx_stream stream);
int clx_adam_step(float* param, const float* grad, float* exp_avg,
                  float* exp_avg_sq, long long n, double lr, double beta1,
                  double beta2, double eps, double weight_decay, int step,
                  clx_stream stream);
int clx_adam_step_guarded(float* param, const float* grad, float* exp_avg,
                          float* exp_avg_sq, long long n, double lr, double beta1,
                          double beta2, double eps, double weight_decay, int step,
                          const double* skip_if_positive, clx_stream stream);

int clx_noise_stats(const float* preds, float* out, int T, int C, long long n,
                    clx_stream stream);
#define CLX_NOISE_MINMAX_FLOATS (2 + 2 * 1024)
int clx_noise_stats_minmax(const float* preds, float* out, int T, int C, long long n, float* std_minmax,
                           int init, clx_stream stream);

int clx_noise_inject(const float* rnd, const float* raw, float* out, int T, int n_half, long long n, float p,
                     clx_stream stream);
#define CLX_ROWS_EXTENT_DOUBLES (6 * (1 + 256))
int clx_rows_extent_f64(const double* src, long long n, int width, double* extent, clx_stream stream);
int clx_zero_many(void* const* buffers, const long long* nbytes, int count, clx_stream stream);
int clx_gather_rows_f64(const double* src, const int* rows, long long n, int width, double* dst, clx_stream stream);

size_t clx_changed_rows_workspace(int T, int ID, int IH, int IW);
int clx_changed_rows(const float* clean, const float* noisy, int T, int C, int ID, int IH, int IW, int KD, int KH,
                     int KW, int chunk, int* rows, int* counts, long long cap, void* workspace, clx_stream stream);
int clx_changed_tiles(const void* workspace, int T, int ID, int IH, int IW, int KD, int KH, int KW, int WH, int WW,
                      int tile, int chunk, int* tiles, int* counts, long long cap, clx_stream stream);
int clx_grey_rows(const float* x, int B, int ID, int IH, int IW, int KD, const int* rows, long long n, const float* wpack,
                  const float* bias, int relu, int N, float* out, int ld_out, clx_stream stream);
int clx_conv_first_dgrad(const float* dy, int ld_dy, const float* w, int N, int cin, int B, int OD, int OH, int OW, int KD,
                         float* dx, clx_stream stream);
int clx_gather_rows(const float* src, int ld_src, const int* rows, long long n, int width, float* dst, int ld_dst,
                    clx_stream stream);
int clx_scatter_rows(const float* src, int ld_src, const int* rows, long long n, int width, float* dst, int ld_dst,
                     clx_stream stream);
int clx_broadcast_rows(const float* src, long long nfloats, float* dst, int copies, clx_stream stream);

size_t clx_ms_prepare_workspace(long long npix);
int clx_ms_prepare(double* emb, const double* std, double threshold, int ND,
                   int Z, int Y, int X, double* Xout, int* index, int* nfg_out,
                   void* workspace, clx_stream stream);
int clx_ms_prepare_f32(const float* emb, const float* std, double threshold, int ND,
                       int Z, int Y, int X, double* Xout, int* index, int* nfg_out,
                       void* workspace, clx_stream stream);
int clx_ms_iterate(const double* fit, int nfit, const double* seeds, int nseeds,
                   int ND, double bandwidth, int max_iter, double* centers,
                   int* counts, int* iters, clx_stream stream);
int clx_ms_iterate_grid(const double* fit_sorted, int nfit, const int* cell_start,
                        const double* origin, double cell, int nx, int ny, int nz,
                        const double* seeds, int nseeds, int ND, double bandwidth,
                        int max_iter, double* centers, int* counts, int* iters,
                        clx_stream stream);
size_t clx_ms_bucket_workspace(int n, long long ncells);
int clx_ms_bucket(const double* fit, int n, int ND, const double* origin, double cell, int nx,
                  int ny, int nz, double* fit_sorted, int* cell_start, void* workspace,
                  clx_stream stream);
enum clx_aug_dtype { CLX_AUG_U8 = 0, CLX_AUG_U16 = 1, CLX_AUG_F32 = 2 };
size_t clx_elastic_crop_workspace(int nd, const int* crop, int B);
int clx_elastic_crop(const void* data, int dtype, int S, int C, int nd, const int* spatial, const int* crop,
                     const int* cp_shape, float factor, int elastic, int B, const double* params, const double* mats,
                     void* workspace, float* raw, float* maxima, clx_stream stream);
int clx_sample_offsets_mt19937(unsigned int* key, int* pos, int radius, int ND, long long number_offsets,
                               long long* offsets, int* rounds);
int clx_ms_dedup_centers(const double* centers, const int* counts, int n, int ND, double bandwidth,
// ... 82 lines not shown
```

Before: 309.1.

## Emit split-precision bf16 planes from Winograd and first-layer conv epilogues

Adds next_planes/next_colsum/planes_only outputs so the Winograd F(4x4,3x3) output kernel, the Winograd adjoint (dgrad) output kernel and the one-channel first-layer kernel write the 3xbf16 operand planes, and optionally column sums, for the following 1x1 split-precision GEMM directly in their epilogue. Each wavefront stages a pixel row in LDS and writes the planes in fragment layout. The planner marks those planes as fresh, so the separate split pass is skipped. With planes_only, the dense f32 output store is also skipped when nothing else reads it. The price is extra LDS, wave barriers, atomic colsum adds in the transform kernels, and a remapped work decomposition.

```diff
diff --git a/cellulus_amd/_clx.py b/cellulus_amd/_clx.py
--- a/cellulus_amd/_clx.py
+++ b/cellulus_amd/_clx.py
@@ -86,6 +86,9 @@
         ("dyplanes_valid", c_int),
         ("out_planes", c_void_p),
         ("out_colsum", c_void_p),
+        ("next_planes", c_void_p),
+        ("next_colsum", c_void_p),
+        ("planes_only", c_int),
     ]
 
 
@@ -112,6 +115,7 @@
     "clx_conv_workspace_bytes": (c_size_t, [POINTER(ClxConvDesc), _I]),
     "clx_conv_vcache_bytes": (c_size_t, [POINTER(ClxConvDesc), _I]),
     "clx_conv_sp_covers": (_I, [POINTER(ClxConvDesc), _I]),
+    "clx_conv_next_planes_check": (_I, [POINTER(ClxConvDesc)]),
     "clx_planes_bytes": (c_size_t, [_LL, _I]),
     "clx_split_planes": (_I, [_P, _LL, _LL, _I, _P, _P]),
     "clx_join_planes": (_I, [_P, _LL, _I, _P, _LL, _P]),
diff --git a/cellulus_amd/csrc/clx_common.h b/cellulus_amd/csrc/clx_common.h
--- a/cellulus_amd/csrc/clx_common.h
+++ b/cellulus_amd/csrc/clx_common.h
@@ -54,6 +54,7 @@
 static inline int cdiv(long long a, long long b) { return (int)((a + b - 1) / b); }
 
 bool clx_smallc_applicable(const clx_conv_desc* d);
+bool clx_smallc_next_planes_ok(const clx_conv_desc* d);
 int clx_smallc_fwd(const clx_conv_desc* d, hipStream_t st);
 int clx_smallc_wgrad(const clx_conv_desc* d, const float* dy, int ld_dy, float* dwpack,
                      float* dbias, hipStream_t st);
diff --git a/cellulus_amd/csrc/conv_igemm.hip b/cellulus_amd/csrc/conv_igemm.hip
--- a/cellulus_amd/csrc/conv_igemm.hip
+++ b/cellulus_amd/csrc/conv_igemm.hip
@@ -506,6 +506,33 @@
   p.accumulate = d->accumulate;
   p.bs_in = p.bs_w = p.bs_out = 0;
   p.flush_every = 0;
+}
+
+extern "C" int clx_conv_next_planes_check(const clx_conv_desc* d) {
+  CLX_REQUIRE(d != nullptr, "clx_conv_next_planes_check: null descriptor");
+  if (d->next_planes == nullptr && d->next_colsum == nullptr && !d->planes_only) return CLX_OK;
+  if (d->next_planes == nullptr && d->next_colsum == nullptr) {
+    CLX_REQUIRE(d->out_planes != nullptr && d->algo == CLX_ALGO_DIRECT && d->aplanes != nullptr && clx_sp_applicable(d) && !d->accumulate,
+                "clx_conv_fwd: planes_only needs a planes pointer: next_planes, or out_planes on the split-precision 1x1 "
+                "product (without accumulate)");
+    return CLX_OK;
+  }
+  CLX_REQUIRE(d->next_planes != nullptr, "clx_conv_fwd: next_colsum needs next_planes");
+  if (d->algo == CLX_ALGO_DIRECT && clx_smallc_next_planes_ok(d)) {
+    CLX_REQUIRE(d->next_colsum == nullptr && !d->planes_only && ((uintptr_t)d->next_planes & 15) == 0,
+                "clx_conv_fwd: the first-layer kernel takes an aligned next_planes alone (no next_colsum / planes_only)");
+    return CLX_OK;
+  }
+  CLX_REQUIRE(d->algo == CLX_ALGO_WINOGRAD4 && d->nsrc == 1 && d->KD == 1 && d->ID == 1 && d->KH == 3 && d->KW == 3 && clx_wino_sp(d) &&
+                  d->wplanes != nullptr,
+              "clx_conv_fwd: next_planes / next_colsum / planes_only need a 2-D 3x3 CLX_ALGO_WINOGRAD4 layer in the split "
+              "precision (clx_conv_sp_covers, wplanes) or the 2-D one-channel first layer with N %% 64 == 0, N >= 128; the split "
+              "1x1 product takes out_planes / out_colsum");
+  CLX_REQUIRE(d->tile_list == nullptr && d->pool_out == nullptr && !d->accumulate,
+              "clx_conv_fwd: next_planes does not go with tile_list / pool_out / accumulate");
+  CLX_REQUIRE(d->ld_out == d->N && d->N % 32 == 0 && ((uintptr_t)d->next_planes & 15) == 0,
+              "clx_conv_fwd: next_planes needs a dense output (ld_out == N) and a 16-byte aligned planes pointer");
+  return CLX_OK;
 }
 
 extern "C" int clx_conv_fwd(const clx_conv_desc* d, clx_stream stream) {
@@ -530,12 +557,15 @@
                   (d->algo == CLX_ALGO_DIRECT && d->aplanes != nullptr && clx_sp_applicable(d)),
               "clx_conv_fwd: out_planes / out_colsum / aplanes_valid need the split-precision 1x1 product "
               "(clx_conv_sp_covers, wplanes and aplanes)");
+  rc = clx_conv_next_planes_check(d);
+  if (rc) return rc;
   if (d->algo == CLX_ALGO_WINOGRAD4_FUSED) return clx_wino_fused_fwd(d, (hipStream_t)stream);
   if (d->algo != CLX_ALGO_DIRECT) return clx_wino_fwd(d, (hipStream_t)stream);
   CLX_REQUIRE(d->pool_out == nullptr && d->tile_list == nullptr && !d->adjoint,
               "clx_conv_fwd: pool_out / tile_list / adjoint need a Winograd algorithm (algo = %d)", d->algo);
   if (clx_smallc_applicable(d) && d->mask == nullptr && d->mask_bits == nullptr && d->gate_out == nullptr) {
-    clx_smallc_fwd(d, (hipStream_t)stream);
+    rc = clx_smallc_fwd(d, (hipStream_t)stream);
+    if (rc) return rc;
     CLX_CHECK_LAUNCH("clx_conv_fwd(small-channel)");
     return CLX_OK;
   }
diff --git a/cellulus_amd/csrc/conv_smallc.hip b/cellulus_amd/csrc/conv_smallc.hip
--- a/cellulus_amd/csrc/conv_smallc.hip
+++ b/cellulus_amd/csrc/conv_smallc.hip
@@ -1,4 +1,5 @@
 #include "clx_common.h"
+#include "sp_planes.h"
 
 namespace {
 
@@ -13,6 +14,7 @@
   const float* bias;
   float* out;
   int ld_out, relu;
+  char* nplanes;
   const float* dy;
   int ld_dy;
   float* dwp;
@@ -264,7 +266,7 @@
   }
 };
 
-template <int KD>
+template <int KD, bool PL = false>
 __global__ __launch_bounds__(256) void conv_grey_fwd_kernel(const SmallP p) {
   using L = GreyLane<KD>;
   const L ln(p);
@@ -304,8 +306,10 @@
 #pragma unroll
         for (int e = 0; e < 4; ++e) acc[e] = fmaxf(acc[e], 0.f);
       }
-      if (live_n && r[s].ox0 + ln.px < p.OW)
+      if (live_n && r[s].ox0 + ln.px < p.OW) {
         *reinterpret_cast<f32x4*>(p.out + (size_t)(r[s].m0 + ln.px) * p.ld_out + n) = acc;
+        if constexpr (PL) sp::store4(p.nplanes, r[s].m0 + ln.px, n, p.N >> 4, acc);
+      }
       item += stride;
     }
   }
@@ -473,16 +477,30 @@
   return taps > 1 && taps <= MAX_TAPS && d->N >= 4;
 }
 
+bool clx_smallc_next_planes_ok(const clx_conv_desc* d) {
+  return clx_smallc_applicable(d) && grey_applicable(d, d->ld_out) && d->KD == 1 && d->ID == 1 && d->N % 64 == 0 && d->N >= 128 &&
+         d->ld_out == d->N && ((uintptr_t)d->out & 15) == 0 && (!d->bias || ((uintptr_t)d->bias & 15) == 0) &&
+         d->mask == nullptr && d->mask_bits == nullptr && d->gate_out == nullptr && d->precision != CLX_PREC_F32;
+}
+
 int clx_smallc_fwd(const clx_conv_desc* d, hipStream_t st) {
   SmallP p{};
   fill(d, p);
   p.wpack = d->wpack; p.bias = d->bias; p.out = d->out; p.ld_out = d->ld_out; p.relu = d->relu;
   if (grey_applicable(d, d->ld_out) && ((uintptr_t)d->out & 15) == 0 && (!d->bias || ((uintptr_t)d->bias & 15) == 0)) {
     const dim3 grid = grey_grid(p);
+    if (d->next_planes != nullptr) {
+      const int rc = clx_sp_zero_tail(d->next_planes, p.M, p.N, 1, 0, st);
+      if (rc) return rc;
+      p.nplanes = (char*)d->next_planes;
+      conv_grey_fwd_kernel<1, true><<<grid, 256, 0, st>>>(p);
+      return CLX_OK;
+    }
     if (d->KD == 1) conv_grey_fwd_kernel<1><<<grid, 256, 0, st>>>(p);
     else conv_grey_fwd_kernel<3><<<grid, 256, 0, st>>>(p);
     return CLX_OK;
   }
+  CLX_REQUIRE(d->next_planes == nullptr, "clx_conv_fwd(small-channel): next_planes needs the one-channel first-layer kernel");
   const int ng = pick_ng(p.N);
   const int K = p.taps * 4;
   const int tiles = cdiv(p.M, PT);
diff --git a/cellulus_amd/csrc/gemm_sp.hip b/cellulus_amd/csrc/gemm_sp.hip
--- a/cellulus_amd/csrc/gemm_sp.hip
+++ b/cellulus_amd/csrc/gemm_sp.hip
@@ -137,6 +137,7 @@
   int nbm, nbn;
   char* out_planes;
   float* colsum; int colsum_n;
+  int planes_only;
   unsigned int stride_a, stride_b;
   int total_steps, steps_per_slice, nslices;
 };
@@ -217,7 +218,7 @@
     }
 #pragma unroll
     for (int j = 0; j < PH; ++j)
-      if (live[j]) *reinterpret_cast<f32x4*>(out_base + (size_t)mrow[j] * p.ld_out) = val[j];
+      if (live[j] && !p.planes_only) *reinterpret_cast<f32x4*>(out_base + (size_t)mrow[j] * p.ld_out) = val[j];
     if (p.out_planes) {
 #pragma unroll
       for (int j = 0; j < PH; ++j)
@@ -1088,6 +1089,7 @@
   CLX_REQUIRE(p.zeros != nullptr, "clx_gemm_planes: cannot resolve the device zero buffer");
   p.out_planes = batch == 1 ? (char*)ep->out_planes : nullptr;
   p.colsum = batch == 1 ? ep->out_colsum : nullptr; p.colsum_n = N;
+  p.planes_only = p.out_planes != nullptr ? ep->planes_only : 0;
   CLX_REQUIRE(p.out_planes == nullptr || ep->ld_out == N, "clx_gemm_planes: out_planes needs a dense output (ld_out == N)");
   p.nbm = cdiv(M, SP_BM); p.nbn = cdiv(N, SP_BN);
   const char* const tile_env = getenv("CLX_SP_TILE");
diff --git a/cellulus_amd/csrc/sp_planes.h b/cellulus_amd/csrc/sp_planes.h
--- a/cellulus_amd/csrc/sp_planes.h
+++ b/cellulus_amd/csrc/sp_planes.h
@@ -54,6 +54,50 @@
   c = cblk * 32 + (lane & 7) * 4;
 }
 
+constexpr int ROW_STAGE_OCT = 32 * 16 + 16;
+constexpr int ROW_STAGE_PIECE = 4 * ROW_STAGE_OCT;
+constexpr int ROW_STAGE = 3 * ROW_STAGE_PIECE;
+
+__device__ __forceinline__ void row_stage_put(char* stage, int lane, int e, const f32x4 v) {
+  u32x2 p0, p1, p2;
+  split4(v, p0, p1, p2);
+  char* w = stage + ((lane & 7) >> 1) * ROW_STAGE_OCT + ((lane >> 3) * 4 + e) * 16 + (lane & 1) * 8;
+  *reinterpret_cast<u32x2*>(w) = p0;
+  *reinterpret_cast<u32x2*>(w + ROW_STAGE_PIECE) = p1;
+  *reinterpret_cast<u32x2*>(w + 2 * ROW_STAGE_PIECE) = p2;
+}
+
+__device__ __forceinline__ void row_stage_flush(const char* stage, int lane, char* planes, int ksteps, long long row0, int nvalid,
+                                                int oct0) {
+  __builtin_amdgcn_fence(__ATOMIC_RELEASE, "wavefront");
+  __builtin_amdgcn_wave_barrier();
+  __builtin_amdgcn_fence(__ATOMIC_ACQUIRE, "wavefront");
+  const int pix = lane & 31;
+#pragma unroll
+  for (int k = 0; k < 6; ++k) {
+    const int piece = k >> 1, oct = (k & 1) * 2 + (lane >> 5);
+    const u32x4 q = *reinterpret_cast<const u32x4*>(stage + piece * ROW_STAGE_PIECE + oct * ROW_STAGE_OCT + pix * 16);
+    if (pix < nvalid) *reinterpret_cast<u32x4*>(planes + piece_offset(row0 + pix, oct0 + oct, ksteps) + piece * FRAG) = q;
+  }
+  __builtin_amdgcn_fence(__ATOMIC_RELEASE, "wavefront");
+  __builtin_amdgcn_wave_barrier();
+  __builtin_amdgcn_fence(__ATOMIC_ACQUIRE, "wavefront");
+}
+
+__device__ __forceinline__ void row_colsum_add(float* colsum, int lane, int n, int nreal, f32x4 s) {
+#pragma unroll
+  for (int e = 0; e < 4; ++e) {
+    s[e] += __shfl_xor(s[e], 8, 64);
+    s[e] += __shfl_xor(s[e], 16, 64);
+    s[e] += __shfl_xor(s[e], 32, 64);
+  }
+  if ((lane >> 3) == 0) {
+#pragma unroll
+    for (int e = 0; e < 4; ++e)
+      if (n + e < nreal) atomicAdd(colsum + n + e, s[e]);
+  }
+}
+
 }
 
 int clx_sp_zero_tail(void* planes, long long rows, int K, int batch, long long bs, hipStream_t st);
diff --git a/cellulus_amd/csrc/wino.hip b/cellulus_amd/csrc/wino.hip
--- a/cellulus_amd/csrc/wino.hip
+++ b/cellulus_amd/csrc/wino.hip
@@ -90,7 +90,7 @@
   }
 }
 
-template <int MT, int R>
+template <int MT, int R, bool PL = false>
 __global__ __launch_bounds__(256) void wino_output_kernel(const float* __restrict__ M, int N4, Geom g,
                                                           const float* __restrict__ bias, int relu,
                                                           const float* __restrict__ mask, int ld_mask,
@@ -99,23 +99,46 @@
                                                           int ld_gate, const unsigned int* __restrict__ mask_bits,
                                                           int ld_mask_bits, float* __restrict__ pool_out, int ld_pool,
                                                           long long total, const int* __restrict__ tile_list = nullptr,
-                                                          long long Tc = 0) {
+                                                          long long Tc = 0, char* __restrict__ nplanes = nullptr,
+                                                          float* __restrict__ ncolsum = nullptr, int planes_only = 0) {
   using W = WT<MT, R>;
   constexpr int A = W::A;
   constexpr int MP = MT / 2;
+  static_assert(!PL || MT == 4, "the plane-writing form deals out 4-pixel groups");
+  __shared__ __attribute__((aligned(16))) char stage_all[PL ? 4 * sp::ROW_STAGE : 16];
+  const int lane = threadIdx.x & 63;
+  char* const stage = stage_all + (PL ? (threadIdx.x >> 6) * sp::ROW_STAGE : 0);
   const int N = N4 * 4;
   const long long plane = (tile_list ? Tc : g.T) * N;
   const int sub = threadIdx.x & 7;
   for (long long i = (long long)blockIdx.x * blockDim.x + threadIdx.x; i < total;
        i += (long long)gridDim.x * blockDim.x) {
-    const int n = (int)(i % N4) * 4;
-    const long long t = i / N4;
-    const long long tg = tile_list ? (long long)tile_list[t] : t;
-    const int tx = (int)(tg % g.tw);
-    const long long q = tg / g.tw;
-    const int ty = (int)(q % g.th);
-    const int b = (int)(q / g.th);
+    int n, tx, ty, b, txg = 0;
+    long long t;
+    bool live = true;
+    if constexpr (PL) {
+      const int wv = __builtin_amdgcn_readfirstlane((int)(i >> 6));
+      const int nblk = N >> 5, ntxg = (g.tw + 7) >> 3;
+      n = (int)(wv % nblk) * 32 + (lane & 7) * 4;
+      int q = wv / nblk;
+      txg = (int)(q % ntxg);
+      q /= ntxg;
+      ty = (int)(q % g.th);
+      b = (int)(q / g.th);
+      tx = txg * 8 + (lane >> 3);
+      live = tx < g.tw;
+      t = ((long long)b * g.th + ty) * g.tw + (live ? tx : g.tw - 1);
+    } else {
+      n = (int)(i % N4) * 4;
+      t = i / N4;
+      const long long tg = tile_list ? (long long)tile_list[t] : t;
+      tx = (int)(tg % g.tw);
+      const long long q = tg / g.tw;
+      ty = (int)(q % g.th);
+      b = (int)(q / g.th);
+    }
     const float* src = M + t * N + n;
+    f32x4 csum = {0.f, 0.f, 0.f, 0.f};
     f32x4 rr[MT][A];
 #pragma unroll
     for (int s = 0; s < A; ++s) {
@@ -144,7 +167,7 @@
 #pragma unroll
       for (int cc = 0; cc < MT; ++cc) {
         const int ox = MT * tx + cc;
-        if (ox >= g.OW) continue;
+        if (ox >= g.OW || !live) continue;
         f32x4 v = {0.f, 0.f, 0.f, 0.f};
         bool first = true;
 #pragma unroll
@@ -179,7 +202,7 @@
 #pragma unroll
             for (int e = 0; e < 4; ++e) v[e] = (mk[e] > 0.f) ? v[e] : 0.f;
           }
-          st4(out + m * ld_out + n, v);
+          if (!PL || !planes_only) st4(out + m * ld_out + n, v);
         } else {
           for (int e = 0; e < 4 && n + e < Nreal; ++e) {
             float xv = v[e];
@@ -187,6 +210,10 @@
             out[m * ld_out + n + e] = xv;
           }
         }
+        if constexpr (PL) {
+          sp::row_stage_put(stage, lane, cc, v);
+          csum += v;
+        }
         if (pool_out) {
           if ((a & 1) == 0 && (cc & 1) == 0) pm[a >> 1][cc >> 1] = v;
           else {
@@ -199,31 +226,60 @@
           }
         }
       }
+      if constexpr (PL) {
+        const int x0 = 32 * txg;
+        sp::row_stage_flush(stage, lane, nplanes, N >> 4, ((long long)b * g.OH + oy) * g.OW + x0, min(32, g.OW - x0), n >> 3 & ~3);
+      }
+    }
+    if constexpr (PL) {
+      if (ncolsum) sp::row_colsum_add(ncolsum, lane, n, Nreal, csum);
     }
   }
 }
 
 constexpr int ADJ_SEG = 8;
 
-__global__ __launch_bounds__(256) void wino_adjoint_output_kernel(const float* __restrict__ Pm, int C4, int Bn, int th,
+template <bool PL = false>
+__global__ __launch_bounds__(256, PL ? 2 : 1) void wino_adjoint_output_kernel(const float* __restrict__ Pm, int C4, int Bn, int th,
                                                                   int tw, int IH, int IW, const float* __restrict__ mask,
                                                                   int ld_mask, const unsigned int* __restrict__ mask_bits,
                                                                   int ld_mask_bits, float* __restrict__ out, int ld_out,
-                                                                  int Creal, long long total) {
+                                                                  int Creal, long long total, char* __restrict__ nplanes = nullptr,
+                                                                  float* __restrict__ ncolsum = nullptr, int planes_only = 0) {
   using W = WT<4, 3>;
   constexpr int A = 6;
+  __shared__ __attribute__((aligned(16))) char stage_all[PL ? 4 * sp::ROW_STAGE : 16];
+  const int lane = threadIdx.x & 63;
+  char* const stage = stage_all + (PL ? (threadIdx.x >> 6) * sp::ROW_STAGE : 0);
   const int C = C4 * 4;
   const int bh = (IH + 3) / 4, bw = (IW + 3) / 4;
   const int nseg = (bh + ADJ_SEG - 1) / ADJ_SEG;
   const long long plane = (long long)Bn * th * tw * C;
   for (long long i = (long long)blockIdx.x * blockDim.x + threadIdx.x; i < total;
        i += (long long)gridDim.x * blockDim.x) {
-    const int c = (int)(i % C4) * 4;
-    long long t = i / C4;
-    const int bx = (int)(t % bw);
-    long long q = t / bw;
-    const int sg = (int)(q % nseg);
-    const int b = (int)(q / nseg);
+    int c, bx, sg, b, bxg = 0;
+    bool live = true;
+    if constexpr (PL) {
+      const int wv = __builtin_amdgcn_readfirstlane((int)(i >> 6));
+      const int nblk = C >> 5, nbxg = (bw + 7) >> 3;
+      c = (int)(wv % nblk) * 32 + (lane & 7) * 4;
+      int q = wv / nblk;
+      bxg = (int)(q % nbxg);
+      q /= nbxg;
+      sg = (int)(q % nseg);
+      b = (int)(q / nseg);
+      bx = bxg * 8 + (lane >> 3);
+      live = bx < bw;
+      if (!live) bx = bw - 1;
+    } else {
+      c = (int)(i % C4) * 4;
+      const long long t = i / C4;
+      bx = (int)(t % bw);
+      const long long q = t / bw;
+      sg = (int)(q % nseg);
+      b = (int)(q / nseg);
+    }
+    f32x4 csum = {0.f, 0.f, 0.f, 0.f};
     const int by0 = sg * ADJ_SEG, by1 = min(by0 + ADJ_SEG, bh);
     f32x4 carry[2][4];
 #pragma unroll
@@ -276,7 +332,7 @@
 #pragma unroll
           for (int e = 0; e < 4; ++e) {
             const int x = 4 * bx + e;
-            if (x >= IW) continue;
+            if (x >= IW || !live) continue;
             f32x4 v = d[a][e];
             if (a < 2) v += carry[a][e];
             const long long m = ((long long)b * IH + y) * IW + x;
@@ -291,7 +347,7 @@
 #pragma unroll
                 for (int k = 0; k < 4; ++k) v[k] = (mk[k] > 0.f) ? v[k] : 0.f;
               }
-              st4(out + m * ld_out + c, v);
+              if (!PL || !planes_only) st4(out + m * ld_out + c, v);
             } else {
               for (int k = 0; k < 4 && c + k < Creal; ++k) {
                 float xv = v[k];
@@ -299,11 +355,22 @@
                 out[m * ld_out + c + k] = xv;
               }
             }
+            if constexpr (PL) {
+              sp::row_stage_put(stage, lane, e, v);
+              csum += v;
+            }
           }
+          if constexpr (PL) {
+            const int x0 = 32 * bxg;
+            sp::row_stage_flush(stage, lane, nplanes, C >> 4, ((long long)b * IH + y) * IW + x0, min(32, IW - x0), c >> 3 & ~3);
+          }
         }
       }
 #pragma unroll
       for (int e = 0; e < 4; ++e) { carry[0][e] = d[4][e]; carry[1][e] = d[5][e]; }
+    }
+    if constexpr (PL) {
+      if (ncolsum) sp::row_colsum_add(ncolsum, lane, c, Creal, csum);
     }
   }
 }
@@ -749,9 +816,24 @@
                     d->mask == nullptr && d->mask_bits == nullptr && !d->accumulate,
                 "clx_conv_fwd(winograd): pool_out needs N %% 4 == 0, an aligned ld_pool >= N, and no mask / accumulate");
   }
+  if (d->next_planes != nullptr) {
+    if constexpr (MT == 4 && R == 3) {
+      const int rc = clx_sp_zero_tail(d->next_planes, (long long)gout.B * gout.OH * gout.OW, Np, 1, 0, st);
+      if (rc) return rc;
+      const long long tot_pl = (long long)gout.B * gout.th * ((gout.tw + 7) / 8) * (Np / 32) * 64;
+      CLX_LAUNCH_KIND(CLX_PROF_WINO_TRANSFORM, (wino_output_kernel<4, 3, true>), dim3(grid_for(tot_pl, 256)), dim3(256), 0, st, M, Np / 4, gout,
+                      d->bias, d->relu, d->mask, d->ld_mask, d->out, d->ld_out, d->N, 0, d->gate_out, d->ld_gate, d->mask_bits,
+                      d->ld_mask_bits, (float*)nullptr, 0, tot_pl, (const int*)nullptr, 0ll, (char*)d->next_planes, d->next_colsum,
+                      d->planes_only);
+      CLX_CHECK_LAUNCH("clx_conv_fwd(winograd, next_planes)");
+      return CLX_OK;
+    } else {
+      CLX_REQUIRE(false, "clx_conv_fwd(winograd): next_planes needs F(4x4, 3x3)");
+    }
+  }
   CLX_LAUNCH_KIND(CLX_PROF_WINO_TRANSFORM, (wino_output_kernel<MT, R>), dim3(grid_for(tot_out, 256)), dim3(256), 0, st, M, Np / 4, gout, d->bias,
                   d->relu, d->mask, d->ld_mask, d->out, d->ld_out, d->N, d->accumulate, d->gate_out, d->ld_gate, d->mask_bits,
-                  d->ld_mask_bits, d->pool_out, d->ld_pool, tot_out, list, Tout);
+                  d->ld_mask_bits, d->pool_out, d->ld_pool, tot_out, list, Tout, (char*)nullptr, (float*)nullptr, 0);
   CLX_CHECK_LAUNCH("clx_conv_fwd(winograd)");
   return CLX_OK;
 }
@@ -908,8 +990,19 @@
   const int IH = OHf + 2, IW = OWf + 2;
   const int nseg = ((IH + 3) / 4 + ADJ_SEG - 1) / ADJ_SEG;
   const long long total = (long long)d->B * planes_dx * nseg * ((IW + 3) / 4) * (Cp / 4);
-  CLX_LAUNCH_KIND(CLX_PROF_WINO_TRANSFORM, wino_adjoint_output_kernel, dim3(grid_for(total, 256)), dim3(256), 0, st, P, Cp / 4,
-                  d->B * planes_dx, th, tw, IH, IW, d->mask, d->ld_mask, d->mask_bits, d->ld_mask_bits, d->out, d->ld_out, Cp, total);
+  if (d->next_planes != nullptr) {
+    const int rc = clx_sp_zero_tail(d->next_planes, (long long)d->B * IH * IW, Cp, 1, 0, st);
+    if (rc) return rc;
+    const long long tot_pl = (long long)d->B * nseg * (((IW + 3) / 4 + 7) / 8) * (Cp / 32) * 64;
+    CLX_LAUNCH_KIND(CLX_PROF_WINO_TRANSFORM, wino_adjoint_output_kernel<true>, dim3(grid_for(tot_pl, 256)), dim3(256), 0, st, P, Cp / 4,
+                    d->B, th, tw, IH, IW, d->mask, d->ld_mask, d->mask_bits, d->ld_mask_bits, d->out, d->ld_out, Cp, tot_pl,
+                    (char*)d->next_planes, d->next_colsum, d->planes_only);
+    CLX_CHECK_LAUNCH("clx_conv_fwd(winograd adjoint, next_planes)");
+    return CLX_OK;
+  }
+  CLX_LAUNCH_KIND(CLX_PROF_WINO_TRANSFORM, wino_adjoint_output_kernel<false>, dim3(grid_for(total, 256)), dim3(256), 0, st, P, Cp / 4,
+                  d->B * planes_dx, th, tw, IH, IW, d->mask, d->ld_mask, d->mask_bits, d->ld_mask_bits, d->out, d->ld_out, Cp, total,
+                  (char*)nullptr, (float*)nullptr, 0);
   CLX_CHECK_LAUNCH("clx_conv_fwd(winograd adjoint)");
   return CLX_OK;
 }
diff --git a/cellulus_amd/models/plan.py b/cellulus_amd/models/plan.py
--- a/cellulus_amd/models/plan.py
+++ b/cellulus_amd/models/plan.py
@@ -1261,6 +1261,15 @@
             if pool is not None:
                 d.pool_out = self.buf[pool.out].data_ptr()
                 d.ld_pool = pad4(pool.channels)
+        nxt = self._pointwise_reader.get(op.out)
+        if (nxt is not None and self.keep and self._bwd_ready and tiles is None
+                and (self.algo[op.name]["fwd"] or op.param_index == 0)
+                and os.environ.get("CLX_SP_EPILOGUE_PLANES", "1") != "0"):
+            d.next_planes = self.xplanes[nxt.name].data_ptr()
+            if _clx.load().clx_conv_next_planes_check(ctypes.byref(d)) == 0:
+                self._xplanes_fresh.add(nxt.name)
+            else:
+                d.next_planes = None
         if tiles is not None:
             d.tile_list = tiles[0].data_ptr()
             d.tile_count = int(tiles[1])
@@ -1553,13 +1562,25 @@
                     self._set_mask(dd, prev.out, relu=prev.relu)
                     dd.out = self.gbuf[prev.out].data_ptr()
                     dd.ld_out = pad4(prev.cout)
-                    if (dgrad_sp and prev.name in self.xplanes and self.sp_pass[prev.name][2]
-                            and os.environ.get("CLX_SP_EPILOGUE_PLANES", "1") != "0"):
-                        other = self.dyplanes2 if dy_planes is self.dyplanes else self.dyplanes
+                    handover = (prev.name in self.xplanes and self.sp_pass[prev.name][2]
+                                and os.environ.get("CLX_SP_EPILOGUE_PLANES", "1") != "0")
+                    dead_dy = 1 if self.sp_pass[prev.name][1] and not self.algo[prev.name]["dgrad"] and prev.param_index > 0 else 0
+                    other = self.dyplanes2 if dy_planes is self.dyplanes else self.dyplanes
+                    gbp = grads[2 * prev.param_index + 1]
+                    if dgrad_sp and handover:
                         dd.out_planes = other.data_ptr()
-                        gbp = grads[2 * prev.param_index + 1]
                         dd.out_colsum = gbp.data_ptr() if gbp is not None else None
+                        dd.planes_only = dead_dy
                         dy_planes_of[prev.out] = other
+                    elif handover and self.algo[layer.name]["dgrad"] and self.sp_pass[layer.name][1]:
+                        dd.next_planes = other.data_ptr()
+                        dd.next_colsum = gbp.data_ptr() if gbp is not None else None
+                        dd.planes_only = dead_dy
+                        if _clx.load().clx_conv_next_planes_check(ctypes.byref(dd)) == 0:
+                            dy_planes_of[prev.out] = other
+                        else:
+                            dd.next_planes = dd.next_colsum = None
+                            dd.planes_only = 0
                     _clx.call("clx_conv_fwd", ctypes.byref(dd), st)
         assert not pending_skip
 
diff --git a/include/clx.h b/include/clx.h
--- a/include/clx.h
+++ b/include/clx.h
@@ -95,6 +95,9 @@
   int dyplanes_valid;
   void* out_planes;
   float* out_colsum;
+  void* next_planes;
+  float* next_colsum;
+  int planes_only;
 } clx_conv_desc;
 
 enum clx_conv_precision { CLX_PREC_F32 = 0, CLX_PREC_F32X3BF16 = 1, CLX_PREC_F32X3BF16_G64 = 2 };
@@ -120,6 +123,7 @@
                      clx_stream stream);
 
 int clx_conv_sp_covers(const clx_conv_desc* d, int pass);
+int clx_conv_next_planes_check(const clx_conv_desc* d);
 
 int clx_conv_fwd(const clx_conv_desc* d, clx_stream stream);
 
```

Result: no change. 310.9 (median of 6 runs) (+0.6%).
